# PRADUMAN-KR/Multimodal-Lip-Sync-Deepfake-Detection-System

Hardware: NVIDIA B200
Metric: windows_per_sec (higher is better)
Workload: dtype bf16

## Files before the change

### multimodal-lip-sync-deepfake-detection-system_b200/csrc/bf16_path.cu

```cuda
#include "forward_common.h"
#include "tok_front.cuh"
#include "tok_fused.cuh"
#include "token_kernels.cuh"
#include "umma_conv.cuh"
#include "stem_ring.cuh"

#include <cuda_fp16.h>

#include <algorithm>
#include <array>
#include <cstdio>
#include <cstdlib>
#include <cstring>
#include <functional>

using namespace lsd;
using namespace lsdfw;

#define LSD_ENV(name) ([]() -> const char* { static const char* const v_ = getenv(name); return v_; }())

namespace {

uint16_t f2bf(float f) {
  uint32_t u;
  memcpy(&u, &f, 4);
  if ((u & 0x7F800000u) == 0x7F800000u) return (uint16_t)(u >> 16);
  u += 0x7FFFu + ((u >> 16) & 1u);
  return (uint16_t)(u >> 16);
}

BGroup make_group(const ConvP& c, int sh, int sw, bool merge_kt = false) {
  BGroup g;
  g.Cin = c.Cin;
  for (int a = 0; a < c.kt; ++a)
    for (int b = 0; b < c.kh; ++b)
      for (int d = 0; d < c.kw; ++d) {
        BTap t;
        t.orig = (a * c.kh + b) * c.kw + d;
        t.dt = a - c.kt / 2;
        int hp = 0, wp = 0;
        const int oh = b - c.kh / 2, ow = d - c.kw / 2;
        if (sh == 2) { hp = oh & 1; t.dh = (oh - hp) / 2; } else t.dh = oh;
        if (sw == 2) { wp = ow & 1; t.dw = (ow - wp) / 2; } else t.dw = ow;
        const int set = hp * 2 + wp;
        BBand* band = nullptr;
        for (BBand& bb : g.bands)
          if (bb.set == set && (merge_kt || bb.taps[0].dt == t.dt) && (int)bb.taps.size() < UC_MAX_TAPS) band = &bb;
        if (!band) { g.bands.push_back(BBand{set, {}}); band = &g.bands.back(); }
        band->taps.push_back(t);
      }
  g.taps_total = c.kt * c.kh * c.kw;
  g.k16 = c.Cin / 16;
  return g;
}

BGroup make_group_toeplitz(const ConvP& c, int kpix, int dw_units) {
  BGroup g;
  g.Cin = c.Cin;
  g.toeplitz = 1;
  g.k16 = kpix * 4 / 16;
  for (int a = 0; a < c.kt; ++a)
    for (int b = 0; b < c.kh; ++b) {
      BTap t;
      t.orig = a * c.kh + b;
      t.dt = a - c.kt / 2;
      const int oh = b - c.kh / 2;
      const int hp = oh & 1;
      t.dh = (oh - hp) / 2;
      t.dw = dw_units;
      BBand* band = nullptr;
      for (BBand& bb : g.bands)
        if (bb.set == hp && bb.taps[0].dt == t.dt) band = &bb;
      if (!band) { g.bands.push_back(BBand{hp, {}}); band = &g.bands.back(); }
      band->taps.push_back(t);
    }
  g.taps_total = c.kt * c.kh;
  return g;
}

struct Packer {
  lsd_handle* h;
  const std::vector<float>& f32;
  std::vector<uint16_t> w;
  std::vector<float> bias;
  int ds_sh = 2, ds_sw = 2;
  void pack_group(BGroup& g, const ConvP& c, int ntile, int part = 0) {
    g.w_off = w.size();
    const int Cout = c.Cout;
    const float* W = &f32[c.w_off];
    const float* sc = c.has_scale ? &f32[c.scale_off] : nullptr;
    g.slice_stride = (size_t)(c.Cin / 16) * g.taps_total * ntile * 16;
    for (int sl = 0; sl < Cout / ntile; ++sl)
      for (int ch = 0; ch < c.Cin / 16; ++ch)
        for (const BBand& b : g.bands)
          for (const BTap& t : b.taps)
            for (int kc = 0; kc < 2; ++kc)
              for (int nn = 0; nn < ntile; ++nn)
                for (int e = 0; e < 8; ++e) {
                  const int ci = ch * 16 + kc * 8 + e, n = sl * ntile + nn;
                  const float v = W[((size_t)t.orig * c.Cin + ci) * Cout + n] * (sc ? sc[n] : 1.0f);
                  const uint16_t hi = f2bf(v);
                  if (part == 0) w.push_back(hi);
                  else { uint32_t u = (uint32_t)hi << 16; float hf; memcpy(&hf, &u, 4); w.push_back(f2bf(v - hf)); }
                }
  }
  void add_toeplitz(const std::string& name, const std::string& key, int kpix, int dw_units, bool dup_lo = false, bool halves = false) {
    const ConvP& c = h->convs.at(key);
    BLayer L;
    L.Cout = c.Cout;
    L.ntile = c.Cout;
    L.halves = halves;
    L.groups.push_back(make_group_toeplitz(c, kpix, dw_units));
    BGroup& g = L.groups[0];
    g.w_off = w.size();
    const float* W = &f32[c.w_off];
    const float* sc = c.has_scale ? &f32[c.scale_off] : nullptr;
    const int nsl = halves ? 2 : 1, ncol = c.Cout / nsl;
    g.slice_stride = (size_t)g.k16 * g.taps_total * ncol * 16;
    for (int sl = 0; sl < nsl; ++sl)
    for (int ch = 0; ch < g.k16; ++ch)
      for (const BBand& b : g.bands)
        for (const BTap& t : b.taps)
          for (int kc = 0; kc < 2; ++kc)
            for (int n = sl * ncol; n < (sl + 1) * ncol; ++n)
              for (int e = 0; e < 8; ++e) {
                const int k = ch * 16 + kc * 8 + e, j = k / 4, kw = j - 1;
                int ci = k % 4;
                const bool lo_part = dup_lo && ci == 2;
                if (dup_lo) ci = ci < 3 ? 0 : 99;
                float v = 0.f;
                if (ci < c.Cin && kw >= 0 && kw < c.kw) v = W[((size_t)(t.orig * c.kw + kw) * c.Cin + ci) * c.Cout + n] * (sc ? sc[n] : 1.0f);
                const uint16_t hi = f2bf(v);
                if (!lo_part) w.push_back(hi);
                else { uint32_t u = (uint32_t)hi << 16; float hf; memcpy(&hf, &u, 4); w.push_back(f2bf(v - hf)); }
              }
    L.bias_off = bias.size();
    for (int i = 0; i < c.Cout; ++i) bias.push_back(f32[c.shift_off + i]);
    while (w.size() % 64) w.push_back(0);
    h->blayers[name] = L;
  }
  void add(const std::string& name, const std::string& key, int sh, int sw, const std::string& ds_key = "", int ntile = 0, bool split = false,
           bool merge_kt = false, bool halves = false) {
    const ConvP& c = h->convs.at(key);
    BLayer L;
    L.Cout = c.Cout;
    L.ntile = ntile > 0 ? ntile : c.Cout;
    L.halves = halves;
    L.groups.push_back(make_group(c, sh, sw, merge_kt));
    pack_group(L.groups[0], c, halves ? L.ntile / 2 : L.ntile);
    if (split) {
      BGroup g1 = L.groups[0]; g1.src = 2;
      BGroup g2 = make_group(c, sh, sw, merge_kt);
      pack_group(g2, c, L.ntile, 1);
      L.groups.push_back(g1);
      L.groups.push_back(g2);
    }
    L.bias_off = bias.size();
    for (int i = 0; i < c.Cout; ++i) bias.push_back(f32[c.shift_off + i]);
    if (!ds_key.empty()) {
      const ConvP& d = h->convs.at(ds_key);
      const int sh_ds = ds_sh, sw_ds = ds_sw;
      BGroup gd = make_group(d, sh_ds, sw_ds);
      gd.src = 1;
      pack_group(gd, d, L.ntile);
      L.groups.push_back(gd);
      if (split) {
        BGroup g1 = gd; g1.src = 3;
        BGroup g2 = make_group(d, sh_ds, sw_ds); g2.src = 1;
        pack_group(g2, d, L.ntile, 1);
        L.groups.push_back(g1);
        L.groups.push_back(g2);
      }
      for (int i = 0; i < c.Cout; ++i) bias[L.bias_off + i] += f32[d.shift_off + i];
    }
    while (w.size() % 64) w.push_back(0);
    h->blayers[name] = L;
  }
  void add_fold(const std::string& name, const std::string& key, const std::string& ds_key, int ntile) {
    const ConvP& c = h->convs.at(key);
    if (c.kt != 3 || c.kh != 3 || c.kw != 3 || c.Cout % ntile) return;
    BLayer L;
    L.Cout = c.Cout;
    L.ntile = ntile;
    BGroup g;
    g.Cin = c.Cin;
    g.taps_total = 27;
    g.k16 = c.Cin / 16;
    for (int b = 0; b < 3; ++b)
      for (int d = 0; d < 3; ++d) {
        BBand band{b * 3 + d, {}};
        for (int a = 0; a < 3; ++a) band.taps.push_back(BTap{(a * 3 + b) * 3 + d, a - 1, b - 1, d - 1});
        g.bands.push_back(band);
      }
    pack_group(g, c, ntile);
    L.groups.push_back(g);
    L.bias_off = bias.size();
    for (int i = 0; i < c.Cout; ++i) bias.push_back(f32[c.shift_off + i]);
    if (!ds_key.empty()) {
      const ConvP& d = h->convs.at(ds_key);
      BGroup gd = make_group(d, 1, 1);
      gd.src = 1;
      pack_group(gd, d, ntile);
      L.groups.push_back(gd);
      for (int i = 0; i < c.Cout; ++i) bias[L.bias_off + i] += f32[d.shift_off + i];
    }
    while (w.size() % 64) w.push_back(0);
    h->blayers[name] = L;
  }
  void add_split(const std::string& name, const std::string& key, int ntile) {
    const ConvP& c = h->convs.at(key);
    BLayer L;
    L.Cout = c.Cout;
    L.ntile = ntile;
    BGroup g0 = make_group(c, 1, 1);
    pack_group(g0, c, ntile, 0);
    BGroup g1 = g0; g1.src = 2;
    BGroup g2 = make_group(c, 1, 1);
    pack_group(g2, c, ntile, 1);
    L.groups = {g0, g1, g2};
    L.bias_off = bias.size();
    for (int i = 0; i < c.Cout; ++i) bias.push_back(f32[c.shift_off + i]);
    while (w.size() % 64) w.push_back(0);
    h->blayers[name] = L;
  }
};

struct PBuf {
  size_t off = 0;
  int C = 0, sets = 1;
  UcGeom g;
  int64_t plane_stride = 0, set_stride = 0, origin = 0;
  size_t bytes() const { return (size_t)sets * set_stride * 2; }
};

constexpr int TILE_MAX = 1024;

PBuf make_pbuf(int C, int sets, UcGeom g) {
  PBuf b;
  b.C = C; b.sets = sets; b.g = g;
  const int64_t gf = ((int64_t)g.SL + 3 * g.RW + 16 + 7) / 8 * 8;
  const int64_t gb = gf + TILE_MAX;
  const int64_t plane_pos = (gf + g.P_total + gb + 7) / 8 * 8;
  b.origin = gf * 8;
  b.plane_stride = plane_pos * 8;
  b.set_stride = b.plane_stride * (C / 8);
  return b;
}

bool fold_route(int H, int W) {
  static const bool off = LSD_ENV("LSD_FOLD") && atoi(LSD_ENV("LSD_FOLD")) == 0;
  return !off && H * W <= 36;
}

struct BPlan {
  Shapes s;
  bool fold3 = false, fold4 = false;
  Plan f32;
  std::map<std::string, PBuf> pb;
  size_t planar_begin = 0, planar_end = 0;
  UcGeom gt, g33, gta;
  void addp(const char* name, int C, int sets, UcGeom g) {
    PBuf b = make_pbuf(C, sets, g);
    f32.cursor = (f32.cursor + 255) & ~size_t(255);
    b.off = f32.cursor;
    f32.cursor += b.bytes();
    pb[name] = b;
  }
};

void build_plan(const Shapes& s, BPlan& P, bool video = true) {
  P.s = s;
  Plan& p = P.f32;
  const int64_t B = s.B, T = s.T, TA = s.A4;
  if (video) p.add("vid", B * T * s.H * s.W * 3);
  p.add("aud", B * s.F * s.Ta);
  if (video) p.add("v_feat", B * T * 256);
  p.add("a_feat", B * TA * 256);
  if (video) {
  p.add("v_emb", B * T * 256);
  p.add("a_emb", B * TA * 256);
  p.add("a_int", B * T * 256);
  p.add("proj_v", B * T * 768);
  p.add("proj_a", B * T * 768);
  p.add("vcomb", B * T * 1024);
  }
  p.add("acomb", B * T * 1024);
  p.add("a_fint", B * T * 256);
  p.add("gate_in", B * T * 512);
  if (video) p.add("gate_h", B * T * 256);
  p.add("fused", B * T * 256);
  p.add("tok", B * (T + 1) * 256);
  if (video) {
  p.add("tok_qkv", B * (T + 1) * 768);
  p.add("comb", B * 448);
  }
  P.planar_begin = (p.cursor + 255) & ~size_t(255);
  const int Bn = s.B, Tn = s.T;
  const UcGeom g1 = make_geom(Bn, Tn, s.H1, s.W1), g2 = make_geom(Bn, Tn, s.H2, s.W2), g3 = make_geom(Bn, Tn, s.H3, s.W3),
               g4 = make_geom(Bn, Tn, s.H4, s.W4), gd = make_geom(Bn, s.Td, s.H4, s.W4), gh = make_geom(Bn, Tn, s.Hg, s.Wg);
  const UcGeom gs = make_geom_ex(Bn, Tn, s.Hs, s.Ws, 1, 2, 0, 0, 2);
  if (video) {
  P.addp("xs", 8, 2, gs);
  P.addp("xl", 8, 2, gs);
  P.addp("s_out", 64, 1, gs);
  P.addp("x1", 64, 1, g1);
  P.addp("l1a", 64, 1, g1);
  P.addp("y1", 64, 4, g2);
  P.addp("l2a", 128, 1, g2);
  P.fold3 = fold_route(s.H3, s.W3);
  P.fold4 = fold_route(s.H4, s.W4);
  const UcGeom gr = make_geom_ex(Bn, Tn, 1, 1, 1, 0, 0, 0, 0);
  if (P.fold3) P.addp("y2", 128, s.H2 * s.W2, gr); else P.addp("y2", 128, 4, g3);
  if (P.fold3) P.addp("l3a", 256, s.H3 * s.W3, gr); else P.addp("l3a", 256, 1, g3);
  if (P.fold4) P.addp("y3", 256, s.H3 * s.W3, gr); else P.addp("y3", 256, 4, g4);
  if (P.fold4) P.addp("l4a", 256, s.H4 * s.W4, gr); else P.addp("l4a", 256, 1, g4);
  P.addp("y4", 256, 1, g4);
  P.addp("art_a", 128, 1, g4);
  P.addp("art_b", 64, 1, g4);
  P.addp("delta", 256, 1, gd);
  P.addp("artd_a", 128, 1, gd);
  P.addp("artd_b", 64, 1, gd);
  P.addp("hf_f", 32, 4, gh);
  P.addp("hf_b", 64, 1, gh);
  }
  const UcGeom as = make_geom_ex(Bn, 1, s.Fs, s.As, 0, 2, 0, 0, 4);
  auto g2d = [&](int H, int W) { return make_geom_ex(Bn, 1, H, W, 0, 1, 0, 1, 0); };
  P.addp("xa", 8, 2, as);
  for (const char* sfx : {"", "_lo"}) {
    auto nm = [&](const char* n) { return std::string(n) + sfx; };
    P.addp(nm("sa_out").c_str(), 64, 1, as);
    P.addp(nm("a1").c_str(), 64, 1, g2d(s.F1, s.A1));
    P.addp(nm("a1a").c_str(), 64, 1, g2d(s.F1, s.A1));
    P.addp(nm("ya1").c_str(), 64, 4, g2d(s.F2, s.A2));
    P.addp(nm("a2a").c_str(), 128, 1, g2d(s.F2, s.A2));
    P.addp(nm("ya2").c_str(), 128, 4, g2d(s.F3, s.A3));
    P.addp(nm("a3a").c_str(), 256, 1, g2d(s.F3, s.A3));
    P.addp(nm("ya3").c_str(), 256, 4, g2d(s.F4, s.A4));
    P.addp(nm("a4a").c_str(), 256, 1, g2d(s.F4, s.A4));
    P.addp(nm("ya4").c_str(), 256, 1, g2d(s.F4, s.A4));
  }
  P.gt = make_geom_ex(Bn, 1, 1, Tn, 0, 0, 0, 3, 0);
  P.g33 = make_geom_rows(Bn * (Tn + 1));
  P.gta = make_geom_rows(Bn * (int)TA);
  for (const char* sfx : {"", "_lo"}) {
    auto nm = [&](const char* n) { return std::string(n) + sfx; };
    P.addp(nm("afeat_p").c_str(), 256, 1, P.gta);
    if (!video) { P.addp(nm("afint_p").c_str(), 256, 1, P.gt); continue; }
    for (const char* n : {"vfeat_p", "vemb_p", "aint_p", "afint_p", "att1_p", "att2_p", "blend_p", "fused_p"}) P.addp(nm(n).c_str(), 256, 1, P.gt);
    P.addp(nm("gatein_p").c_str(), 512, 1, P.gt);
    P.addp(nm("mscat_p").c_str(), 768, 1, P.gt);
    P.addp(nm("tokln_p").c_str(), 256, 1, P.g33);
    P.addp(nm("tokatt_p").c_str(), 256, 1, P.g33);
    P.addp(nm("tokff_p").c_str(), 1024, 1, P.g33);
  }
  P.planar_end = p.cursor;
}

struct BCtx {
  lsd_handle* h;
  char* ws;
  const BPlan* P;
  cudaStream_t st;
  int max_ctas = 0;
  __nv_bfloat16* base(const PBuf& b) const { return reinterpret_cast<__nv_bfloat16*>(ws + b.off); }
  __nv_bfloat16* org(const PBuf& b) const { return base(b) + b.origin; }
  float* f(const char* name) const { return reinterpret_cast<float*>(ws + P->f32.find(name)); }
  const float* W(const char* key) const { return h->warena + h->vecs.at(key); }
};

struct UArgs {
  const PBuf* in = nullptr;
  const PBuf* in_ds = nullptr;
  const PBuf* in_lo = nullptr;
  const PBuf* in_ds_lo = nullptr;
  const PBuf* res_lo = nullptr;
  const PBuf* yp_lo = nullptr;
  UcGeom og;
  int act = ACT_NONE;
  const PBuf* yp = nullptr;
  int y_plane_off = 0;
  int y_mode = -1;
  const PBuf* res = nullptr;
  float* y32 = nullptr;
  int y32_ld = 0, y32_outer_stride = -1, y32_row_off = 0;
  const float* res32 = nullptr;
  int res32_ld = 0;
};

int stage_program(const BCtx& c, const std::string& name, UmmaConvP& p, const std::function<void(std::vector<UcStageDesc>&)>& build,
                  std::initializer_list<uint64_t> salt = {}) {
  uint64_t hkey = 1469598103934665603ull;
  for (uint64_t v : salt) { hkey ^= v; hkey *= 1099511628211ull; hkey ^= hkey >> 29; }
  static_assert(sizeof(UmmaConvP) % 8 == 0, "UmmaConvP is hashed in 8-byte words");
  const uint64_t* pw = reinterpret_cast<const uint64_t*>(&p);
  for (size_t i = 0; i < sizeof(p) / 8; ++i) { hkey ^= pw[i]; hkey *= 1099511628211ull; hkey ^= hkey >> 29; }
  auto it = c.h->prog_cache.find(hkey);
  if (it == c.h->prog_cache.end()) {
    std::vector<UcStageDesc> host;
    build(host);
    const size_t bytes = host.size() * sizeof(UcStageDesc);
    if (!c.h->prog_arena) {
      c.h->prog_cap = 64u << 20;
      if (cudaMalloc(&c.h->prog_arena, c.h->prog_cap) != cudaSuccess) return lsd_fail(c.h, LSD_ERR_CUDA, "stage-program arena allocation failed");
      c.h->prog_cursor = 0;
    }
    if (c.h->prog_cursor + bytes > c.h->prog_cap) {
      cudaDeviceSynchronize();
      c.h->prog_cache.clear();
      c.h->prog_cursor = 0;
      ++c.h->generation;
    }
    char* dst = c.h->prog_arena + c.h->prog_cursor;
    cudaError_t e = cudaMemcpy(dst, host.data(), bytes, cudaMemcpyHostToDevice);
    if (e != cudaSuccess) return lsd_fail(c.h, LSD_ERR_CUDA, "%s: stage program upload: %s", name.c_str(), cudaGetErrorString(e));
    c.h->prog_cursor += (bytes + 255) & ~size_t(255);
    it = c.h->prog_cache.emplace(hkey, dst).first;
  }
  p.prog = reinterpret_cast<const UcStageDesc*>(it->second);
  return 0;
}

int run_umma(const BCtx& c, const std::string& name, const UArgs& a) {
  const BLayer& L = c.h->blayers.at(name);
  const UcGeom& og = a.og;
  if (og.P_total >= ((int64_t)1 << 31) - 1024) return lsd_fail(c.h, LSD_ERR_SHAPE, "%s: more than 2^31 padded positions in one launch (reduce the batch)", name.c_str());
  UmmaConvP p;
  memset(&p, 0, sizeof(p));
  p.w = reinterpret_cast<const __nv_bfloat16*>(c.h->barena);
  p.bias = c.h->bbias + L.bias_off;
  p.Cout = L.ntile;
  const int slices = L.Cout / L.ntile;
  p.act = a.act;
  p.g = og;
  p.cta2 = L.halves ? 1 : 0;
  if (a.yp) {
    p.y_mode = a.y_mode >= 0 ? a.y_mode : (a.yp->sets == 4 ? UC_Y_PARITY : UC_Y_PLAIN);
    p.y = c.org(*a.yp) + (int64_t)a.y_plane_off * a.yp->plane_stride;
    p.y_plane_stride = a.yp->plane_stride; p.y_set_stride = a.yp->set_stride;
    p.g2 = a.yp->g;
    p.ymap_W = og.W;
    if (a.yp_lo) p.ylo = c.org(*a.yp_lo) + (int64_t)a.y_plane_off * a.yp_lo->plane_stride;
  }
  if (a.y32) {
    p.y32 = a.y32; p.y32_ld = a.y32_ld;
    p.y32_outer_stride = a.y32_outer_stride >= 0 ? a.y32_outer_stride : og.W;
    p.y32_row_off = a.y32_row_off;
  }
  if (a.res) { p.res = c.org(*a.res); p.res_plane_stride = a.res->plane_stride; }
  if (a.res_lo) p.res_lo = c.org(*a.res_lo);
  if (a.res32) { p.res32 = a.res32; p.res32_ld = a.res32_ld; }
  const int mt_cap = L.ntile <= 32 ? 8 : 4;
  const int mt2 = std::max(1, std::min(mt_cap, 256 / L.ntile));
  p.MT = std::max(1, std::min(mt_cap, 512 / L.ntile));
  const int cta_budget = (c.max_ctas > 0 && c.max_ctas < c.h->num_sms) ? c.max_ctas : c.h->num_sms;
  while (p.MT > 1 && ((og.P_total + p.MT * 128 - 1) / (p.MT * 128)) * slices < cta_budget) p.MT /= 2;
  p.nbuf = (p.MT <= mt2 && 2 * p.MT * L.ntile <= 512) ? 2 : 1;
  if (const char* e = LSD_ENV("LSD_UMMA_NBUF")) {
    const int v = atoi(e);
    if (v == 1) p.nbuf = 1;
    if (v == 2 && 2 * L.ntile <= 512) { p.nbuf = 2; p.MT = std::min(p.MT, mt2); }
  }
  p.issuers = std::min(p.MT, 4);
  if (const char* e = LSD_ENV("LSD_UMMA_ISSUERS")) { const int v = atoi(e); if (v >= 1 && v <= 4 && v <= p.MT && p.MT % v == 0 && p.MT / v <= 4) p.issuers = v; }
  uint32_t cols = 32;
  while ((int)cols < p.nbuf * p.MT * L.ntile) cols *= 2;
  p.tmem_cols = cols;
  const int S = p.MT * 128;
  int nb = 0, max_a = 0, max_taps = 0, min_k16 = 1 << 30;
  bool any_toeplitz = false;
  p.ngroups = (int)L.groups.size();
  for (int gi = 0; gi < p.ngroups; ++gi) {
    const BGroup& G = L.groups[gi];
    const PBuf* srcp = G.src == 0 ? a.in : (G.src == 1 ? a.in_ds : (G.src == 2 ? a.in_lo : a.in_ds_lo));
    if (!srcp) return lsd_fail(c.h, LSD_ERR_ARG, "%s: missing input for group %d", name.c_str(), gi);
    const PBuf& src = *srcp;
    UcGroup& ug = p.groups[gi];
    ug.band_begin = nb;
    ug.k16 = G.k16;
    ug.taps_total = G.taps_total;
    ug.w_off = (int64_t)G.w_off;
    ug.slice_stride = (int64_t)G.slice_stride;
    int tap_begin = 0;
    int wkb = 40;
    if (const char* e = LSD_ENV("LSD_UMMA_WKB")) wkb = std::max(8, atoi(e));
    const int tmax = std::max(1, std::min(UC_MAX_TAPS, (wkb * 1024) / (L.ntile * 32)));
    for (const BBand& b : G.bands) {
      const int nt = (int)b.taps.size();
      const int pieces = (nt + tmax - 1) / tmax, per = (nt + pieces - 1) / pieces;
      for (int t0 = 0; t0 < nt; t0 += per) {
        const int t1 = std::min(nt, t0 + per);
        if (nb >= UC_MAX_BANDS) return lsd_fail(c.h, LSD_ERR_UNSUPPORTED, "%s: too many bands", name.c_str());
        UcBand& ub = p.bands[nb++];
        ub.base = c.org(src) + (int64_t)b.set * src.set_stride;
        ub.plane_stride = src.plane_stride;
        ub.toeplitz = G.toeplitz;
        ub.chunk_stride = G.toeplitz ? 16 : 2 * src.plane_stride;
        int mn = INT32_MAX, mx = INT32_MIN;
        for (int j = t0; j < t1; ++j) {
          const BTap& t = b.taps[j];
          const int sft = t.dt * og.SL + t.dh * og.RW + t.dw;
          mn = std::min(mn, sft); mx = std::max(mx, sft);
        }
        ub.start = mn;
        ub.len_extra = mx - mn;
        ub.ntaps = t1 - t0;
        ub.tap_begin = tap_begin;
        for (int j = t0; j < t1; ++j) ub.rel[j - t0] = b.taps[j].dt * og.SL + b.taps[j].dh * og.RW + b.taps[j].dw - mn;
        tap_begin += ub.ntaps;
        max_a = std::max(max_a, G.toeplitz ? (S + ub.len_extra + 1 + 2 * (G.k16 - 1)) * 16 : 2 * (S + ub.len_extra) * 16);
        max_taps = std::max(max_taps, ub.ntaps);
        min_k16 = std::min(min_k16, G.k16);
        any_toeplitz = any_toeplitz || G.toeplitz;
        if (-(int64_t)ub.start * 8 > src.origin || (int64_t)mx * 8 > src.origin)
          return lsd_fail(c.h, LSD_ERR_UNSUPPORTED, "%s: guard zone too small", name.c_str());
      }
    }
    ug.band_end = nb;
  }
  p.nbands = nb;
  const int w_chunk = max_taps * (L.halves ? L.ntile / 2 : L.ntile) * 32;
  if (any_toeplitz) p.kpack = min_k16;
  else {
    bool single_band = true;
    for (int gi = 0; gi < p.ngroups; ++gi) single_band = single_band && (p.groups[gi].band_end - p.groups[gi].band_begin) == 1;
    int stage_kb = single_band ? 64 : 24;
    if (const char* e = LSD_ENV("LSD_UMMA_STAGE_KB")) stage_kb = std::max(8, atoi(e));
    p.kpack = std::max(1, std::min(std::min(8, min_k16), (stage_kb * 1024) / (max_a + w_chunk)));
  }
  p.a_stage_bytes = ((uint32_t)(any_toeplitz ? max_a : max_a * p.kpack) + 127u) & ~127u;
  p.w_stage_bytes = (uint32_t)(w_chunk * p.kpack);
  const uint32_t stage = p.a_stage_bytes + p.w_stage_bytes;
  p.nst_tile = 0;
  for (int gi = 0; gi < p.ngroups; ++gi)
    p.nst_tile += ((p.groups[gi].k16 + p.kpack - 1) / p.kpack) * (p.groups[gi].band_end - p.groups[gi].band_begin);
  const uint32_t prog_bytes = (uint32_t)p.nst_tile * (uint32_t)umma_conv_stage_desc_bytes();
  uint32_t budget = 211u * 1024u;
  const uint32_t extra_bytes = (uint32_t)umma_conv_extra_smem_bytes(p);
  budget -= extra_bytes;
  if (prog_bytes + 2 * stage > budget) return lsd_fail(c.h, LSD_ERR_UNSUPPORTED, "%s: stage program of %u bytes does not fit", name.c_str(), prog_bytes);
  int stages = (int)((budget - prog_bytes) / stage);
  stages = std::max(2, std::min(stages, 8));
  if ((size_t)stages * stage + prog_bytes + extra_bytes + 1024 > 223u * 1024u) return lsd_fail(c.h, LSD_ERR_UNSUPPORTED, "%s: stage of %u bytes does not fit", name.c_str(), stage);
  p.stages = stages;
  double kflop = 0;
  for (const BGroup& G : L.groups) kflop += (double)G.taps_total * G.Cin;
  if (L.groups[0].toeplitz) { const ConvP& cp = c.h->convs.at(name); kflop = (double)cp.kt * cp.kh * cp.kw * cp.Cin; }
  if (const char* e = getenv("LSD_UMMA_SKIP")) p.skip = atoi(e);
  if (const char* why = umma_conv_config_error(p)) return lsd_fail(c.h, LSD_ERR_UNSUPPORTED, "%s: %s", name.c_str(), why);
  if (int rc = stage_program(c, name, p, [&](std::vector<UcStageDesc>& v) { v.resize((size_t)p.nst_tile); umma_conv_build_program(p, v.data()); }))
    return rc;
  if (const char* e = getenv("LSD_UMMA_TRACE")) {
    static long long* dbuf = nullptr;
    if (!dbuf) cudaMalloc(&dbuf, 512);
    cudaMemsetAsync(dbuf, 0, 512, c.st);
    p.dbg = dbuf;
    launch_umma_conv(p, slices, c.st, c.h->num_sms, c.max_ctas);
    long long hv[64];
    cudaMemcpyAsync(hv, dbuf, 512, cudaMemcpyDeviceToHost, c.st);
    cudaStreamSynchronize(c.st);
    if (atoi(e) > 0)
      fprintf(stderr, "[umma] %-34s MT=%d N=%d slices=%d stages=%d kpack=%d tiles=%lld | prologue %lld, first-data %lld, mma-issued %lld, acc-done %lld, epi-done %lld, total %lld cycles\n",
              name.c_str(), p.MT, p.Cout, slices, p.stages, p.kpack, hv[7], hv[1] - hv[0], hv[2] - hv[0], hv[3] - hv[0], hv[4] - hv[0], hv[5] - hv[0], hv[6] - hv[0]);
    if (atoi(e) > 1) {
      fprintf(stderr, "        full-wait done at:");
      for (int i = 0; i < 24 && hv[8 + i]; ++i) fprintf(stderr, " %lld", hv[8 + i] - hv[0]);
      fprintf(stderr, "\n        producer issue at:");
      for (int i = 0; i < 24 && hv[32 + i]; ++i) fprintf(stderr, " %lld", hv[32 + i] - hv[0]);
      fprintf(stderr, "\n        copies issued at: ");
      for (int i = 0; i < 8 && hv[56 + i]; ++i) fprintf(stderr, " %lld", hv[56 + i] - hv[0]);
      fprintf(stderr, "\n");
    }
    return 0;
  }
  c.h->prof.begin(c.st, 2.0 * (double)og.N * og.T * og.H * og.W * L.Cout * kflop, name.rfind("visual_encoder.", 0) == 0 ? 2 : 3);
  launch_umma_conv(p, slices, c.st, c.h->num_sms, c.max_ctas);
  c.h->prof.end(c.st);
  return 0;
}

int ring_table(const BCtx& c, const UcGeom& g, const lsd_handle::RingTab** out) {
  lsd_handle* h = c.h;
  const int T = g.T, CH = (g.SL + 127) / 128;
  const int64_t G = (int64_t)g.N * CH * T;
  const int budget = (c.max_ctas > 0 && c.max_ctas < h->num_sms) ? c.max_ctas : h->num_sms;
  uint64_t key = 1469598103934665603ull;
  for (uint64_t v : {(uint64_t)g.N, (uint64_t)T, (uint64_t)g.SL, (uint64_t)g.TS, (uint64_t)g.ot, (uint64_t)budget}) { key ^= v; key *= 1099511628211ull; key ^= key >> 29; }
  auto it = h->ring_tabs.find(key);
  if (it == h->ring_tabs.end()) {
    int grid = budget;
    int64_t Lr = (G + 2 * (int64_t)grid - 1) / (2 * (int64_t)grid);
    if (Lr < 8) { Lr = 8; grid = (int)((G + 2 * Lr - 1) / (2 * Lr)); }
    if (grid < 1) grid = 1;
    std::vector<std::vector<SrStep>> lists((size_t)2 * grid);
    size_t nsteps = 0;
    auto add_range = [&](int sg, int64_t col, int ta, int tb) {
      const int n = (int)(col / CH), sp = (int)(col % CH);
      const int t_first = std::max(ta - 1, 0);
      for (int t_in = t_first; t_in <= tb; ++t_in) {
        SrStep st;
        st.in_pos = (int32_t)(((int64_t)n * g.TS + t_in + g.ot) * g.SL + (int64_t)sp * 128);
        const int t_out = t_in - 1;
        st.flags = SR_ACTIVE | (t_in == t_first ? SR_FIRST : 0u) | ((t_out >= ta && t_out < tb) ? SR_STORE : 0u) |
                   ((uint32_t)std::min(128, g.SL - sp * 128) << 8);
        lists[sg].push_back(st);
      }
    };
    for (int sg = 0; sg < 2 * grid; ++sg) {
      int64_t g0 = (int64_t)sg * Lr;
      const int64_t g1 = std::min(G, g0 + Lr);
      while (g0 < g1) {
        const int64_t col = g0 / T;
        const int ta = (int)(g0 % T), tb = (int)std::min<int64_t>(T, ta + (g1 - g0));
        add_range(sg, col, ta, tb);
        g0 += tb - ta;
      }
    }
    for (int sg = 0; sg < 2 * grid; ++sg) nsteps = std::max(nsteps, lists[sg].size());
    std::vector<SrStep> flat((size_t)2 * grid * nsteps);
    memset(flat.data(), 0, flat.size() * sizeof(SrStep));
    for (int sg = 0; sg < 2 * grid; ++sg) std::copy(lists[sg].begin(), lists[sg].end(), flat.begin() + (size_t)sg * nsteps);
    lsd_handle::RingTab tab;
    tab.nsteps = (int)nsteps; tab.grid = grid;
    if (cudaMalloc(&tab.dev, std::max<size_t>(flat.size(), 1) * sizeof(SrStep)) != cudaSuccess ||
        cudaMemcpy(tab.dev, flat.data(), flat.size() * sizeof(SrStep), cudaMemcpyHostToDevice) != cudaSuccess)
      return lsd_fail(h, LSD_ERR_CUDA, "stem: step table upload failed");
    it = h->ring_tabs.emplace(key, tab).first;
  }
  *out = &it->second;
  return 0;
}

int run_stem_ring(const BCtx& c, const PBuf& xs, const PBuf& so) {
  lsd_handle* h = c.h;
  const UcGeom& g = xs.g;
  if (g.P_total >= ((int64_t)1 << 31) - 4096) return lsd_fail(h, LSD_ERR_SHAPE, "stem: more than 2^31 padded positions in one launch (reduce the batch)");
  const BLayer& L = h->blayers.at("visual_encoder.stem");
  StemRingP p;
  memset(&p, 0, sizeof(p));
  p.xs[0] = c.org(xs);
  p.xs[1] = c.org(xs) + xs.set_stride;
  p.w = reinterpret_cast<const __nv_bfloat16*>(h->barena) + h->stem_ring_w_off;
  p.bias = h->bbias + L.bias_off;
  p.y = c.org(so);
  p.y_plane_stride = so.plane_stride;
  p.g = g;
  p.ntap[0] = 3; p.ntap[1] = 4;
  for (int t = 0; t < 4; ++t) { p.rel[0][t] = t * g.RW; p.rel[1][t] = t * g.RW; }
  p.start[0] = -g.RW; p.start[1] = -2 * g.RW;
  p.units[0] = 128 + 2 * g.RW + 3; p.units[1] = 128 + 3 * g.RW + 3;
  if ((int64_t)(2 * g.RW + 3) * 8 > xs.origin) return lsd_fail(h, LSD_ERR_UNSUPPORTED, "stem: guard zone too small");
  const lsd_handle::RingTab* tab = nullptr;
  if (int trc = ring_table(c, g, &tab)) return trc;
  p.steps = reinterpret_cast<const SrStep*>(tab->dev);
  p.nsteps = tab->nsteps;
  p.nst = 6;
  if (const char* e = getenv("LSD_SR_SKIP")) p.skip = atoi(e);
  while (p.nst > 3 && stem_ring_smem_bytes(p) > 223u * 1024u) --p.nst;
  if (stem_ring_smem_bytes(p) > 223u * 1024u) return lsd_fail(h, LSD_ERR_UNSUPPORTED, "stem: batch too large for the ring kernel (LSD_STEM_RING=0)");
  const ConvP& cp = h->convs.at("visual_encoder.stem");
  h->prof.begin(c.st, 2.0 * (double)g.N * g.T * g.H * g.W * 64.0 * (double)cp.kt * cp.kh * cp.kw * cp.Cin, 2);
  if (getenv("LSD_SR_TRACE")) {
    static long long* dbuf = nullptr;
    constexpr int kDbg = 256 + 4 * 160;
    if (!dbuf) cudaMalloc(&dbuf, kDbg * sizeof(long long));
    cudaMemsetAsync(dbuf, 0, kDbg * sizeof(long long), c.st);
    p.dbg = dbuf;
    launch_stem_ring(p, tab->grid, c.st);
    long long hv[kDbg];
    cudaMemcpyAsync(hv, dbuf, sizeof(hv), cudaMemcpyDeviceToHost, c.st);
    cudaStreamSynchronize(c.st);
    {
      long long g0 = INT64_MAX, g1 = 0, cmin = INT64_MAX, cmax = 0, csum = 0, smax = 0;
      const int nc = std::min(tab->grid, 160);
      for (int i = 0; i < nc; ++i) g0 = std::min(g0, hv[256 + 4 * i]);
      for (int i = 0; i < nc; ++i) {
        const long long* d = hv + 256 + 4 * i;
        g1 = std::max(g1, d[1]); smax = std::max(smax, d[0] - g0);
        const long long cy = d[3] - d[2];
        cmin = std::min(cmin, cy); cmax = std::max(cmax, cy); csum += cy;
      }
      fprintf(stderr, "[sr] %d CTAs x %d steps: kernel span %.1f us (globaltimer), latest CTA start +%.1f us, CTA cycles min %lld avg %lld max %lld\n", nc,
              p.nsteps, (g1 - g0) / 1e3, smax / 1e3, cmin, csum / nc, cmax);
    }
    const long long t0 = hv[0];
    for (int k = 0; k < 32; ++k)
      fprintf(stderr, "[sr] step %2d | prod free %7lld issued %7lld | mma landed %7lld blockfree %7lld issued %7lld | epi complete %7lld back %7lld\n", k + 16,
              hv[(0 * 32 + k) * 2] - t0, hv[(0 * 32 + k) * 2 + 1] - t0, hv[(1 * 32 + k) * 2] - t0, hv[(1 * 32 + k) * 2 + 1] - t0,
              hv[(2 * 32 + k) * 2] - t0, hv[(3 * 32 + k) * 2] - t0, hv[(3 * 32 + k) * 2 + 1] - t0);
    h->prof.end(c.st);
    return 0;
  }
  launch_stem_ring(p, tab->grid, c.st);
  h->prof.end(c.st);
  return 0;
}

#define RUN(name, ...)                            \
  do {                                            \
    UArgs a_;                                     \
    __VA_ARGS__;                                  \
    if ((rc = run_umma(b, name, a_))) return rc;  \
  } while (0)

#define RUNC(ctx, name, ...)                        \
  do {                                              \
    UArgs a_;                                       \
    __VA_ARGS__;                                    \
    if ((rc = run_umma(ctx, name, a_))) return rc;  \
  } while (0)

#define RUNS(name, ...)                            \
  do {                                             \
    UArgs a_;                                      \
    __VA_ARGS__;                                   \
    if ((rc = run_umma(bs, name, a_))) return rc;  \
  } while (0)

PlanarOut pout(const BCtx& c, const PBuf& p, const PBuf* lo = nullptr, int plane_off = 0) {
  PlanarOut o;
  o.y = c.org(p) + (int64_t)plane_off * p.plane_stride;
  o.ylo = lo ? c.org(*lo) + (int64_t)plane_off * lo->plane_stride : nullptr;
  o.plane_stride = p.plane_stride;
  if (p.g.ow > 0 && p.g.HP == 1) { o.grp = p.g.W; o.grp_stride = p.g.RW; o.off = p.g.ow; }
  else { o.grp = 0; o.grp_stride = 0; o.off = 0; }
  return o;
}

int res_stage_umma(const BCtx& b, const std::string& p, const PBuf& x, const PBuf& mid, const PBuf& y, bool has_ds, int y_mode,
                   const PBuf* x_lo = nullptr, const PBuf* mid_lo = nullptr, const PBuf* y_lo = nullptr) {
  int rc = 0;
  RUN(p + ".conv1", a_.in = &x; a_.in_lo = x_lo; a_.og = mid.g; a_.act = ACT_RELU; a_.yp = &mid; a_.yp_lo = mid_lo);
  if (has_ds) RUN(p + ".conv2", a_.in = &mid; a_.in_lo = mid_lo; a_.in_ds = &x; a_.in_ds_lo = x_lo; a_.og = mid.g; a_.act = ACT_RELU;
                  a_.yp = &y; a_.yp_lo = y_lo; a_.y_mode = y_mode);
  else RUN(p + ".conv2", a_.in = &mid; a_.in_lo = mid_lo; a_.og = mid.g; a_.act = ACT_RELU; a_.yp = &y; a_.yp_lo = y_lo; a_.y_mode = y_mode;
           a_.res = &x; a_.res_lo = x_lo);
  return 0;
}

int run_umma_fold(const BCtx& c, const std::string& name, const PBuf& x, int Hi, int Wi, int stride, const PBuf* x_ds, int Hd, int Wd,
                  int Ho, int Wo, const PBuf& yp, int y_mode) {
  const auto itL = c.h->blayers.find(name + "#fold");
  if (itL == c.h->blayers.end()) return lsd_fail(c.h, LSD_ERR_UNSUPPORTED, "%s: no weights packed for the folded route (LSD_FOLD=0)", name.c_str());
  const BLayer& L = itL->second;
  const UcGeom& og = x.g;
  if (og.P_total >= ((int64_t)1 << 31) - 1024) return lsd_fail(c.h, LSD_ERR_SHAPE, "%s: more than 2^31 rows in one launch (reduce the batch)", name.c_str());
  if ((L.groups.size() == 2) != (x_ds != nullptr) || x.sets != Hi * Wi || (x_ds && x_ds->sets != Hd * Wd))
    return lsd_fail(c.h, LSD_ERR_ARG, "%s: folded inputs do not match the layer", name.c_str());
  UmmaConvP p;
  memset(&p, 0, sizeof(p));
  p.w = reinterpret_cast<const __nv_bfloat16*>(c.h->barena);
  p.bias = c.h->bbias + L.bias_off;
  p.Cout = L.ntile;
  p.act = ACT_RELU;
  p.g = og;
  p.fold = 1;
  p.y_mode = y_mode;
  p.y = c.org(yp);
  p.y_plane_stride = yp.plane_stride; p.y_set_stride = yp.set_stride;
  p.g2 = yp.g;
  p.ymap_W = Wo;
  int mt = 2;
  if (const char* e = LSD_ENV("LSD_FOLD_MT")) mt = std::max(1, std::min(4, atoi(e)));
  p.MT = (int)std::max<int64_t>(1, std::min<int64_t>(mt, (og.P_total + 127) / 128));
  p.nbuf = 1;
  p.issuers = std::min(p.MT, 4);
  uint32_t cols = 32;
  while ((int)cols < p.MT * L.ntile) cols *= 2;
  p.tmem_cols = cols;
  const int S = p.MT * 128;
  const PBuf* srcs[2] = {&x, x_ds};
  p.ngroups = (int)L.groups.size();
  p.nbands = p.ngroups;
  int max_a = 0, max_w = 0, min_k16 = 1 << 30;
  for (int gi = 0; gi < p.ngroups; ++gi) {
    const BGroup& G = L.groups[gi];
    UcGroup& ug = p.groups[gi];
    ug.band_begin = gi; ug.band_end = gi + 1;
    ug.k16 = G.k16; ug.taps_total = G.taps_total;
    ug.w_off = (int64_t)G.w_off; ug.slice_stride = (int64_t)G.slice_stride;
    UcBand& ub = p.bands[gi];
    const PBuf& src = *srcs[gi];
    ub.base = c.org(src);
    ub.plane_stride = src.plane_stride;
    ub.chunk_stride = 2 * src.plane_stride;
    ub.ntaps = gi == 0 ? 3 : 1;
    ub.start = gi == 0 ? -1 : 0;
    ub.len_extra = gi == 0 ? 2 : 0;
    for (int j = 0; j < ub.ntaps; ++j) ub.rel[j] = j;
    if ((int64_t)8 > src.origin) return lsd_fail(c.h, LSD_ERR_UNSUPPORTED, "%s: guard zone too small", name.c_str());
    max_a = std::max(max_a, 2 * (S + ub.len_extra) * 16);
    max_w = std::max(max_w, ub.ntaps * L.ntile * 32);
    min_k16 = std::min(min_k16, G.k16);
  }
  p.kpack = std::max(1, std::min(std::min(8, min_k16), (48 * 1024) / (max_a + max_w)));
  p.a_stage_bytes = ((uint32_t)(max_a * p.kpack) + 127u) & ~127u;
  p.w_stage_bytes = (uint32_t)(max_w * p.kpack);
  const int cslices = L.Cout / L.ntile;
  std::vector<std::array<int, 3>> pos;
  auto inb = [&](int o, int k, int n) { const int i = stride * o + k - 1; return i >= 0 && i < n; };
  for (int ho = 0; ho < Ho; ++ho)
    for (int wo = 0; wo < Wo; ++wo) {
      int nq = 0;
      for (int kh = 0; kh < 3; ++kh)
        for (int kw = 0; kw < 3; ++kw) nq += inb(ho, kh, Hi) && inb(wo, kw, Wi);
      pos.push_back({-nq, ho, wo});
    }
  std::stable_sort(pos.begin(), pos.end(), [](const std::array<int, 3>& a, const std::array<int, 3>& b) { return a[0] < b[0]; });
  const int nslices = (int)pos.size() * cslices;
  if (nslices > UC_MAX_FSLICES || Ho > 255 || Wo > 255) return lsd_fail(c.h, LSD_ERR_UNSUPPORTED, "%s: map too large for the folded route", name.c_str());
  auto chunks = [&](int k16) { return (k16 + p.kpack - 1) / p.kpack; };
  int off = 0;
  for (int i = 0; i < nslices; ++i) {
    const auto& q = pos[(size_t)(i / cslices)];
    const int nst = -q[0] * chunks(p.groups[0].k16) + (x_ds ? chunks(p.groups[1].k16) : 0);
    p.fslice[i] = UcFoldSlice{(uint16_t)off, (uint16_t)nst, (uint8_t)q[1], (uint8_t)q[2], (uint8_t)(i % cslices), 0};
    p.nst_tile = std::max(p.nst_tile, nst);
    off += nst;
  }
  if (off > 65535) return lsd_fail(c.h, LSD_ERR_UNSUPPORTED, "%s: folded stage programs too long", name.c_str());
  const uint32_t stage = p.a_stage_bytes + p.w_stage_bytes;
  const uint32_t prog_bytes = (uint32_t)p.nst_tile * (uint32_t)umma_conv_stage_desc_bytes();
  const uint32_t budget = 211u * 1024u - (uint32_t)umma_conv_extra_smem_bytes(p);
  if (prog_bytes + 2 * stage > budget) return lsd_fail(c.h, LSD_ERR_UNSUPPORTED, "%s: stage program of %u bytes does not fit", name.c_str(), prog_bytes);
  p.stages = std::max(2, std::min((int)((budget - prog_bytes) / stage), 8));
  if (const char* e = getenv("LSD_UMMA_SKIP")) p.skip = atoi(e);
  if (const char* why = umma_conv_config_error(p)) return lsd_fail(c.h, LSD_ERR_UNSUPPORTED, "%s: %s", name.c_str(), why);
  auto build = [&](std::vector<UcStageDesc>& v) {
    for (int i = 0; i < nslices; ++i) {
      const UcFoldSlice& f = p.fslice[i];
      for (int kh = 0; kh < 3; ++kh)
        for (int kw = 0; kw < 3; ++kw) {
          if (!inb(f.h, kh, Hi) || !inb(f.w, kw, Wi)) continue;
          UcBand bq = p.bands[0];
          bq.base = c.org(x) + (int64_t)((stride * f.h + kh - 1) * Wi + stride * f.w + kw - 1) * x.set_stride;
          bq.tap_begin = (kh * 3 + kw) * 3;
          for (int c0 = 0; c0 < p.groups[0].k16; c0 += p.kpack) v.push_back(umma_conv_stage(p, p.groups[0], bq, 0, c0, f.col));
        }
      if (x_ds) {
        UcBand bd = p.bands[1];
        bd.base = c.org(*x_ds) + (int64_t)(2 * f.h * Wd + 2 * f.w) * x_ds->set_stride;
        for (int c0 = 0; c0 < p.groups[1].k16; c0 += p.kpack) v.push_back(umma_conv_stage(p, p.groups[1], bd, 1, c0, f.col));
      }
    }
  };
  if (int rc = stage_program(c, name + "#fold", p, build, {(uint64_t)Hi, (uint64_t)Wi, (uint64_t)stride, (uint64_t)Hd, (uint64_t)Wd,
                                                          (uint64_t)x.set_stride, (uint64_t)(x_ds ? x_ds->set_stride : 0)})) return rc;
  double kflop = 0;
  for (const BGroup& G : L.groups) kflop += (double)G.taps_total * G.Cin;
  c.h->prof.begin(c.st, 2.0 * (double)og.N * og.T * Ho * Wo * L.Cout * kflop, 2);
  launch_umma_conv(p, nslices, c.st, c.h->num_sms, c.max_ctas);
  c.h->prof.end(c.st);
  return 0;
}

int res_stage_fold(const BCtx& b, const std::string& p, const PBuf& x, int Hi, int Wi, const PBuf& mid, int Ho, int Wo, const PBuf& y, int y_mode) {
  int rc = 0;
  if ((rc = run_umma_fold(b, p + ".conv1", x, Hi, Wi, 2, nullptr, 0, 0, Ho, Wo, mid, UC_Y_FOLD))) return rc;
  return run_umma_fold(b, p + ".conv2", mid, Ho, Wo, 1, &x, Hi, Wi, Ho, Wo, y, y_mode);
}

}

static int pack_tok_fused(lsd_handle* h, const std::vector<float>& f32) {
  std::vector<TfBlock> blocks;
  tf_layer_blocks(blocks);
  std::vector<uint32_t> stage_bytes;
  for (const TfBlock& b : blocks)
    for (int k0 = 0; k0 < b.k16; k0 += b.kps) stage_bytes.push_back((uint32_t)b.kps * (uint32_t)b.N * 32u);
  std::vector<__half> w;
  std::vector<float> vec((size_t)TF_LAYERS * TF_VEC_LAYER + (size_t)(2 * TF_LAYERS + 1) * TF_D, 0.f);
  std::vector<float> cum(TF_D, 0.f);
  float* cum_out = vec.data() + (size_t)TF_LAYERS * TF_VEC_LAYER;
  for (int l = 0; l < TF_LAYERS; ++l) {
    const std::string k = "t" + std::to_string(l);
    const ConvP &cin = h->convs.at(k + ".in"), &cout = h->convs.at(k + ".out"), &cf1 = h->convs.at(k + ".ff1"), &cf2 = h->convs.at(k + ".ff2");
    const size_t w0 = w.size();
    for (const TfBlock& b : blocks) {
      const ConvP& c = b.kind == 0 ? cin : (b.kind == 1 ? cout : (b.kind == 2 ? cf1 : cf2));
      for (int k16 = 0; k16 < b.k16; ++k16)
        for (int pl = 0; pl < 2; ++pl)
          for (int n = 0; n < b.N; ++n)
            for (int e = 0; e < 8; ++e) {
              const int kk = k16 * 16 + pl * 8 + e;
              int co, ci;
              if (b.kind == 0) { co = ((n % 96) / 32) * 256 + (2 * b.idx + n / 96) * 32 + (n % 32); ci = kk; }
              else if (b.kind == 1) { co = n; ci = 64 * b.idx + kk; }
              else if (b.kind == 2) { co = 128 * b.idx + n; ci = kk; }
              else { co = n; ci = 128 * b.idx + kk; }
              w.push_back(__float2half_rn(f32[c.w_off + (size_t)ci * c.Cout + co]));
            }
    }
    if (l == 0) h->tokf_layer_bytes = (uint32_t)((w.size() - w0) * sizeof(__half));
    float* lv = vec.data() + (size_t)l * TF_VEC_LAYER;
    const char* names[4] = {".ln1.w", ".ln1.b", ".ln2.w", ".ln2.b"};
    for (int i = 0; i < 4; ++i) memcpy(lv + 256 * i, &f32[h->vecs.at(k + names[i])], 256 * sizeof(float));
    for (int n = 0; n < 768; ++n) {
      const int hp = n / 192, r = n % 192;
      lv[1024 + n] = f32[cin.shift_off + ((r % 96) / 32) * 256 + (2 * hp + r / 96) * 32 + (r % 32)];
    }
    memcpy(lv + 1024 + 768, &f32[cf1.shift_off], 1024 * sizeof(float));
    memcpy(cum_out + (size_t)(2 * l) * TF_D, cum.data(), TF_D * sizeof(float));
    for (int i = 0; i < TF_D; ++i) cum[i] += f32[cout.shift_off + i];
    memcpy(cum_out + (size_t)(2 * l + 1) * TF_D, cum.data(), TF_D * sizeof(float));
    for (int i = 0; i < TF_D; ++i) cum[i] += f32[cf2.shift_off + i];
  }
  memcpy(cum_out + (size_t)(2 * TF_LAYERS) * TF_D, cum.data(), TF_D * sizeof(float));
  h->tokf_n_stage = (int)stage_bytes.size();
  for (void* q : {(void*)h->tokf_w, (void*)h->tokf_stage_bytes, (void*)h->tokf_vec}) if (q) cudaFree(q);
  h->tokf_w = nullptr; h->tokf_stage_bytes = nullptr; h->tokf_vec = nullptr;
  cudaError_t e = cudaMalloc(&h->tokf_w, w.size() * sizeof(__half));
  if (e == cudaSuccess) e = cudaMemcpy(h->tokf_w, w.data(), w.size() * sizeof(__half), cudaMemcpyHostToDevice);
  if (e == cudaSuccess) e = cudaMalloc(&h->tokf_stage_bytes, stage_bytes.size() * sizeof(uint32_t));
  if (e == cudaSuccess) e = cudaMemcpy(h->tokf_stage_bytes, stage_bytes.data(), stage_bytes.size() * sizeof(uint32_t), cudaMemcpyHostToDevice);
  if (e == cudaSuccess) e = cudaMalloc(&h->tokf_vec, vec.size() * sizeof(float));
  if (e == cudaSuccess) e = cudaMemcpy(h->tokf_vec, vec.data(), vec.size() * sizeof(float), cudaMemcpyHostToDevice);
  if (e != cudaSuccess) return lsd_fail(h, LSD_ERR_CUDA, "pack_tok_fused: %s", cudaGetErrorString(e));
  return 0;
}

static int pack_tok_front(lsd_handle* h, const std::vector<float>& f32) {
  std::vector<__half> w;
  w.reserve((size_t)TFR_K16_TOTAL * 16 * 256);
  auto emit = [&](int k16, auto&& get) {
    for (int k = 0; k < k16; ++k)
      for (int pl = 0; pl < 2; ++pl)
        for (int n = 0; n < 256; ++n)
          for (int e = 0; e < 8; ++e) w.push_back(__float2half_rn(get(k * 16 + pl * 8 + e, n)));
  };
  const ConvP &o0 = h->convs.at("cross.v2a.out"), &o1 = h->convs.at("cross.a2v.out"), &g0 = h->convs.at("cross.gate0"),
              &fu = h->convs.at("cross.fuse"), &pp = h->convs.at("temporal.pre_scale_proj");
  for (const ConvP* o : {&o0, &o1})
    for (int hp = 0; hp < 4; ++hp) emit(4, [&](int ci, int co) { return f32[o->w_off + (size_t)(64 * hp + ci) * 256 + co]; });
  emit(32, [&](int ci, int co) { return f32[g0.w_off + (size_t)ci * 256 + co]; });
  emit(16, [&](int ci, int co) { return f32[fu.w_off + (size_t)ci * 256 + co]; });
  const int ks[3] = {3, 5, 7};
  for (int b = 0; b < 3; ++b) {
    const ConvP& c = h->convs.at("temporal.branch_k" + std::to_string(ks[b]));
    for (int j = 0; j < ks[b]; ++j)
      emit(16, [&](int ci, int co) { return f32[c.w_off + ((size_t)j * 256 + ci) * 256 + co] * (c.has_scale ? f32[c.scale_off + co] : 1.0f); });
    emit(16, [&](int ci, int co) { return f32[pp.w_off + (size_t)(256 * b + ci) * 256 + co]; });
  }
  if (w.size() != (size_t)TFR_N_STAGES * TFR_STAGE_BYTES / sizeof(__half)) return lsd_fail(h, LSD_ERR_WEIGHTS, "pack_tok_front: stream size mismatch");
  std::vector<float> vec(TFR_V_TOTAL, 0.f);
  auto cp = [&](int dst, size_t src, int n) { memcpy(vec.data() + dst, &f32[src], (size_t)n * sizeof(float)); };
  cp(TFR_V_BO0, o0.shift_off, 256); cp(TFR_V_BO1, o1.shift_off, 256); cp(TFR_V_BG0, g0.shift_off, 256);
  cp(TFR_V_WG2, h->vecs.at("cross.gate2.w"), 256); cp(TFR_V_BG2, h->vecs.at("cross.gate2.b"), 1);
  cp(TFR_V_BF, fu.shift_off, 256);
  cp(TFR_V_SH3, h->convs.at("temporal.branch_k3").shift_off, 256); cp(TFR_V_SH5, h->convs.at("temporal.branch_k5").shift_off, 256);
  cp(TFR_V_SH7, h->convs.at("temporal.branch_k7").shift_off, 256);
  cp(TFR_V_BP, pp.shift_off, 256); cp(TFR_V_CLS, h->vecs.at("temporal.cls"), 256);
  for (void* q : {(void*)h->tokfr_w, (void*)h->tokfr_vec}) if (q) cudaFree(q);
  h->tokfr_w = nullptr; h->tokfr_vec = nullptr;
  cudaError_t e = cudaMalloc(&h->tokfr_w, w.size() * sizeof(__half));
  if (e == cudaSuccess) e = cudaMemcpy(h->tokfr_w, w.data(), w.size() * sizeof(__half), cudaMemcpyHostToDevice);
  if (e == cudaSuccess) e = cudaMalloc(&h->tokfr_vec, vec.size() * sizeof(float));
  if (e == cudaSuccess) e = cudaMemcpy(h->tokfr_vec, vec.data(), vec.size() * sizeof(float), cudaMemcpyHostToDevice);
  if (e != cudaSuccess) return lsd_fail(h, LSD_ERR_CUDA, "pack_tok_front: %s", cudaGetErrorString(e));
  return 0;
}

int pack_bf16_weights(lsd_handle* h, const std::vector<float>& f32_arena) {
  Packer P{h, f32_arena, {}, {}};
  memcpy(h->lapw_host, &f32_arena[h->convs.at("art.lap").w_off], sizeof(h->lapw_host));
  h->blayers.clear();
  const int vstr[4] = {1, 2, 2, 2};
  for (int l = 1; l <= 4; ++l) {
    const std::string p = "visual_encoder.layer" + std::to_string(l);
    const int s = vstr[l - 1];
    int nt = l >= 3 ? 128 : 0;
    if (const char* e = getenv(l == 3 ? "LSD_UMMA_NT3" : (l == 4 ? "LSD_UMMA_NT4" : "LSD_UMMA_NTX"))) nt = atoi(e);
    const bool pairs = l == 1;
    P.add(p + ".conv1", p + ".conv1", s, s, "", nt, false, l >= 2, pairs);
    P.ds_sh = 2; P.ds_sw = 2;
    P.add(p + ".conv2", p + ".conv2", 1, 1, l == 1 ? "" : p + ".downsample", nt, false, false, pairs);
    if (l >= 3) {
      int fnt = 128;
      if (const char* e = LSD_ENV("LSD_FOLD_NT")) fnt = atoi(e) == 256 ? 256 : 128;
      P.add_fold(p + ".conv1#fold", p + ".conv1", "", fnt);
      P.add_fold(p + ".conv2#fold", p + ".conv2", p + ".downsample", fnt);
    }
  }
  P.add_toeplitz("visual_encoder.stem", "visual_encoder.stem", 8, 0, false, true);
  {
    const ConvP& c = h->convs.at("visual_encoder.stem");
    h->stem_ring_w_off = 0;
    if (c.kt == 3 && c.kh == 7 && c.kw == 7 && c.Cin == 3 && c.Cout == 64) {
      h->stem_ring_w_off = P.w.size();
      const float* W = &f32_arena[c.w_off];
      const float* sc = c.has_scale ? &f32_arena[c.scale_off] : nullptr;
      for (int set = 0; set < 2; ++set)
        for (int b = 0; b < 7; ++b) {
          if (((b - 3) & 1) != set) continue;
          for (int ch = 0; ch < 2; ++ch)
            for (int kc = 0; kc < 2; ++kc)
              for (int n = 0; n < 192; ++n)
                for (int e = 0; e < 8; ++e) {
                  const int k = ch * 16 + kc * 8 + e, j = k / 4, kw = j - 1, ci = k % 4, a = n / 64, co = n % 64;
                  float v = 0.f;
                  if (ci < 3 && kw >= 0 && kw < 7) v = W[((size_t)((a * 7 + b) * 7 + kw) * 3 + ci) * 64 + co] * (sc ? sc[co] : 1.0f);
                  P.w.push_back(f2bf(v));
                }
        }
      while (P.w.size() % 64) P.w.push_back(0);
    }
  }
  P.add_toeplitz("art.hf0", "art.hf0", 4, 1);
  P.add("art.td0", "art.td0", 1, 1);
  P.add("art.td3", "art.td3", 1, 1);
  P.add("art.hf3", "art.hf3", 2, 2);
  P.add_toeplitz("audio_encoder.stem", "audio_encoder.stem", 8, 0, true);
  const int ash[4] = {1, 2, 2, 2}, asw[4] = {1, 2, 1, 1};
  for (int l = 1; l <= 4; ++l) {
    const std::string p = "audio_encoder.layer" + std::to_string(l);
    P.add(p + ".conv1", p + ".conv1", ash[l - 1], asw[l - 1], "", 0, true);
    P.ds_sh = ash[l - 1]; P.ds_sw = asw[l - 1];
    P.add(p + ".conv2", p + ".conv2", 1, 1, l == 1 ? "" : p + ".downsample", 0, true);
  }
  int wide = 128;
  if (const char* e = LSD_ENV("LSD_UMMA_NTW")) wide = atoi(e);
  int narrow = 64;
  if (const char* e = LSD_ENV("LSD_UMMA_NTN")) narrow = atoi(e);
  for (const char* k : {"projection.visual_proj", "projection.audio_proj", "cross.v2a.out", "cross.a2v.out",
                        "cross.gate0", "cross.fuse", "temporal.branch_k3", "temporal.branch_k5", "temporal.branch_k7",
                        "temporal.pre_scale_proj"})
    P.add_split(k, k, narrow);
  for (const char* k : {"cross.in_v", "cross.in_a", "cross.vcomb", "cross.acomb"}) P.add_split(k, k, wide);
  for (int l = 0; l < 4; ++l)
    for (const char* k : {".in", ".out", ".ff1", ".ff2"})
      P.add_split("t" + std::to_string(l) + k, "t" + std::to_string(l) + k, (k[1] == 'i' || (k[1] == 'f' && k[3] == '1')) ? wide : narrow);
  if (h->barena) { cudaFree(h->barena); h->barena = nullptr; }
  if (h->bbias) { cudaFree(h->bbias); h->bbias = nullptr; }
  cudaError_t e = cudaMalloc(&h->barena, P.w.size() * 2);
  if (e == cudaSuccess) e = cudaMemcpy(h->barena, P.w.data(), P.w.size() * 2, cudaMemcpyHostToDevice);
  if (e == cudaSuccess) e = cudaMalloc(&h->bbias, P.bias.size() * 4);
  if (e == cudaSuccess) e = cudaMemcpy(h->bbias, P.bias.data(), P.bias.size() * 4, cudaMemcpyHostToDevice);
  if (e != cudaSuccess) return lsd_fail(h, LSD_ERR_CUDA, "pack_bf16_weights: %s", cudaGetErrorString(e));
  if (int rc = pack_tok_fused(h, f32_arena)) return rc;
  return pack_tok_front(h, f32_arena);
}

void make_plan_bf16(lsd_handle* h, int B, int T, int H, int W, int F, int Ta, std::vector<Stage>& stages, size_t& bytes) {
  Shapes s;
  if (make_shapes(h, B, T, H, W, F, Ta, s) != 0) { bytes = 0; return; }
  BPlan P;
  build_plan(s, P);
  stages = P.f32.stages;
  bytes = P.f32.cursor;
}

struct Timeline {
  bool on = false;
  std::vector<std::pair<std::string, cudaEvent_t>> marks;
  void mark(cudaStream_t st, const char* name) {
    if (!on) return;
    cudaEvent_t e; cudaEventCreate(&e); cudaEventRecord(e, st);
    marks.emplace_back(name, e);
  }
  void dump() {
    if (!on || marks.empty()) return;
    cudaDeviceSynchronize();
    fprintf(stderr, "[timeline]");
    for (auto& m : marks) { float ms = 0; cudaEventElapsedTime(&ms, marks[0].second, m.second); fprintf(stderr, " %s=%.0f", m.first.c_str(), ms * 1000.0f); }
    fprintf(stderr, " (us)\n");
    for (auto& m : marks) cudaEventDestroy(m.second);
    marks.clear();
  }
};
static Timeline g_tl;

static int audio_encoder_bf16(const BCtx& b, const Shapes& s, bool inputs_ready, const void* audio, int adt) {
  const BPlan& P = *b.P;
  auto pbf = [&](const char* n) -> const PBuf& { return P.pb.at(n); };
  cudaStream_t st = b.st;
  int rc = 0;
  const PBuf &xa = pbf("xa"), &sao = pbf("sa_out"), &a1 = pbf("a1");
  if (inputs_ready) launch_audio_rows(b.f("aud"), LSD_F32, b.org(xa), xa.set_stride, xa.g, s.F, s.Ta, st);
  else launch_audio_rows(audio, adt, b.org(xa), xa.set_stride, xa.g, s.F, s.Ta, st);
  RUN("audio_encoder.stem", a_.in = &xa; a_.og = xa.g; a_.act = ACT_RELU; a_.yp = &sao; a_.yp_lo = &pbf("sa_out_lo"));
  launch_planar_maxpool(b.org(sao), sao.plane_stride, sao.g, b.org(a1), a1.plane_stride, a1.g, 64, st, b.org(pbf("sa_out_lo")), b.org(pbf("a1_lo")));
  if ((rc = res_stage_umma(b, "audio_encoder.layer1", a1, pbf("a1a"), pbf("ya1"), false, UC_Y_PARITY, &pbf("a1_lo"), &pbf("a1a_lo"), &pbf("ya1_lo")))) return rc;
  if ((rc = res_stage_umma(b, "audio_encoder.layer2", pbf("ya1"), pbf("a2a"), pbf("ya2"), true, UC_Y_PARITY_H, &pbf("ya1_lo"), &pbf("a2a_lo"), &pbf("ya2_lo")))) return rc;
  if ((rc = res_stage_umma(b, "audio_encoder.layer3", pbf("ya2"), pbf("a3a"), pbf("ya3"), true, UC_Y_PARITY_H, &pbf("ya2_lo"), &pbf("a3a_lo"), &pbf("ya3_lo")))) return rc;
  if ((rc = res_stage_umma(b, "audio_encoder.layer4", pbf("ya3"), pbf("a4a"), pbf("ya4"), true, UC_Y_PLAIN, &pbf("ya3_lo"), &pbf("a4a_lo"), &pbf("ya4_lo")))) return rc;
  const PBuf& ya4 = pbf("ya4");
  launch_planar_mean2(b.org(ya4), ya4.plane_stride, ya4.g, 256, b.f("a_feat"), 256, 2, pout(b, pbf("afeat_p"), &pbf("afeat_p_lo")), st,
                      b.org(pbf("ya4_lo")));
  return 0;
}

static bool token_front_enabled(int T) {
  const char* e = getenv("LSD_TOK_FRONT");
  return !(e && atoi(e) == 0) && tok_front_supported(T);
}
static int token_path_bf16(const BCtx& b, const Shapes& s, bool combined = false, const float* vcomb = nullptr, int K = 1) {
  const BPlan& P = *b.P;
  auto pbf = [&](const char* n) -> const PBuf& { return P.pb.at(n); };
  cudaStream_t st = b.st;
  const int B = s.B, T = s.T, TA = s.A4, NT = T + 1;
  const UcGeom gt = P.gt;
  int rc = 0;
  lsd_handle* h = b.h;
  if (!h->tok_stream[0]) {
    for (int i = 0; i < 2; ++i)
      if (cudaStreamCreateWithFlags(&h->tok_stream[i], cudaStreamNonBlocking) != cudaSuccess ||
          cudaEventCreateWithFlags(&h->ev_tok_join[i], cudaEventDisableTiming) != cudaSuccess)
        return lsd_fail(h, LSD_ERR_CUDA, "token helper stream creation failed");
    if (cudaEventCreateWithFlags(&h->ev_tok_fork, cudaEventDisableTiming) != cudaSuccess) return lsd_fail(h, LSD_ERR_CUDA, "token helper event creation failed");
  }
  BCtx b1 = b, b2 = b;
  b1.st = h->tok_stream[0]; b2.st = h->tok_stream[1];
  auto fork = [&](int n) { cudaEventRecord(h->ev_tok_fork, st); for (int i = 0; i < n; ++i) cudaStreamWaitEvent(h->tok_stream[i], h->ev_tok_fork, 0); };
  auto join = [&](int n) { for (int i = 0; i < n; ++i) { cudaEventRecord(h->ev_tok_join[i], h->tok_stream[i]); cudaStreamWaitEvent(st, h->ev_tok_join[i], 0); } };
  float *pv = combined ? nullptr : b.f("proj_v"), *pa = combined ? nullptr : b.f("proj_a"), *gi = b.f("gate_in");
  if (!combined) {
    fork(1);
    launch_lerp_tokens_p(b.f("a_emb"), b.f("a_int"), B, TA, T, 256, pout(b, pbf("aint_p"), &pbf("aint_p_lo")), b1.st);
    RUNC(b1, "cross.in_a", a_.in = &pbf("aint_p"); a_.in_lo = &pbf("aint_p_lo"); a_.og = gt; a_.y32 = pa; a_.y32_ld = 768);
    RUN("cross.in_v", a_.in = &pbf("vemb_p"); a_.in_lo = &pbf("vemb_p_lo"); a_.og = gt; a_.y32 = pv; a_.y32_ld = 768);
    join(1);
  }
  g_tl.mark(st, "T:inproj");
  float* tok = b.f("tok");
  if (token_front_enabled(T)) {
    TokFrontP fp;
    memset(&fp, 0, sizeof(fp));
    if (combined) {
      fp.v_emb = vcomb ? vcomb : b.f("vcomb"); fp.pv = fp.v_emb + 256; fp.a_int = b.f("acomb"); fp.pa = fp.a_int + 256;
      fp.ld_e = 1024; fp.ld_p = 1024;
    } else {
      fp.pv = pv; fp.pa = pa; fp.v_emb = b.f("v_emb"); fp.a_int = b.f("a_int");
      fp.ld_e = 256; fp.ld_p = 768;
    }
    fp.gi = gi; fp.fused = b.f("fused"); fp.tok = tok;
    fp.w = reinterpret_cast<const __half*>(h->tokfr_w);
    fp.vec = h->tokfr_vec;
    fp.B = B; fp.T = T; fp.K = K;
    tok_front_geometry(T, fp.SL, fp.G, fp.KW);
    if (getenv("LSD_TOKF_TRACE")) {
      static long long* dbuf = nullptr;
      if (!dbuf) cudaMalloc(&dbuf, 256 * sizeof(long long));
      cudaMemsetAsync(dbuf, 0, 256 * sizeof(long long), st);
      fp.dbg = dbuf;
      launch_tok_front(fp, st);
      std::vector<long long> hv(256);
      cudaMemcpyAsync(hv.data(), dbuf, 256 * sizeof(long long), cudaMemcpyDeviceToHost, st);
      cudaStreamSynchronize(st);
      const long long t0 = hv[128];
      fprintf(stderr, "[tokfront] compute (start=0) then (hand-over, next arrival):");
      for (int i = 0; i < 63 && hv[128 + 2 * i + 1]; ++i) fprintf(stderr, " (%lld,%lld)", hv[128 + 2 * i + 1] - t0, hv[128 + 2 * i + 2] ? hv[128 + 2 * i + 2] - t0 : 0);
      fprintf(stderr, "\n[tokfront] mma phases (start, issue-end):");
      for (int i = 0; i < 64 && hv[2 * i + 1]; ++i) fprintf(stderr, " (%lld,%lld)", hv[2 * i] - t0, hv[2 * i + 1] - t0);
      fprintf(stderr, "\n");
      fp.dbg = nullptr;
    } else
    launch_tok_front(fp, st);
    g_tl.mark(st, "T:cross");
  } else {
  fork(1);
  launch_mha_core_p(pv, 768, pa + 256, 768, pa + 512, 768, B, T, T, 8, pout(b, pbf("att1_p"), &pbf("att1_p_lo")), st);
  RUN("cross.v2a.out", a_.in = &pbf("att1_p"); a_.in_lo = &pbf("att1_p_lo"); a_.og = gt; a_.res32 = b.f("v_emb"); a_.res32_ld = 256; a_.y32 = gi; a_.y32_ld = 512;
      a_.yp = &pbf("gatein_p"); a_.yp_lo = &pbf("gatein_p_lo"));
  launch_mha_core_p(pa, 768, pv + 256, 768, pv + 512, 768, B, T, T, 8, pout(b, pbf("att2_p"), &pbf("att2_p_lo")), b1.st);
  RUNC(b1, "cross.a2v.out", a_.in = &pbf("att2_p"); a_.in_lo = &pbf("att2_p_lo"); a_.og = gt; a_.res32 = b.f("a_int"); a_.res32_ld = 256; a_.y32 = gi + 256; a_.y32_ld = 512;
      a_.yp = &pbf("gatein_p"); a_.yp_lo = &pbf("gatein_p_lo"); a_.y_plane_off = 32);
  join(1);
  RUN("cross.gate0", a_.in = &pbf("gatein_p"); a_.in_lo = &pbf("gatein_p_lo"); a_.og = gt; a_.act = ACT_GELU; a_.y32 = b.f("gate_h"); a_.y32_ld = 256);
  launch_gate_blend_p(b.f("gate_h"), b.W("cross.gate2.w"), b.W("cross.gate2.b"), gi, 512, gi + 256, 512, B * T, 256, pout(b, pbf("blend_p"), &pbf("blend_p_lo")), st);
  RUN("cross.fuse", a_.in = &pbf("blend_p"); a_.in_lo = &pbf("blend_p_lo"); a_.og = gt; a_.act = ACT_RELU; a_.y32 = b.f("fused"); a_.y32_ld = 256; a_.yp = &pbf("fused_p"); a_.yp_lo = &pbf("fused_p_lo"));
  g_tl.mark(st, "T:cross");
  fork(2);
  RUNC(b1, "temporal.branch_k5", a_.in = &pbf("fused_p"); a_.in_lo = &pbf("fused_p_lo"); a_.og = gt; a_.act = ACT_GELU; a_.yp = &pbf("mscat_p"); a_.yp_lo = &pbf("mscat_p_lo"); a_.y_plane_off = 32);
  RUNC(b2, "temporal.branch_k3", a_.in = &pbf("fused_p"); a_.in_lo = &pbf("fused_p_lo"); a_.og = gt; a_.act = ACT_GELU; a_.yp = &pbf("mscat_p"); a_.yp_lo = &pbf("mscat_p_lo"); a_.y_plane_off = 0);
  launch_set_cls(b.W("temporal.cls"), tok, B, NT, 256, b2.st);
  RUN("temporal.branch_k7", a_.in = &pbf("fused_p"); a_.in_lo = &pbf("fused_p_lo"); a_.og = gt; a_.act = ACT_GELU; a_.yp = &pbf("mscat_p"); a_.yp_lo = &pbf("mscat_p_lo"); a_.y_plane_off = 64);
  join(2);
  RUN("temporal.pre_scale_proj", a_.in = &pbf("mscat_p"); a_.in_lo = &pbf("mscat_p_lo"); a_.og = gt; a_.res32 = b.f("fused"); a_.res32_ld = 256; a_.y32 = tok; a_.y32_ld = 256;
      a_.y32_outer_stride = NT; a_.y32_row_off = 1);
  }
  const char* fused_env = getenv("LSD_TOK_FUSED");
  const bool fused_off = fused_env && atoi(fused_env) == 0;
  if (!fused_off && tok_fused_supported(NT)) {
    TokFusedP fp;
    memset(&fp, 0, sizeof(fp));
    fp.tok = tok;
    fp.w = reinterpret_cast<const __half*>(h->tokf_w);
    fp.stage_bytes = h->tokf_stage_bytes;
    fp.n_stage_layer = h->tokf_n_stage;
    fp.layer_bytes = h->tokf_layer_bytes;
    fp.vec = h->tokf_vec;
    fp.B = B; fp.NT = NT;
    tok_fused_geometry(NT, fp.SL, fp.G, fp.KW);
    if (getenv("LSD_TOKF_TRACE")) {
      static long long* dbuf = nullptr;
      if (!dbuf) cudaMalloc(&dbuf, 384 * sizeof(long long));
      cudaMemsetAsync(dbuf, 0, 384 * sizeof(long long), st);
      fp.dbg = dbuf;
      launch_tok_fused(fp, st);
      std::vector<long long> hv(384);
      cudaMemcpyAsync(hv.data(), dbuf, 384 * sizeof(long long), cudaMemcpyDeviceToHost, st);
      cudaStreamSynchronize(st);
      const long long t0 = hv[192];
      fprintf(stderr, "[tokf] compute phases (wait-return, hand-over) cycles from start:");
      for (int i = 0; i < 96 && hv[192 + 2 * i + 1]; ++i) fprintf(stderr, " (%lld,%lld)", hv[192 + 2 * i] - t0, hv[192 + 2 * i + 1] - t0);
      fprintf(stderr, "\n[tokf] mma phases (start, issue-end):");
      for (int i = 0; i < 96 && hv[2 * i + 1]; ++i) fprintf(stderr, " (%lld,%lld)", hv[2 * i] - t0, hv[2 * i + 1] - t0);
      fprintf(stderr, "\n");
      return 0;
    }
    launch_tok_fused(fp, st);
    return 0;
  }
  const UcGeom g33 = P.g33;
  for (int l = 0; l < 4; ++l) {
    const std::string k = "t" + std::to_string(l);
    launch_layernorm_p(tok, 256, b.W((k + ".ln1.w").c_str()), b.W((k + ".ln1.b").c_str()), B * NT, 256, pout(b, pbf("tokln_p"), &pbf("tokln_p_lo")), st);
    RUN(k + ".in", a_.in = &pbf("tokln_p"); a_.in_lo = &pbf("tokln_p_lo"); a_.og = g33; a_.y32 = b.f("tok_qkv"); a_.y32_ld = 768);
    const float* qkv = b.f("tok_qkv");
    launch_mha_core_p(qkv, 768, qkv + 256, 768, qkv + 512, 768, B, NT, NT, 8, pout(b, pbf("tokatt_p"), &pbf("tokatt_p_lo")), st);
    RUN(k + ".out", a_.in = &pbf("tokatt_p"); a_.in_lo = &pbf("tokatt_p_lo"); a_.og = g33; a_.res32 = tok; a_.res32_ld = 256; a_.y32 = tok; a_.y32_ld = 256);
    launch_layernorm_p(tok, 256, b.W((k + ".ln2.w").c_str()), b.W((k + ".ln2.b").c_str()), B * NT, 256, pout(b, pbf("tokln_p"), &pbf("tokln_p_lo")), st);
    RUN(k + ".ff1", a_.in = &pbf("tokln_p"); a_.in_lo = &pbf("tokln_p_lo"); a_.og = g33; a_.act = ACT_GELU; a_.yp = &pbf("tokff_p"); a_.yp_lo = &pbf("tokff_p_lo"));
    RUN(k + ".ff2", a_.in = &pbf("tokff_p"); a_.in_lo = &pbf("tokff_p_lo"); a_.og = g33; a_.res32 = tok; a_.res32_ld = 256; a_.y32 = tok; a_.y32_ld = 256);
  }
  return 0;
}


static int ws_prepare(lsd_handle* h, const Shapes& s, const BPlan& P, char* ws, size_t ws_bytes, cudaStream_t st, int slot) {
  const int sig[6] = {s.B, s.T, s.H, s.W, s.F, s.Ta};
  WsSig& mine = h->ws_sig[slot];
  for (WsSig& other : h->ws_sig) {
    if (&other == &mine || !other.ptr) continue;
    const char* o0 = reinterpret_cast<const char*>(other.ptr);
    if (o0 < ws + ws_bytes && ws < o0 + other.bytes) other.ptr = nullptr;
  }
  if (mine.ptr == ws && mine.bytes == ws_bytes && memcmp(mine.shape, sig, sizeof(sig)) == 0) return 0;
  cudaError_t e = cudaMemsetAsync(ws + P.planar_begin, 0, P.planar_end - P.planar_begin, st);
  if (e != cudaSuccess) return lsd_fail(h, LSD_ERR_CUDA, "workspace init: %s", cudaGetErrorString(e));
  mine.ptr = ws; mine.bytes = ws_bytes; memcpy(mine.shape, sig, sizeof(sig));
  return 0;
}

struct VarTail {
  int K = 1, gB = 1;
  char* ws = nullptr;
  size_t ws_bytes = 0;
  char* ws_last = nullptr;
  size_t ws_last_bytes = 0;
  const void* audio = nullptr;
  int adt = LSD_F32;
  const float* mel_full = nullptr;
  int Ta_full = 0;
  const int32_t* d_astarts = nullptr;
};

static size_t dtype_bytes(int dt) { return dt == LSD_F32 ? 4 : (dt == LSD_U8 ? 1 : 2); }

static int forward_bf16_impl(lsd_handle* h, const Shapes& s, float* logits, const lsd_aux* aux, char* ws, size_t ws_bytes,
                             cudaStream_t st, bool inputs_ready, const void* video, int vdt, int vlayout, const void* audio, int adt,
                             const int32_t* vstarts = nullptr, int n_frames = 0, int pipe_parity = -1, const VarTail* vt = nullptr) {
  BPlan P;
  build_plan(s, P);
  if (P.f32.cursor > ws_bytes) return lsd_fail(h, LSD_ERR_WORKSPACE, "workspace too small: need %zu bytes, got %zu", P.f32.cursor, ws_bytes);
  h->stages = P.f32.stages;
  h->planar_stages.clear();
  for (const auto& kv : P.pb) {
    const PBuf& b = kv.second;
    PlanarStage ps;
    ps.off = b.off; ps.C = b.C; ps.sets = b.sets; ps.plane_stride = b.plane_stride; ps.set_stride = b.set_stride; ps.origin = b.origin;
    ps.N = b.g.N; ps.T = b.g.T; ps.H = b.g.H; ps.W = b.g.W; ps.ot = b.g.ot; ps.oh = b.g.oh; ps.hp_extra = b.g.HP - b.g.H - b.g.oh;
    ps.ow = b.g.ow; ps.wp_extra = b.g.RW - b.g.W - b.g.ow;
    h->planar_stages[kv.first] = ps;
  }
  int rc0 = 0;
  if ((rc0 = ws_prepare(h, s, P, ws, ws_bytes, st, pipe_parity == 1 ? 1 : 0))) return rc0;
  BCtx b{h, ws, &P, st};
  const int B = s.B, T = s.T, TA = s.A4, NT = T + 1;
  auto& pb = P.pb;
  int rc = 0;
  if (!h->side_stream) {
    if (cudaStreamCreateWithFlags(&h->side_stream, cudaStreamNonBlocking) != cudaSuccess || cudaEventCreateWithFlags(&h->ev_fork, cudaEventDisableTiming) != cudaSuccess ||
        cudaEventCreateWithFlags(&h->ev_join, cudaEventDisableTiming) != cudaSuccess || cudaEventCreateWithFlags(&h->ev_start, cudaEventDisableTiming) != cudaSuccess ||
        cudaEventCreateWithFlags(&h->ev_audio, cudaEventDisableTiming) != cudaSuccess)
      return lsd_fail(h, LSD_ERR_CUDA, "side stream creation failed");
  }
  cudaStream_t sst = h->side_stream;
  BCtx bs{h, ws, &P, sst};
  bs.max_ctas = h->num_sms / 2;
  if (const char* e = LSD_ENV("LSD_SIDE_CTAS")) bs.max_ctas = atoi(e);
  int art_ctas = bs.max_ctas;
  if (const char* e = LSD_ENV("LSD_ART_CTAS")) art_ctas = atoi(e);
  if (const char* e = LSD_ENV("LSD_MAIN_CTAS")) { b.max_ctas = atoi(e); bs.max_ctas = h->num_sms - b.max_ctas; }
  const bool audio_early = LSD_ENV("LSD_AUDIO_LATE") == nullptr;
  const bool tcomb = token_front_enabled(T);
  auto audio_tokens = [&](const BCtx& c, const Shapes& sc) -> int {
    int rc = 0;
    const auto& q = c.P->pb;
    launch_lerp_tokens_p(c.f("a_feat"), c.f("a_fint"), sc.B, sc.A4, sc.T, 256, pout(c, q.at("afint_p"), &q.at("afint_p_lo")), c.st);
    RUNC(c, "cross.acomb", a_.in = &q.at("afint_p"); a_.in_lo = &q.at("afint_p_lo"); a_.og = c.P->gt; a_.y32 = c.f("acomb"); a_.y32_ld = 1024);
    if (aux && aux->audio_tokens) RUNC(c, "projection.audio_proj", a_.in = &q.at("afeat_p"); a_.in_lo = &q.at("afeat_p_lo"); a_.og = c.P->gta; a_.y32 = c.f("a_emb"); a_.y32_ld = 256);
    return 0;
  };
  const int n_groups = vt ? (B + vt->gB - 1) / vt->gB : 0;
  const bool short_last = vt && B - (n_groups - 1) * vt->gB < vt->gB;
  auto plan_of = [&](int g) { return short_last && g == n_groups - 1 ? 1 : 0; };
  Shapes sA[2];
  BPlan PA[2];
  char* aws[2] = {nullptr, nullptr};
  if (vt) {
    aws[0] = vt->ws; aws[1] = vt->ws_last;
    for (int i = 0; i < 2; ++i) {
      if (i != plan_of(0) && i != plan_of(n_groups - 1)) continue;
      const int nb = i == 0 ? vt->gB : B - (n_groups - 1) * vt->gB;
      const size_t cap = i == 0 ? vt->ws_bytes : vt->ws_last_bytes;
      if ((rc = make_shapes(h, nb * vt->K, T, 16, 16, s.F, s.Ta, sA[i]))) return rc;
      build_plan(sA[i], PA[i], false);
      if (!aws[i] || PA[i].f32.cursor > cap) return lsd_fail(h, LSD_ERR_WORKSPACE, "audio-variant workspace too small: need %zu bytes, got %zu", PA[i].f32.cursor, cap);
    }
  }
  auto var_audio = [&](int g, cudaStream_t stream, int max_ctas) -> int {
    const int pi = plan_of(g);
    int rc = ws_prepare(h, sA[pi], PA[pi], aws[pi], pi ? vt->ws_last_bytes : vt->ws_bytes, stream, 1 + pi);
    if (rc) return rc;
    BCtx c{h, aws[pi], &PA[pi], stream};
    c.max_ctas = max_ctas;
    const size_t r0 = (size_t)g * vt->gB * vt->K;
    if (vt->d_astarts) launch_gather_audio(vt->mel_full, s.F, vt->Ta_full, vt->d_astarts + r0, c.f("aud"), sA[pi].B, s.Ta, stream);
    const void* au = vt->audio ? reinterpret_cast<const char*>(vt->audio) + r0 * s.F * s.Ta * dtype_bytes(vt->adt) : nullptr;
    if ((rc = audio_encoder_bf16(c, sA[pi], vt->d_astarts != nullptr, au, vt->adt))) return rc;
    return audio_tokens(c, sA[pi]);
  };
  g_tl.on = LSD_ENV("LSD_TIMELINE") != nullptr;
  g_tl.mark(st, "start");
  if (vt) {
    cudaEventRecord(h->ev_start, st);
    cudaStreamWaitEvent(sst, h->ev_start, 0);
    if ((rc = var_audio(0, sst, bs.max_ctas))) return rc;
    cudaEventRecord(h->ev_audio, sst);
  } else if (audio_early) {
    cudaEventRecord(h->ev_start, st);
    cudaStreamWaitEvent(sst, h->ev_start, 0);
    if ((rc = audio_encoder_bf16(bs, s, inputs_ready, audio, adt))) return rc;
    if (tcomb && (rc = audio_tokens(bs, s))) return rc;
    g_tl.mark(sst, "S:audio_enc");
    cudaEventRecord(h->ev_audio, sst);
  }
  const PBuf &xs = pb["xs"], &xl = pb["xl"], &so = pb["s_out"], &x1 = pb["x1"];
  const float* lapw = h->warena + h->convs.at("art.lap").w_off;
  if (vstarts) launch_video_rows(video, vdt, vlayout, lapw, h->lapw_host, b.org(xs), b.org(xl), xs.set_stride, xs.g, s.H, s.W, st, h->num_sms, vstarts, n_frames);
  else if (inputs_ready) launch_video_rows(b.f("vid"), LSD_F32, LSD_NDHWC, lapw, h->lapw_host, b.org(xs), b.org(xl), xs.set_stride, xs.g, s.H, s.W, st, h->num_sms);
  else launch_video_rows(video, vdt, vlayout, lapw, h->lapw_host, b.org(xs), b.org(xl), xs.set_stride, xs.g, s.H, s.W, st, h->num_sms);
  g_tl.mark(st, "M:video_rows");
  float* comb = b.f("comb");
  PlanarOut none{nullptr, nullptr, 0, 0, 0, 0};
  const PBuf& hf = pb["hf_f"];
  static const bool ring_env = !(LSD_ENV("LSD_STEM_RING") && atoi(LSD_ENV("LSD_STEM_RING")) == 0);
  if (ring_env && h->stem_ring_w_off != 0 && 128 + 3 * xs.g.RW + 3 <= 640) {
    if ((rc = run_stem_ring(b, xs, so))) return rc;
  } else {
    RUN("visual_encoder.stem", a_.in = &xs; a_.og = xs.g; a_.act = ACT_RELU; a_.yp = &so);
  }
  g_tl.mark(st, "M:stem");
  launch_planar_maxpool(b.org(so), so.plane_stride, so.g, b.org(x1), x1.plane_stride, x1.g, 64, st);
  g_tl.mark(st, "M:maxpool");
  if ((rc = res_stage_umma(b, "visual_encoder.layer1", x1, pb["l1a"], pb["y1"], false, UC_Y_PARITY))) return rc;
  g_tl.mark(st, "M:layer1");
  if ((rc = res_stage_umma(b, "visual_encoder.layer2", pb["y1"], pb["l2a"], pb["y2"], true, P.fold3 ? UC_Y_FOLD : UC_Y_PARITY))) return rc;
  g_tl.mark(st, "M:layer2");
  if (P.fold3) rc = res_stage_fold(b, "visual_encoder.layer3", pb["y2"], s.H2, s.W2, pb["l3a"], s.H3, s.W3, pb["y3"], UC_Y_FOLD);
  else rc = res_stage_umma(b, "visual_encoder.layer3", pb["y2"], pb["l3a"], pb["y3"], true, P.fold4 ? UC_Y_FOLD : UC_Y_PARITY);
  if (rc) return rc;
  g_tl.mark(st, "M:layer3");
  if (P.fold4) rc = res_stage_fold(b, "visual_encoder.layer4", pb["y3"], s.H3, s.W3, pb["l4a"], s.H4, s.W4, pb["y4"], UC_Y_MAP);
  else rc = res_stage_umma(b, "visual_encoder.layer4", pb["y3"], pb["l4a"], pb["y4"], true, UC_Y_PLAIN);
  if (rc) return rc;
  g_tl.mark(st, "M:layer4");
  b.max_ctas = 0;
  const PBuf& y4 = pb["y4"];
  launch_planar_mean2(b.org(y4), y4.plane_stride, y4.g, 256, b.f("v_feat"), 256, 0, pout(b, pb["vfeat_p"], &pb["vfeat_p_lo"]), st);
  cudaEventRecord(h->ev_fork, st);
  cudaStreamWaitEvent(sst, h->ev_fork, 0);
  const bool skip_art = LSD_ENV("LSD_SKIP_ART") != nullptr;
  bs.max_ctas = art_ctas;
  if (!skip_art) {
  RUNS("art.td0", a_.in = &y4; a_.og = y4.g; a_.act = ACT_RELU; a_.yp = &pb["art_a"]);
  RUNS("art.td3", a_.in = &pb["art_a"]; a_.og = y4.g; a_.act = ACT_RELU; a_.yp = &pb["art_b"]);
  launch_planar_mean2(bs.org(pb["art_b"]), pb["art_b"].plane_stride, y4.g, 64, comb + 256, 448, 1, none, sst);
  g_tl.mark(sst, "S:td_feat");
  const PBuf& dl = pb["delta"];
  if (T > 1) launch_planar_delta(bs.org(y4), y4.plane_stride, y4.g, bs.org(dl), dl.plane_stride, dl.g, 256, sst);
  RUNS("art.td0", a_.in = &dl; a_.og = dl.g; a_.act = ACT_RELU; a_.yp = &pb["artd_a"]);
  RUNS("art.td3", a_.in = &pb["artd_a"]; a_.og = dl.g; a_.act = ACT_RELU; a_.yp = &pb["artd_b"]);
  launch_planar_mean2(bs.org(pb["artd_b"]), pb["artd_b"].plane_stride, dl.g, 64, comb + 320, 448, 1, none, sst);
  g_tl.mark(sst, "S:td_delta");
  if (!h->side2_stream) {
    if (cudaStreamCreateWithFlags(&h->side2_stream, cudaStreamNonBlocking) != cudaSuccess || cudaEventCreateWithFlags(&h->ev_join2, cudaEventDisableTiming) != cudaSuccess)
      return lsd_fail(h, LSD_ERR_CUDA, "second side stream creation failed");
  }
  const cudaStream_t hst = h->side2_stream;
  cudaStreamWaitEvent(hst, h->ev_fork, 0);
  BCtx bh = bs;
  bh.st = hst;
  if (const char* e = LSD_ENV("LSD_HF_CTAS")) bh.max_ctas = atoi(e);
  RUNC(bh, "art.hf0", a_.in = &xl; a_.og = xl.g; a_.act = ACT_RELU; a_.yp = &hf);
  g_tl.mark(hst, "S:hf0");
  RUNC(bh, "art.hf3", a_.in = &hf; a_.og = hf.g; a_.act = ACT_RELU; a_.yp = &pb["hf_b"]);
  launch_planar_mean2(bh.org(pb["hf_b"]), pb["hf_b"].plane_stride, hf.g, 64, comb + 384, 448, 1, none, hst);
  g_tl.mark(hst, "S:hf3");
  cudaEventRecord(h->ev_join2, hst);
  cudaStreamWaitEvent(sst, h->ev_join2, 0);
  }
  cudaEventRecord(h->ev_join, sst);
  cudaStream_t tst = st;
  if (pipe_parity >= 0) {
    cudaEventRecord(h->ev_front[pipe_parity], st);
    cudaStreamWaitEvent(h->tail_stream, h->ev_front[pipe_parity], 0);
    tst = h->tail_stream;
  }
  {
  BCtx b{h, ws, &P, tst};
  cudaStream_t st = tst;
  HeadW hw;
  auto cw = [&](const char* key) { return h->warena + h->convs.at(key).w_off; };
  auto cb = [&](const char* key) { return h->warena + h->convs.at(key).shift_off; };
  hw.w0 = cw("art.fuse0"); hw.b0 = cb("art.fuse0"); hw.w2 = cw("art.fuse2"); hw.b2 = cb("art.fuse2");
  hw.wc = cw("head.fc0"); hw.bc = cb("head.fc0");
  hw.lng = b.W("head.ln.w"); hw.lnb = b.W("head.ln.b"); hw.wo = b.W("head.out.w"); hw.bo = b.W("head.out.b");
  if (vt) {
    RUN("cross.vcomb", a_.in = &pb["vfeat_p"]; a_.in_lo = &pb["vfeat_p_lo"]; a_.og = P.gt; a_.y32 = b.f("vcomb"); a_.y32_ld = 1024);
    for (int g = 0; g < n_groups; ++g) {
      if (g == 0) cudaStreamWaitEvent(st, h->ev_audio, 0);
      else if ((rc = var_audio(g, st, 0))) return rc;
      const int pi = plan_of(g), b0 = g * vt->gB;
      BCtx c{h, aws[pi], &PA[pi], st};
      if ((rc = token_path_bf16(c, sA[pi], true, b.f("vcomb") + (size_t)b0 * T * 1024, vt->K))) return rc;
      if (g == 0) cudaStreamWaitEvent(st, h->ev_join, 0);
      launch_head(c.f("tok"), (int64_t)NT * 256, comb + (size_t)b0 * 448, hw, logits + (size_t)b0 * vt->K, sA[pi].B, st, vt->K);
    }
    if (pipe_parity >= 0) cudaEventRecord(h->ev_tail_done[pipe_parity], st);
    return 0;
  }
  if (!audio_early) { if ((rc = audio_encoder_bf16(b, s, inputs_ready, audio, adt))) return rc; }
  const UcGeom gt = P.gt;
  if (tcomb) {
    if (!audio_early) { if ((rc = audio_tokens(b, s))) return rc; }
    RUN("cross.vcomb", a_.in = &pb["vfeat_p"]; a_.in_lo = &pb["vfeat_p_lo"]; a_.og = gt; a_.y32 = b.f("vcomb"); a_.y32_ld = 1024);
    if (audio_early) cudaStreamWaitEvent(st, h->ev_audio, 0);
  } else {
    RUN("projection.visual_proj", a_.in = &pb["vfeat_p"]; a_.in_lo = &pb["vfeat_p_lo"]; a_.og = gt; a_.yp = &pb["vemb_p"]; a_.yp_lo = &pb["vemb_p_lo"]; a_.y32 = b.f("v_emb"); a_.y32_ld = 256);
    if (audio_early) cudaStreamWaitEvent(st, h->ev_audio, 0);
    RUN("projection.audio_proj", a_.in = &pb["afeat_p"]; a_.in_lo = &pb["afeat_p_lo"]; a_.og = P.gta; a_.y32 = b.f("a_emb"); a_.y32_ld = 256);
  }
  g_tl.mark(st, "T:proj");
  if ((rc = token_path_bf16(b, s, tcomb))) return rc;
  float* tok = b.f("tok");
  g_tl.mark(st, "T:tokens");
  cudaStreamWaitEvent(st, h->ev_join, 0);
  launch_head(tok, (int64_t)NT * 256, comb, hw, logits, B, st);
  g_tl.mark(st, "T:head");
  g_tl.dump();
  if (aux) {
    const size_t tb = (size_t)B * T * 256 * sizeof(float);
    if (aux->visual_tokens) {
      if (tcomb) launch_copy_rows(b.f("vcomb"), 1024, aux->visual_tokens, 256, B * T, 256, st);
      else cudaMemcpyAsync(aux->visual_tokens, b.f("v_emb"), tb, cudaMemcpyDeviceToDevice, st);
    }
    if (aux->audio_tokens) cudaMemcpyAsync(aux->audio_tokens, b.f("a_emb"), (size_t)B * TA * 256 * sizeof(float), cudaMemcpyDeviceToDevice, st);
    if (aux->fused_tokens) cudaMemcpyAsync(aux->fused_tokens, b.f("fused"), tb, cudaMemcpyDeviceToDevice, st);
    if (aux->cls_output) launch_copy_rows(tok, (int64_t)NT * 256, aux->cls_output, 256, B, 256, st);
  }
  if (pipe_parity >= 0) cudaEventRecord(h->ev_tail_done[pipe_parity], st);
  }
  return 0;
}

int planar_stage_read(lsd_handle* h, const char* name, const char* name_lo, const char* ws, float* out, int64_t out_elems, int Hf, int Wf,
                      cudaStream_t st) {
  auto it = h->planar_stages.find(name);
  if (it == h->planar_stages.end()) return lsd_fail(h, LSD_ERR_ARG, "unknown planar stage %s", name);
  const PlanarStage& ps = it->second;
  const PlanarStage* pl = nullptr;
  if (name_lo && *name_lo) {
    auto il = h->planar_stages.find(name_lo);
    if (il == h->planar_stages.end()) return lsd_fail(h, LSD_ERR_ARG, "unknown planar stage %s", name_lo);
    pl = &il->second;
  }
  const UcGeom g = make_geom_ex(ps.N, ps.T, ps.H, ps.W, ps.ot, ps.oh, ps.hp_extra, ps.ow, ps.wp_extra);
  if (ps.sets == 1) { Hf = ps.H; Wf = ps.W; }
  if ((int64_t)ps.N * ps.T * Hf * Wf * ps.C != out_elems) return lsd_fail(h, LSD_ERR_SHAPE, "stage %s holds %lld elements", name, (long long)ps.N * ps.T * Hf * Wf * ps.C);
  const __nv_bfloat16* x = reinterpret_cast<const __nv_bfloat16*>(ws + ps.off) + ps.origin;
  const __nv_bfloat16* xlo = pl ? reinterpret_cast<const __nv_bfloat16*>(ws + pl->off) + pl->origin : nullptr;
  launch_unpack_planar_any(x, xlo, ps.plane_stride, ps.set_stride, g, ps.C, ps.sets, Hf, Wf, out, st);
  return 0;
}

int ensure_pipeline(lsd_handle* h) {
  if (h->tail_stream) return 0;
  if (cudaStreamCreateWithFlags(&h->tail_stream, cudaStreamNonBlocking) != cudaSuccess) return lsd_fail(h, LSD_ERR_CUDA, "tail stream creation failed");
  for (int i = 0; i < 2; ++i)
    if (cudaEventCreateWithFlags(&h->ev_front[i], cudaEventDisableTiming) != cudaSuccess ||
        cudaEventCreateWithFlags(&h->ev_tail_done[i], cudaEventDisableTiming) != cudaSuccess)
      return lsd_fail(h, LSD_ERR_CUDA, "pipeline event creation failed");
  return 0;
}

static int subpath_begin(lsd_handle* h, const Shapes& s, BPlan& P, char* ws, size_t ws_bytes, cudaStream_t st) {
  build_plan(s, P);
  if (P.f32.cursor > ws_bytes) return lsd_fail(h, LSD_ERR_WORKSPACE, "workspace too small: need %zu bytes, got %zu", P.f32.cursor, ws_bytes);
  h->stages = P.f32.stages;
  if (int rc = ws_prepare(h, s, P, ws, ws_bytes, st, 0)) return rc;
  return 0;
}

size_t audio_encoder_bf16_bytes(lsd_handle* h, int B, int F, int Ta) {
  Shapes s;
  if (make_shapes(h, B, 1, 16, 16, F, Ta, s) != 0) return 0;
  BPlan P;
  build_plan(s, P);
  return P.f32.cursor + 256;
}

int audio_encoder_bf16_run(lsd_handle* h, int B, int F, int Ta, const void* audio, int adt, float* feats_out, char* ws, size_t ws_bytes,
                           cudaStream_t st) {
  Shapes s;
  int rc = make_shapes(h, B, 1, 16, 16, F, Ta, s);
  if (rc) return rc;
  BPlan P;
  if ((rc = subpath_begin(h, s, P, ws, ws_bytes, st))) return rc;
  BCtx b{h, ws, &P, st};
  if ((rc = audio_encoder_bf16(b, s, false, audio, adt))) return rc;
  cudaMemcpyAsync(feats_out, b.f("a_feat"), (size_t)B * s.A4 * 256 * sizeof(float), cudaMemcpyDeviceToDevice, st);
  return 0;
}

size_t token_path_bf16_bytes(lsd_handle* h, int B, int T, int TA) {
  Shapes s;
  if (make_shapes(h, B, T, 16, 16, 16, 8 * TA, s) != 0) return 0;
  BPlan P;
  build_plan(s, P);
  return P.f32.cursor + 256;
}

int token_path_bf16_run(lsd_handle* h, int B, int T, int TA, const float* v_emb, const float* a_emb, float* fused_out, float* cls_out,
                        char* ws, size_t ws_bytes, cudaStream_t st) {
  Shapes s;
  int rc = make_shapes(h, B, T, 16, 16, 16, 8 * TA, s);
  if (rc) return rc;
  if (s.A4 != TA) return lsd_fail(h, LSD_ERR_SHAPE, "lsd_token_path: unsupported audio token count %d", TA);
  BPlan P;
  if ((rc = subpath_begin(h, s, P, ws, ws_bytes, st))) return rc;
  BCtx b{h, ws, &P, st};
  cudaMemcpyAsync(b.f("a_emb"), a_emb, (size_t)B * TA * 256 * sizeof(float), cudaMemcpyDeviceToDevice, st);
  launch_lerp_tokens_p(v_emb, b.f("v_emb"), B, T, T, 256, pout(b, P.pb.at("vemb_p"), &P.pb.at("vemb_p_lo")), st);
  if ((rc = token_path_bf16(b, s))) return rc;
  if (fused_out) cudaMemcpyAsync(fused_out, b.f("fused"), (size_t)B * T * 256 * sizeof(float), cudaMemcpyDeviceToDevice, st);
  if (cls_out) launch_copy_rows(b.f("tok"), (int64_t)(T + 1) * 256, cls_out, 256, B, 256, st);
  return 0;
}

int forward_bf16(lsd_handle* h, int B, int T, int H, int W, int F, int Ta, const void* video, int vdt, int vlayout,
                 const void* audio, int adt, float* logits, const lsd_aux* aux, char* ws, size_t ws_bytes, cudaStream_t st,
                 bool inputs_ready) {
  Shapes s;
  int rc = make_shapes(h, B, T, H, W, F, Ta, s);
  if (rc) return rc;
  return forward_bf16_impl(h, s, logits, aux, ws, ws_bytes, st, inputs_ready, video, vdt, vlayout, audio, adt);
}

int score_batch_bf16(lsd_handle* h, const uint8_t* track, int n_frames, const int32_t* d_vstarts, const int32_t* d_astarts,
                     const float* mel_full, int Ta_full, int nb, int T, int H, int W, int F, int Ta, float* logits, char* ws,
                     size_t ws_bytes, cudaStream_t st, int pipe_parity) {
  Shapes s;
  int rc = make_shapes(h, nb, T, H, W, F, Ta, s);
  if (rc) return rc;
  BPlan P;
  build_plan(s, P);
  if (P.f32.cursor > ws_bytes) return lsd_fail(h, LSD_ERR_WORKSPACE, "workspace too small: need %zu bytes, got %zu", P.f32.cursor, ws_bytes);
  BCtx b{h, ws, &P, st};
  launch_gather_audio(mel_full, F, Ta_full, d_astarts, b.f("aud"), nb, Ta, st);
  if (video_rows_bulk_ok(track, LSD_U8, LSD_NDHWC, W))
    return forward_bf16_impl(h, s, logits, nullptr, ws, ws_bytes, st, true, track, LSD_U8, LSD_NDHWC, nullptr, 0, d_vstarts, n_frames, pipe_parity);
  launch_gather_windows_u8(track, n_frames, d_vstarts, b.f("vid"), nb, T, H * W * 3, st);
  return forward_bf16_impl(h, s, logits, nullptr, ws, ws_bytes, st, true, nullptr, 0, 0, nullptr, 0, nullptr, 0, pipe_parity);
}

bool variants_shared_route(int T) {
  const char* fe = getenv("LSD_TOK_FUSED");
  return token_front_enabled(T) && !(fe && atoi(fe) == 0) && tok_fused_supported(T + 1);
}

static int variants_group(int B, int K) {
  int cap = 512;
  if (const char* e = getenv("LSD_VARIANT_ROWS")) cap = std::max(1, atoi(e));
  const int per = std::max(1, cap / K);
  const int n_groups = (B + per - 1) / per;
  return std::max(1, (B + n_groups - 1) / n_groups);
}

static size_t variants_visual_bytes(const Shapes& s) {
  BPlan P;
  build_plan(s, P);
  return (P.f32.cursor + 255) & ~size_t(255);
}

static size_t variants_audio_bytes(int rows, int T, int F, int Ta) {
  Shapes sa;
  if (rows < 1 || make_shapes(nullptr, rows, T, 16, 16, F, Ta, sa) != 0) return 0;
  BPlan PA;
  build_plan(sa, PA, false);
  return (PA.f32.cursor + 255) & ~size_t(255);
}

size_t variants_bf16_bytes(lsd_handle* h, int B, int K, int T, int H, int W, int F, int Ta) {
  Shapes s;
  if (B < 1 || K < 1 || make_shapes(h, B, T, H, W, F, Ta, s) != 0) return 0;
  const int gB = variants_group(B, K);
  const size_t a0 = variants_audio_bytes(gB * K, T, F, Ta);
  if (a0 == 0) return 0;
  return variants_visual_bytes(s) + a0 + variants_audio_bytes((gB - 1) * K, T, F, Ta) + 256;
}

static int variants_run(lsd_handle* h, const Shapes& s, int plan_B, VarTail& vt, float* logits, char* ws, size_t ws_bytes, cudaStream_t st,
                        bool inputs_ready, const void* video, int vdt, int vlayout, const int32_t* vstarts, int n_frames) {
  const size_t vb = variants_visual_bytes(s);
  vt.gB = variants_group(plan_B, vt.K);
  const size_t a0 = variants_audio_bytes(vt.gB * vt.K, s.T, s.F, s.Ta);
  if (vb + a0 > ws_bytes) return lsd_fail(h, LSD_ERR_WORKSPACE, "workspace too small: need more than %zu bytes, got %zu", vb + a0, ws_bytes);
  vt.ws = ws + vb;
  vt.ws_bytes = a0;
  vt.ws_last = ws + vb + a0;
  vt.ws_last_bytes = ws_bytes - vb - a0;
  return forward_bf16_impl(h, s, logits, nullptr, ws, vb, st, inputs_ready, video, vdt, vlayout, nullptr, 0, vstarts, n_frames, -1, &vt);
}

int forward_variants_bf16(lsd_handle* h, int B, int K, int T, int H, int W, int F, int Ta, const void* video, int vdt, int vlayout,
                          const void* audio, int adt, float* logits, char* ws, size_t ws_bytes, cudaStream_t st) {
  Shapes s;
  int rc = make_shapes(h, B, T, H, W, F, Ta, s);
  if (rc) return rc;
  VarTail vt;
  vt.K = K; vt.audio = audio; vt.adt = adt;
  return variants_run(h, s, B, vt, logits, ws, ws_bytes, st, false, video, vdt, vlayout, nullptr, 0);
}

int score_offsets_batch_bf16(lsd_handle* h, const uint8_t* track, int n_frames, const int32_t* d_vstarts, const int32_t* d_astarts,
                             const float* mel_full, int Ta_full, int nb, int batch, int K, int T, int H, int W, int F, int Ta, float* logits,
                             char* ws, size_t ws_bytes, cudaStream_t st) {
  Shapes s;
  int rc = make_shapes(h, nb, T, H, W, F, Ta, s);
  if (rc) return rc;
  VarTail vt;
  vt.K = K; vt.mel_full = mel_full; vt.Ta_full = Ta_full; vt.d_astarts = d_astarts;
  if (video_rows_bulk_ok(track, LSD_U8, LSD_NDHWC, W))
    return variants_run(h, s, batch, vt, logits, ws, ws_bytes, st, true, track, LSD_U8, LSD_NDHWC, d_vstarts, n_frames);
  BPlan P;
  build_plan(s, P);
  BCtx b{h, ws, &P, st};
  launch_gather_windows_u8(track, n_frames, d_vstarts, b.f("vid"), nb, T, H * W * 3, st);
  return variants_run(h, s, batch, vt, logits, ws, ws_bytes, st, true, nullptr, 0, 0, nullptr, 0);
}
```

### multimodal-lip-sync-deepfake-detection-system_b200/csrc/umma_conv.cu

```cuda
#include "umma_conv.cuh"
#include "token_kernels.cuh"

#include <algorithm>
#include <cstdio>
#include <cstdlib>
#include <cstring>

#include "lsd_kernels.h"
#include "umma.cuh"

namespace lsd {

using namespace umma;

struct F8 { float v[8]; };
__device__ __noinline__ F8 gelu8(F8 x) {
#pragma unroll
  for (int e = 0; e < 8; ++e) x.v[e] = 0.5f * x.v[e] * (1.0f + erff(x.v[e] * 0.70710678118654752f));
  return x;
}

__device__ __forceinline__ float uc_act(float v, int act) {
  if (act == ACT_RELU) return fmaxf(v, 0.0f);
  if (act == ACT_GELU) return 0.5f * v * (1.0f + erff(v * 0.70710678118654752f));
  return v;
}

__device__ __forceinline__ uint32_t uc_div(uint32_t n, uint32_t m, int s) { return (uint32_t)(((uint64_t)n * m) >> (31 + s)); }
__device__ __forceinline__ bool uc_decode(const UcGeom& g, int64_t P, int& n, int& t, int& h, int& w) {
  if (P < 0 || P >= g.P_total) return false;
  const uint32_t Pu = (uint32_t)P;
  const uint32_t S = uc_div(Pu, g.mSL, g.sSL);
  const int r = (int)(Pu - S * (uint32_t)g.SL);
  const int row = (int)uc_div((uint32_t)r, g.mRW, g.sRW), col = r - row * g.RW;
  n = (int)uc_div(S, g.mTS, g.sTS);
  t = (int)(S - (uint32_t)n * (uint32_t)g.TS) - g.ot;
  h = row - g.oh; w = col - g.ow;
  return (unsigned)t < (unsigned)g.T && (unsigned)h < (unsigned)g.H && (unsigned)w < (unsigned)g.W && n < g.N;
}

__device__ __forceinline__ int64_t uc_flat(const UcGeom& g, int n, int t, int h, int w) {
  return (((int64_t)n * g.TS + t + g.ot) * g.HP + h + g.oh) * g.RW + w + g.ow;
}

__device__ __forceinline__ uint4 pack8(const float* v) {
  uint4 o;
  __nv_bfloat162* ob = reinterpret_cast<__nv_bfloat162*>(&o);
#pragma unroll
  for (int e = 0; e < 4; ++e) ob[e] = __floats2bfloat162_rn(v[2 * e], v[2 * e + 1]);
  return o;
}
__device__ __forceinline__ uint4 pack8_relu(const float* v) {
  uint4 o;
  uint32_t* ow = reinterpret_cast<uint32_t*>(&o);
#pragma unroll
  for (int e = 0; e < 4; ++e) asm("cvt.rn.relu.bf16x2.f32 %0, %1, %2;" : "=r"(ow[e]) : "f"(v[2 * e + 1]), "f"(v[2 * e]));
  return o;
}
__device__ __forceinline__ void unpack8(const uint4& r, float* v) {
  const __nv_bfloat162* rb = reinterpret_cast<const __nv_bfloat162*>(&r);
#pragma unroll
  for (int e = 0; e < 4; ++e) { const float2 f = __bfloat1622float2(rb[e]); v[2 * e] = f.x; v[2 * e + 1] = f.y; }
}

constexpr int UC_THREADS = 512;
constexpr int UC_PROD_WARPS = 4, UC_MMA_WARP0 = 4, UC_MMA_WARPS = 4, UC_EPI_WARP0 = 8, UC_EPI_WARPS = 8;

#define UC_MMA(...) do { if constexpr (CTA2) mma2_bf16_ss_pred(__VA_ARGS__); else mma_bf16_ss_pred(__VA_ARGS__); } while (0)
#define UC_COMMIT(...) do { if constexpr (CTA2) mma2_commit_pred(__VA_ARGS__); else mma_commit_pred(__VA_ARGS__); } while (0)
template <int MODE>
__global__ void __launch_bounds__(UC_THREADS, 1) umma_conv_kernel(const __grid_constant__ UmmaConvP p) {
  constexpr bool GENERIC = MODE == 1, CTA2 = MODE == 3;
  extern __shared__ __align__(1024) uint8_t smem[];
  __shared__ uint64_t full_bar[8], empty_bar[8], tfull_bar[2], tempty_bar[2];
  __shared__ uint64_t full2_bar[8], tempty2_bar[2];
  __shared__ uint32_t tmem_base_s;
  __shared__ __align__(16) float bias_s[256];
  const int tid = threadIdx.x, warp = tid >> 5, lane = tid & 31;
  const bool dbg = p.dbg != nullptr && blockIdx.x == 0 && blockIdx.y == 0;
  if (dbg && tid == 0) p.dbg[0] = clock64();
  const int S = p.MT * 128;
  const uint32_t stage_bytes = p.a_stage_bytes + p.w_stage_bytes;
  const int num_tiles = (int)((p.g.P_total + S - 1) / S);
  const uint32_t cta_rank = CTA2 ? cluster_ctarank() : 0u;
  const int slice = blockIdx.y;
  const bool fold = p.fold != 0;
  const int nst = fold ? (int)p.fslice[slice].nst : p.nst_tile;
  const int ch0 = (fold ? (int)p.fslice[slice].col : slice) * p.Cout;
  const int bcols = CTA2 ? p.Cout >> 1 : p.Cout;
  const uint32_t buf_cols = (uint32_t)(p.MT * p.Cout);
  int tile_first = blockIdx.x, tile_step = gridDim.x, tile_end = num_tiles;
  if constexpr (CTA2) {
    tile_first = blockIdx.x >> 1; tile_step = gridDim.x >> 1; tile_end = (num_tiles + 1) >> 1;
  }
  auto tile_p0 = [&](int tile) -> int64_t {
    if constexpr (CTA2) return (int64_t)min(2 * tile + (int)cta_rank, num_tiles - 1) * S;
    return (int64_t)tile * S;
  };

  const int n_issuers = p.issuers;
  if (tid == 0) {
    for (int i = 0; i < p.stages; ++i) { mbar_init(&full_bar[i], 1); mbar_init(&empty_bar[i], n_issuers); }
    for (int i = 0; i < 2; ++i) { mbar_init(&tfull_bar[i], n_issuers); mbar_init(&tempty_bar[i], UC_EPI_WARPS); mbar_init(&tempty2_bar[i], UC_EPI_WARPS); }
    for (int i = 0; i < p.stages; ++i) mbar_init(&full2_bar[i], 1);
    fence_barrier_init();
  }
  if (warp == UC_EPI_WARP0) {
    if constexpr (CTA2) { tmem_alloc2(&tmem_base_s, p.tmem_cols); tmem_relinquish2(); }
    else { tmem_alloc(&tmem_base_s, p.tmem_cols); tmem_relinquish(); }
  }
  for (int i = tid; i < p.Cout; i += UC_THREADS) bias_s[i] = p.bias ? p.bias[ch0 + i] : 0.0f;
  uint8_t* const bias_a = smem + (size_t)p.stages * stage_bytes + (((size_t)p.nst_tile * sizeof(UcStageDesc) + 127) & ~(size_t)127);
  uint8_t* const bias_b = bias_a + 2048;
  if constexpr (!GENERIC) {
    for (int i = tid; i < 128; i += UC_THREADS) reinterpret_cast<uint4*>(bias_a)[i] = make_uint4(0x3F803F80u, 0x00003F80u, 0u, 0u);
    for (int i = tid; i < 2 * bcols; i += UC_THREADS) {
      uint4 o = make_uint4(0u, 0u, 0u, 0u);
      if (i < bcols && p.bias) {
        const float b = p.bias[ch0 + (int)cta_rank * bcols + i];
        const __nv_bfloat16 hi = __float2bfloat16_rn(b);
        const float r1 = b - __bfloat162float(hi);
        const __nv_bfloat16 mid = __float2bfloat16_rn(r1);
        const __nv_bfloat16 lo = __float2bfloat16_rn(r1 - __bfloat162float(mid));
        o.x = (uint32_t)__bfloat16_as_ushort(hi) | ((uint32_t)__bfloat16_as_ushort(mid) << 16);
        o.y = (uint32_t)__bfloat16_as_ushort(lo);
      }
      reinterpret_cast<uint4*>(bias_b)[i] = o;
    }
    fence_proxy_async_smem();
  }
  UcStageDesc* prog = reinterpret_cast<UcStageDesc*>(smem + (size_t)p.stages * stage_bytes);
  {
    const uint4* psrc = reinterpret_cast<const uint4*>(p.prog + (fold ? (int)p.fslice[slice].prog_off : 0));
    uint4* pdst = reinterpret_cast<uint4*>(prog);
    for (int i = tid; i < nst * 4; i += UC_THREADS) pdst[i] = psrc[i];
  }
  tc_fence_before();
  if constexpr (CTA2) cluster_sync_all();
  else __syncthreads();
  tc_fence_after();
  const uint32_t tmem_base = tmem_base_s;
  if (dbg && tid == 0) p.dbg[1] = clock64();

  if (warp < UC_PROD_WARPS) {
    const int npw = min(UC_PROD_WARPS, p.stages);
    if (warp >= npw) goto done;
    const uint32_t smem_base = smem_u32(smem);
    const uint64_t slice64 = CTA2 ? (uint64_t)cta_rank : (uint64_t)slice;
    int k = 0;
    for (int tile = tile_first; tile < tile_end; tile += tile_step, k += nst) {
      const uint64_t p0_bytes = (uint64_t)tile_p0(tile) * 16u;
      for (int si = ((warp - k) % npw + npw) % npw; si < nst; si += npw) {
        const int kk = k + si;
        const int stage = kk % p.stages;
        const uint32_t ph = (uint32_t)(kk / p.stages) & 1u;
        const UcStageDesc& d = prog[si];
        const uint32_t counts = d.counts;
        const uint32_t n_a = counts & 0xffu, n_all = n_a + ((counts >> 8) & 0xffu);
        const bool is_a = (uint32_t)lane < n_a;
        const bool mine = (uint32_t)lane < n_all;
        const uint32_t j = is_a ? ((uint32_t)lane >> 1) : ((uint32_t)lane - n_a);
        const uint32_t sa = smem_base + (uint32_t)stage * stage_bytes;
        const uint64_t gsrc = is_a ? d.a_src + p0_bytes + (uint64_t)j * d.chunk_stride_b + (uint64_t)(lane & 1) * d.plane_stride_b
                                   : d.w_src + slice64 * d.w_slice_stride_b + (uint64_t)j * (uint64_t)d.w_src_step;
        const uint32_t dst = is_a ? sa + (uint32_t)lane * d.bytesA : sa + p.a_stage_bytes + j * d.w_dst_step;
        const uint32_t nbytes = is_a ? d.bytesA : d.w_copy_bytes;
        const uint32_t tx_bytes = d.tx_bytes;
        mbar_wait(&empty_bar[stage], ph ^ 1u);
        if (dbg && lane == 0 && tile == (int)blockIdx.x && si < 24) p.dbg[32 + si] = clock64();
        if (lane == 0) mbar_arrive_expect_tx(&full_bar[stage], tx_bytes);
        __syncwarp();
        if (mine) bulk_s2(dst, reinterpret_cast<const void*>(gsrc), nbytes, &full_bar[stage]);
        __syncwarp();
        if (dbg && lane == 0 && tile == (int)blockIdx.x && si < 8) p.dbg[56 + si] = clock64();
      }
    }
  } else if (warp < UC_MMA_WARP0 + UC_MMA_WARPS) {
    if (warp - UC_MMA_WARP0 >= n_issuers) goto done;
    if constexpr (CTA2) {
      if (cta_rank != 0) {
        if (warp != UC_MMA_WARP0) goto done;
        int stage = 0;
        uint32_t ph = 0;
        for (int tile = tile_first; tile < tile_end; tile += tile_step)
          for (int si = 0; si < nst; ++si) {
            mbar_wait(&full_bar[stage], ph);
            if (lane == 0) mbar_arrive_cluster(mapa_shared(smem_u32(&full2_bar[stage]), 0u));
            __syncwarp();
            if (++stage == p.stages) { stage = 0; ph ^= 1u; }
          }
        goto done;
      }
    }
    const int warp_u = __shfl_sync(0xffffffffu, warp, 0);
    const int mt_n = p.MT / n_issuers;
    const int mt_lo = (warp_u - UC_MMA_WARP0) * mt_n;
    const uint32_t idesc = idesc_bf16(CTA2 ? 256 : 128, p.Cout);
    const uint32_t smem_base = smem_u32(smem);
    const uint64_t desc_hi64 = ((uint64_t)8 << 32) | ((uint64_t)1 << 46);
    const uint32_t b_lbo = (uint32_t)bcols << 16;
    const uint32_t tap_w = (uint32_t)bcols * 2u;
    const uint32_t leader = elect_one() ? 1u : 0u;
    int stage = 0, lt = 0, dbg_it = 0;
    uint32_t ph = 0;
    for (int tile = tile_first; tile < tile_end; ++lt, tile += tile_step) {
      const int buf = p.nbuf == 2 ? (lt & 1) : 0;
      const uint32_t use = p.nbuf == 2 ? ((uint32_t)lt >> 1) : (uint32_t)lt;
      const uint32_t tb = tmem_base + (uint32_t)buf * buf_cols + (uint32_t)(mt_lo * p.Cout);
      mbar_wait(&tempty_bar[buf], (use & 1u) ^ 1u);
      if constexpr (CTA2) mbar_wait_cluster(&tempty2_bar[buf], (use & 1u) ^ 1u);
      tc_fence_after();
      uint32_t acc = 0;
      if constexpr (!GENERIC) {
        const uint64_t da = desc_hi64 | (uint64_t)(smem_u32(bias_a) >> 4);
        const uint64_t db = desc_hi64 | (uint64_t)((smem_u32(bias_b) >> 4) | b_lbo);
        UC_MMA(tb, da, db, idesc, 0u, leader);
        if (mt_n > 1) UC_MMA(tb + (uint32_t)p.Cout, da, db, idesc, 0u, leader);
        if (mt_n > 2) {
          UC_MMA(tb + 2u * (uint32_t)p.Cout, da, db, idesc, 0u, leader);
          UC_MMA(tb + 3u * (uint32_t)p.Cout, da, db, idesc, 0u, leader);
        }
        acc = 1u;
      }
      for (int si = 0; si < nst; ++si) {
        const uint32_t counts = __shfl_sync(0xffffffffu, prog[si].counts, 0);
        const int b = (int)((counts >> 16) & 0xffu), nc = (int)(counts >> 24);
        const UcBand& bd = p.bands[b];
        const int ntaps = bd.ntaps;
        const uint32_t unitsA = (uint32_t)(S + bd.len_extra);
        const uint32_t a_lbo = (bd.toeplitz ? 1u : unitsA) << 16;
        const uint32_t a_chunk = bd.toeplitz ? 2u : 2u * unitsA;
        const uint32_t w_chunk = (uint32_t)ntaps * tap_w;
        mbar_wait(&full_bar[stage], ph);
        if constexpr (CTA2) mbar_wait_cluster(&full2_bar[stage], ph);
        tc_fence_after();
        if (dbg && warp == UC_MMA_WARP0 && lane == 0 && acc == 0 && lt == 0) p.dbg[2] = clock64();
        if (dbg && warp == UC_MMA_WARP0 && lane == 0 && lt == 0 && dbg_it < 24) p.dbg[8 + dbg_it++] = clock64();
        const uint32_t sa = ((smem_base + (uint32_t)stage * stage_bytes) >> 4) + (uint32_t)mt_lo * 128u;
        const uint32_t sw = ((smem_base + (uint32_t)stage * stage_bytes + p.a_stage_bytes) >> 4) | b_lbo;
        if (ntaps == 1) {
          uint32_t at = (sa | a_lbo) + (uint32_t)bd.rel[0], wj = sw;
#pragma unroll 1
          for (int j = 0; j < nc; ++j, at += a_chunk, wj += w_chunk) {
            const uint64_t da = desc_hi64 | (uint64_t)at, db = desc_hi64 | (uint64_t)wj;
            UC_MMA(tb, da, db, idesc, acc, leader);
            if (mt_n > 1) UC_MMA(tb + (uint32_t)p.Cout, da + 128u, db, idesc, acc, leader);
            acc = 1u;
          }
        } else
        for (int j = 0; j < nc; ++j) {
          const uint32_t aj = (sa + (uint32_t)j * a_chunk) | a_lbo;
          uint32_t wj = sw + (uint32_t)j * w_chunk;
#pragma unroll 1
          for (int tp = 0; tp < ntaps; ++tp) {
            const uint32_t at = aj + (uint32_t)bd.rel[tp];
            const uint64_t da = desc_hi64 | (uint64_t)at, db = desc_hi64 | (uint64_t)wj;
            UC_MMA(tb, da, db, idesc, acc, leader);
            if (mt_n > 1) UC_MMA(tb + (uint32_t)p.Cout, da + 128u, db, idesc, acc, leader);
            if (mt_n > 2) {
              UC_MMA(tb + 2u * (uint32_t)p.Cout, da + 256u, db, idesc, acc, leader);
              UC_MMA(tb + 3u * (uint32_t)p.Cout, da + 384u, db, idesc, acc, leader);
            }
            acc = 1u;
            wj += tap_w;
          }
        }
        UC_COMMIT(&empty_bar[stage], leader);
        if (++stage == p.stages) { stage = 0; ph ^= 1u; }
      }
      UC_COMMIT(&tfull_bar[buf], leader);
      if (dbg && warp == UC_MMA_WARP0 && lane == 0 && lt == 0) p.dbg[3] = clock64();
    }
  } else {
    const int quarter = warp & 3;
    const int half = (warp - UC_EPI_WARP0) >> 2;
    const float act_lo = p.act == ACT_RELU ? 0.0f : -INFINITY;
    const int rowt = quarter * 32 + lane;
    int lt = 0;
    for (int tile = tile_first; tile < tile_end; ++lt, tile += tile_step) {
      const int buf = p.nbuf == 2 ? (lt & 1) : 0;
      const uint32_t use = p.nbuf == 2 ? ((uint32_t)lt >> 1) : (uint32_t)lt;
      const uint32_t tb = tmem_base + (uint32_t)buf * buf_cols + ((uint32_t)(quarter * 32) << 16);
      const int64_t P0 = tile_p0(tile);
      mbar_wait(&tfull_bar[buf], use & 1u);
      tc_fence_after();
      if (dbg && warp == UC_EPI_WARP0 && lane == 0 && lt == 0) p.dbg[4] = clock64();
      const bool split_m = !GENERIC && p.MT >= 2;
      const bool split_c = !split_m && (GENERIC || (p.Cout & 63) == 0);
      const int m_end = (!split_m && !split_c && half == 1) ? 0 : p.MT;
      for (int m = split_m ? half : 0; m < m_end; m += split_m ? 2 : 1) {
        const int64_t P = P0 + (int64_t)m * 128 + rowt;
        int n = 0, t = 0, h = 0, w = 0;
        const bool valid = (p.skip & 8) ? true : uc_decode(p.g, P, n, t, h, w);
        if (fold) { h = p.fslice[slice].h; w = p.fslice[slice].w; }
        const bool inrange = P < p.g.P_total;
        const int64_t outer = valid ? ((int64_t)n * p.g.T + t) * p.g.H + h : 0;
        int64_t dst = P * 8;
        if (valid && p.y_mode == UC_Y_PARITY)
          dst = (int64_t)((h & 1) * 2 + (w & 1)) * p.y_set_stride + uc_flat(p.g2, n, t, h >> 1, w >> 1) * 8;
        else if (valid && p.y_mode == UC_Y_PARITY_H)
          dst = (int64_t)((h & 1) * 2) * p.y_set_stride + uc_flat(p.g2, n, t, h >> 1, w) * 8;
        else if (valid && p.y_mode == UC_Y_FOLD)
          dst = (int64_t)(h * p.ymap_W + w) * p.y_set_stride + uc_flat(p.g2, n, t, 0, 0) * 8;
        else if (valid && p.y_mode == UC_Y_MAP)
          dst = uc_flat(p.g2, n, t, h, w) * 8;
        const bool store_planar = ((p.y_mode == UC_Y_PLAIN && inrange) || (p.y_mode >= UC_Y_PARITY && valid)) && !(p.skip & 4);
        const int cbeg = split_c ? half * (p.Cout >> 1) : 0, cend = split_c ? cbeg + (p.Cout >> 1) : p.Cout;
        if constexpr (!GENERIC) {
          char* yp = reinterpret_cast<char*>(p.y + (int64_t)((ch0 + cbeg) >> 3) * p.y_plane_stride + dst);
          const char* rp = reinterpret_cast<const char*>(p.res + (int64_t)((ch0 + cbeg) >> 3) * p.res_plane_stride + P * 8);
          const int64_t yps = p.y_plane_stride * 2, rps = p.res_plane_stride * 2;
          const bool has_res = p.res != nullptr;
          const bool relu = p.act == ACT_RELU;
          const uint32_t vmask = valid ? 0xffffffffu : 0u;
          uint32_t ta = tb + (uint32_t)(m * p.Cout + cbeg);
#pragma unroll 1
          for (int c = cbeg; c < cend; c += 32, yp += 4 * yps, rp += 4 * rps, ta += 32) {
            float v[32];
            uint4 rr[4];
            tmem_ld32(ta, v);
            if (has_res) {
#pragma unroll
              for (int q = 0; q < 4; ++q) rr[q] = valid ? *reinterpret_cast<const uint4*>(rp + q * rps) : make_uint4(0, 0, 0, 0);
            }
            tmem_ld_wait();
            if (has_res) {
#pragma unroll
              for (int q = 0; q < 4; ++q) {
                float f[8];
                unpack8(rr[q], f);
#pragma unroll
                for (int e = 0; e < 8; ++e) v[8 * q + e] += f[e];
              }
            }
            if (store_planar) {
#pragma unroll
              for (int q = 0; q < 4; ++q) {
                uint4 o = relu ? pack8_relu(v + 8 * q) : pack8(v + 8 * q);
                o.x &= vmask; o.y &= vmask; o.z &= vmask; o.w &= vmask;
                *reinterpret_cast<uint4*>(yp + q * yps) = o;
              }
            }
          }
        } else {
        const float* r32row = p.res32 ? p.res32 + (outer * p.g.W + w) * p.res32_ld + ch0 : nullptr;
        float* y32row = p.y32 ? p.y32 + (outer * p.y32_outer_stride + w + p.y32_row_off) * p.y32_ld + ch0 : nullptr;
        const bool use_res = valid && p.res != nullptr, use_lo = use_res && p.res_lo != nullptr, use_r32 = valid && p.res32 != nullptr;
#pragma unroll 1
        for (int c0 = cbeg; c0 < cend; c0 += 32) {
          float v[32];
          uint4 pre[8];
          tmem_ld32(tb + (uint32_t)(m * p.Cout + c0), v);
          if (use_res) {
            const int64_t roff = (int64_t)((ch0 + c0) >> 3) * p.res_plane_stride + P * 8;
#pragma unroll
            for (int q = 0; q < 4; ++q) pre[q] = *reinterpret_cast<const uint4*>(p.res + roff + (int64_t)q * p.res_plane_stride);
            if (use_lo) {
#pragma unroll
              for (int q = 0; q < 4; ++q) pre[4 + q] = *reinterpret_cast<const uint4*>(p.res_lo + roff + (int64_t)q * p.res_plane_stride);
            }
          } else if (use_r32) {
#pragma unroll
            for (int q = 0; q < 8; ++q) pre[q] = *reinterpret_cast<const uint4*>(r32row + c0 + 4 * q);
          }
          tmem_ld_wait();
#pragma unroll
          for (int q = 0; q < 4; ++q) {
            const int c = c0 + 8 * q;
            F8 x;
#pragma unroll
            for (int e = 0; e < 8; ++e) x.v[e] = v[8 * q + e];
            if (valid) {
              const float4 b0 = *reinterpret_cast<const float4*>(&bias_s[c]);
              const float4 b1 = *reinterpret_cast<const float4*>(&bias_s[c + 4]);
              x.v[0] += b0.x; x.v[1] += b0.y; x.v[2] += b0.z; x.v[3] += b0.w; x.v[4] += b1.x; x.v[5] += b1.y; x.v[6] += b1.z; x.v[7] += b1.w;
              if (use_res) {
                float f[8];
                unpack8(pre[q], f);
#pragma unroll
                for (int e = 0; e < 8; ++e) x.v[e] += f[e];
                if (use_lo) {
                  unpack8(pre[4 + q], f);
#pragma unroll
                  for (int e = 0; e < 8; ++e) x.v[e] += f[e];
                }
              } else if (use_r32) {
                const uint4 q0 = pre[2 * q], q1 = pre[2 * q + 1];
                x.v[0] += __uint_as_float(q0.x); x.v[1] += __uint_as_float(q0.y); x.v[2] += __uint_as_float(q0.z); x.v[3] += __uint_as_float(q0.w);
                x.v[4] += __uint_as_float(q1.x); x.v[5] += __uint_as_float(q1.y); x.v[6] += __uint_as_float(q1.z); x.v[7] += __uint_as_float(q1.w);
              }
              if (p.act == ACT_GELU) {
                x = gelu8(x);
              } else {
#pragma unroll
                for (int e = 0; e < 8; ++e) x.v[e] = fmaxf(x.v[e], act_lo);
              }
              if (y32row) {
                float4* o = reinterpret_cast<float4*>(y32row + c);
                o[0] = make_float4(x.v[0], x.v[1], x.v[2], x.v[3]);
                o[1] = make_float4(x.v[4], x.v[5], x.v[6], x.v[7]);
              }
            } else {
#pragma unroll
              for (int e = 0; e < 8; ++e) x.v[e] = 0.0f;
            }
            if (store_planar) {
              const uint4 hi4 = pack8(x.v);
              const int64_t off = (int64_t)((ch0 + c) >> 3) * p.y_plane_stride + dst;
              *reinterpret_cast<uint4*>(p.y + off) = hi4;
              if (p.ylo) {
                float hf[8];
                unpack8(hi4, hf);
#pragma unroll
                for (int e = 0; e < 8; ++e) hf[e] = x.v[e] - hf[e];
                *reinterpret_cast<uint4*>(p.ylo + off) = pack8(hf);
              }
            }
          }
        }
        }
      }
      tc_fence_before();
      __syncwarp();
      if (lane == 0) {
        if (CTA2 && cta_rank != 0) mbar_arrive_cluster(mapa_shared(smem_u32(&tempty2_bar[buf]), 0u));
        else mbar_arrive(&tempty_bar[buf]);
      }
      if (dbg && warp == UC_EPI_WARP0 && lane == 0 && lt == 0) p.dbg[5] = clock64();
    }
  }
done:
  tc_fence_before();
  if constexpr (CTA2) cluster_sync_all();
  else __syncthreads();
  if (warp == UC_EPI_WARP0) {
    if constexpr (CTA2) tmem_dealloc2(tmem_base, p.tmem_cols);
    else tmem_dealloc(tmem_base, p.tmem_cols);
  }
  if (dbg && tid == 0) { p.dbg[6] = clock64(); p.dbg[7] = num_tiles; }
}

UcStageDesc umma_conv_stage(const UmmaConvP& p, const UcGroup& g, const UcBand& bd, int band, int c0, int col) {
  const int S = p.MT * 128;
  const int bcols = p.cta2 ? p.Cout / 2 : p.Cout;
  const int nc = std::min(p.kpack, g.k16 - c0);
  UcStageDesc d;
  const uint32_t bytesW = (uint32_t)bd.ntaps * (uint32_t)bcols * 32u;
  d.bytesA = bd.toeplitz ? (uint32_t)(S + bd.len_extra + 1 + 2 * (nc - 1)) * 16u : (uint32_t)(S + bd.len_extra) * 16u;
  uint32_t n_a = bd.toeplitz ? 1u : 2u * (uint32_t)nc;
  const bool w_merged = bd.ntaps == g.taps_total;
  uint32_t n_w = w_merged ? 1u : (uint32_t)nc;
  d.w_copy_bytes = w_merged ? (uint32_t)nc * bytesW : bytesW;
  d.w_dst_step = bytesW;
  if (p.skip & 1) n_a = 0;
  if (p.skip & 2) n_w = 0;
  d.tx_bytes = n_a * d.bytesA + (n_w ? (uint32_t)nc * bytesW : 0u);
  d.a_src = reinterpret_cast<uint64_t>(bd.base + (int64_t)c0 * bd.chunk_stride + (int64_t)bd.start * 8);
  d.chunk_stride_b = (uint64_t)bd.chunk_stride * 2u;
  d.plane_stride_b = (uint64_t)bd.plane_stride * 2u;
  d.w_src = reinterpret_cast<uint64_t>(p.w + g.w_off + (col > 0 ? (int64_t)col * g.slice_stride : 0) +
                                       ((int64_t)c0 * g.taps_total + bd.tap_begin) * (int64_t)bcols * 16);
  d.w_slice_stride_b = col >= 0 ? 0u : (uint64_t)g.slice_stride * 2u;
  d.w_src_step = (uint32_t)g.taps_total * (uint32_t)bcols * 32u;
  d.counts = n_a | (n_w << 8) | ((uint32_t)band << 16) | ((uint32_t)nc << 24);
  return d;
}

void umma_conv_build_program(const UmmaConvP& p, UcStageDesc* out) {
  int s = 0;
  for (int gi = 0; gi < p.ngroups; ++gi) {
    const UcGroup& g = p.groups[gi];
    for (int c0 = 0; c0 < g.k16; c0 += p.kpack)
      for (int b = g.band_begin; b < g.band_end; ++b) out[s++] = umma_conv_stage(p, g, p.bands[b], b, c0);
  }
}

size_t umma_conv_smem_bytes(const UmmaConvP& p) {
  size_t b = (size_t)p.stages * (p.a_stage_bytes + p.w_stage_bytes) + (size_t)p.nst_tile * sizeof(UcStageDesc) + 1024;
  return b + umma_conv_extra_smem_bytes(p);
}
int umma_conv_stage_desc_bytes() { return (int)sizeof(UcStageDesc); }
static bool uc_is_generic(const UmmaConvP& p);
size_t umma_conv_extra_smem_bytes(const UmmaConvP& p) {
  if (uc_is_generic(p)) return 0;
  return 128 + 2048 + (size_t)(p.cta2 ? p.Cout / 2 : p.Cout) * 32u;
}

static bool uc_is_generic(const UmmaConvP& p) {
  return p.y32 || p.res32 || p.ylo || p.res_lo || p.act == ACT_GELU || p.y_mode == UC_Y_NONE || (p.Cout & 31);
}
const char* umma_conv_config_error(const UmmaConvP& p) {
  if (2 * p.kpack + p.kpack > 32) return "K chunks per stage exceed the producer lanes";
  if (p.res && p.res32) return "bf16 and fp32 residuals are mutually exclusive";
  if (uc_is_generic(p) && (p.Cout & 63)) return "the generic epilogue needs a column slice that is a multiple of 64";
  if (p.MT / p.issuers > 4 || p.MT % p.issuers) return "unsupported M-tiles per issuing warp";
  if (p.fold && (uc_is_generic(p) || p.cta2 || p.res || p.MT > 4))
    return "folded convolutions need the lean epilogue, no residual, single CTAs and at most 4 M-tiles";
  if (p.cta2 && (uc_is_generic(p) || (p.Cout & 31))) return "CTA pairs need the lean epilogue and a multiple of 32 columns";
  return nullptr;
}

cudaError_t umma_conv_device_init() {
  cudaError_t e = cudaFuncSetAttribute(umma_conv_kernel<0>, cudaFuncAttributeMaxDynamicSharedMemorySize, 223 * 1024);
  if (e == cudaSuccess) e = cudaFuncSetAttribute(umma_conv_kernel<1>, cudaFuncAttributeMaxDynamicSharedMemorySize, 223 * 1024);
  if (e == cudaSuccess) e = cudaFuncSetAttribute(umma_conv_kernel<3>, cudaFuncAttributeMaxDynamicSharedMemorySize, 223 * 1024);
  if (e == cudaSuccess) e = video_rows_device_init();
  return e;
}

void launch_umma_conv(const UmmaConvP& p, int n_slices, cudaStream_t s, int num_sms, int max_ctas) {
  if (const char* why = umma_conv_config_error(p)) { fprintf(stderr, "umma_conv: %s\n", why); abort(); }
  const int S = p.MT * 128;
  const int tiles = (int)((p.g.P_total + S - 1) / S);
  const int budget = (max_ctas > 0 && max_ctas < num_sms) ? max_ctas : num_sms;
  int gx = (budget + n_slices - 1) / n_slices;
  gx = gx < 1 ? 1 : (gx > tiles ? tiles : gx);
  const bool generic = uc_is_generic(p);
  if (p.cta2) {
    if (n_slices != 1) { fprintf(stderr, "umma_conv: CTA pairs take one column slice\n"); abort(); }
    const int pairs = (tiles + 1) / 2;
    int gp = budget / 2;
    gp = gp < 1 ? 1 : (gp > pairs ? pairs : gp);
    cudaLaunchConfig_t cfg = {};
    cfg.gridDim = dim3(2 * gp, 1, 1);
    cfg.blockDim = dim3(UC_THREADS, 1, 1);
    cfg.dynamicSmemBytes = umma_conv_smem_bytes(p);
    cfg.stream = s;
    cudaLaunchAttribute at[1];
    at[0].id = cudaLaunchAttributeClusterDimension;
    at[0].val.clusterDim.x = 2; at[0].val.clusterDim.y = 1; at[0].val.clusterDim.z = 1;
    cfg.attrs = at; cfg.numAttrs = 1;
    cudaLaunchKernelEx(&cfg, umma_conv_kernel<3>, p);
    count_launch();
    return;
  }
  if (p.fold) gx = tiles;
  if (generic) umma_conv_kernel<1><<<dim3(gx, n_slices), UC_THREADS, umma_conv_smem_bytes(p), s>>>(p);
  else umma_conv_kernel<0><<<dim3(gx, n_slices), UC_THREADS, umma_conv_smem_bytes(p), s>>>(p);
  count_launch();
}

__global__ void pack_planar_kernel(const float* __restrict__ x, __nv_bfloat16* __restrict__ y, int64_t plane_stride, int64_t set_stride,
                                   UcGeom g, UcGeom g2, int C, int parity, int64_t total) {
  const int64_t i = (int64_t)blockIdx.x * blockDim.x + threadIdx.x;
  if (i >= total) return;
  const int64_t npos = (int64_t)g.N * g.T * g.H * g.W;
  const int chunk = (int)(i / npos);
  int64_t r = i - (int64_t)chunk * npos;
  const int w = (int)(r % g.W); r /= g.W;
  const int h = (int)(r % g.H); r /= g.H;
  const int t = (int)(r % g.T);
  const int n = (int)(r / g.T);
  const float* src = x + ((((int64_t)n * g.T + t) * g.H + h) * g.W + w) * C + chunk * 8;
  float v[8];
#pragma unroll
  for (int e = 0; e < 8; ++e) v[e] = src[e];
  int64_t dst;
  if (parity) dst = (int64_t)((h & 1) * 2 + (w & 1)) * set_stride + uc_flat(g2, n, t, h >> 1, w >> 1) * 8;
  else dst = uc_flat(g, n, t, h, w) * 8;
  *reinterpret_cast<uint4*>(y + (int64_t)chunk * plane_stride + dst) = pack8(v);
}
void launch_pack_planar(const float* x, __nv_bfloat16* y, int64_t plane_stride, int64_t set_stride, UcGeom g, UcGeom g2, int C,
                        int parity, cudaStream_t s) {
  const int64_t total = (int64_t)g.N * g.T * g.H * g.W * (C / 8);
  if (total == 0) return;
  pack_planar_kernel<<<(unsigned)((total + 255) / 256), 256, 0, s>>>(x, y, plane_stride, set_stride, g, g2, C, parity, total);
  count_launch();
}

__global__ void unpack_planar_kernel(const __nv_bfloat16* __restrict__ x, int64_t plane_stride, UcGeom g, int C, float* __restrict__ y,
                                     int ld, int64_t total) {
  const int64_t i = (int64_t)blockIdx.x * blockDim.x + threadIdx.x;
  if (i >= total) return;
  const int nch = C / 8;
  const int chunk = (int)(i % nch);
  int64_t r = i / nch;
  const int64_t row = r;
  const int w = (int)(r % g.W); r /= g.W;
  const int h = (int)(r % g.H); r /= g.H;
  const int t = (int)(r % g.T);
  const int n = (int)(r / g.T);
  const uint4 v = *reinterpret_cast<const uint4*>(x + (int64_t)chunk * plane_stride + uc_flat(g, n, t, h, w) * 8);
  float f[8];
  unpack8(v, f);
  float4* o = reinterpret_cast<float4*>(y + row * ld + chunk * 8);
  o[0] = make_float4(f[0], f[1], f[2], f[3]);
  o[1] = make_float4(f[4], f[5], f[6], f[7]);
}
void launch_unpack_planar(const __nv_bfloat16* x, int64_t plane_stride, UcGeom g, int C, float* y, int ld, cudaStream_t s) {
  const int64_t total = (int64_t)g.N * g.T * g.H * g.W * (C / 8);
  if (total == 0) return;
  unpack_planar_kernel<<<(unsigned)((total + 255) / 256), 256, 0, s>>>(x, plane_stride, g, C, y, ld, total);
  count_launch();
}

__global__ void unpack_planar_any_kernel(const __nv_bfloat16* __restrict__ x, const __nv_bfloat16* __restrict__ xlo, int64_t plane_stride,
                                         int64_t set_stride, UcGeom g, int C, int sets, int Hf, int Wf, float* __restrict__ y, int64_t total) {
  const int64_t i = (int64_t)blockIdx.x * blockDim.x + threadIdx.x;
  if (i >= total) return;
  const int nch = C / 8;
  const int chunk = (int)(i % nch);
  int64_t r = i / nch;
  const int64_t row = r;
  const int w = (int)(r % Wf); r /= Wf;
  const int h = (int)(r % Hf); r /= Hf;
  const int t = (int)(r % g.T);
  const int n = (int)(r / g.T);
  int64_t src;
  if (sets == 1) src = uc_flat(g, n, t, h, w) * 8;
  else if (g.SL == 1 && sets == Hf * Wf) src = (int64_t)(h * Wf + w) * set_stride + uc_flat(g, n, t, 0, 0) * 8;
  else if (Wf == g.W) src = (int64_t)((h & 1) * 2) * set_stride + uc_flat(g, n, t, h >> 1, w) * 8;
  else src = (int64_t)((h & 1) * 2 + (w & 1)) * set_stride + uc_flat(g, n, t, h >> 1, w >> 1) * 8;
  src += (int64_t)chunk * plane_stride;
  float f[8];
  unpack8(*reinterpret_cast<const uint4*>(x + src), f);
  if (xlo) {
    float fl[8];
    unpack8(*reinterpret_cast<const uint4*>(xlo + src), fl);
#pragma unroll
    for (int e = 0; e < 8; ++e) f[e] += fl[e];
  }
  float4* o = reinterpret_cast<float4*>(y + row * C + chunk * 8);
  o[0] = make_float4(f[0], f[1], f[2], f[3]);
  o[1] = make_float4(f[4], f[5], f[6], f[7]);
}
void launch_unpack_planar_any(const __nv_bfloat16* x, const __nv_bfloat16* xlo, int64_t plane_stride, int64_t set_stride, UcGeom g, int C, int sets,
                              int Hf, int Wf, float* y, cudaStream_t s) {
  const int64_t total = (int64_t)g.N * g.T * Hf * Wf * (C / 8);
  if (total == 0) return;
  unpack_planar_any_kernel<<<(unsigned)((total + 255) / 256), 256, 0, s>>>(x, xlo, plane_stride, set_stride, g, C, sets, Hf, Wf, y, total);
  count_launch();
}

__global__ void planar_mean_kernel(const __nv_bfloat16* __restrict__ x, int64_t plane_stride, UcGeom g, float* __restrict__ y, int ld,
                                   int per_window) {
  __shared__ float part[256][9];
  const int row = blockIdx.x, chunk = blockIdx.y, tid = threadIdx.x;
  const int count = per_window ? g.T * g.H * g.W : g.H * g.W;
  const int n = per_window ? row : row / g.T;
  const int t0 = per_window ? 0 : row % g.T;
  float acc[8] = {0, 0, 0, 0, 0, 0, 0, 0};
  for (int i = tid; i < count; i += blockDim.x) {
    const int w = i % g.W;
    const int r = i / g.W;
    const int h = r % g.H;
    const int t = t0 + r / g.H;
    const uint4 v = *reinterpret_cast<const uint4*>(x + (int64_t)chunk * plane_stride + uc_flat(g, n, t, h, w) * 8);
    float f[8];
    unpack8(v, f);
#pragma unroll
    for (int e = 0; e < 8; ++e) acc[e] += f[e];
  }
#pragma unroll
  for (int e = 0; e < 8; ++e) part[tid][e] = acc[e];
  __syncthreads();
  for (int sft = blockDim.x >> 1; sft > 0; sft >>= 1) {
    if (tid < sft) {
#pragma unroll
      for (int e = 0; e < 8; ++e) part[tid][e] += part[tid + sft][e];
    }
    __syncthreads();
  }
  if (tid < 8) y[(int64_t)row * ld + chunk * 8 + tid] = part[0][tid] / (float)count;
}
void launch_planar_mean(const __nv_bfloat16* x, int64_t plane_stride, UcGeom g, int C, float* y, int ld, int per_window, cudaStream_t s) {
  const int rows = per_window ? g.N : g.N * g.T;
  if (rows == 0) return;
  const int count = per_window ? g.T * g.H * g.W : g.H * g.W;
  int threads = 32;
  while (threads < 256 && threads < count) threads <<= 1;
  planar_mean_kernel<<<dim3(rows, C / 8), threads, 0, s>>>(x, plane_stride, g, y, ld, per_window);
  count_launch();
}

__global__ void planar_delta_kernel(const __nv_bfloat16* __restrict__ x, int64_t xs, UcGeom g, __nv_bfloat16* __restrict__ d, int64_t ds,
                                    UcGeom gd, int64_t total) {
  const int64_t i = (int64_t)blockIdx.x * blockDim.x + threadIdx.x;
  if (i >= total) return;
  const int64_t npos = (int64_t)gd.N * gd.T * gd.H * gd.W;
  const int chunk = (int)(i / npos);
  int64_t r = i - (int64_t)chunk * npos;
  const int w = (int)(r % gd.W); r /= gd.W;
  const int h = (int)(r % gd.H); r /= gd.H;
  const int t = (int)(r % gd.T);
  const int n = (int)(r / gd.T);
  float a[8], b[8], o[8];
  unpack8(*reinterpret_cast<const uint4*>(x + (int64_t)chunk * xs + uc_flat(g, n, t + 1, h, w) * 8), a);
  unpack8(*reinterpret_cast<const uint4*>(x + (int64_t)chunk * xs + uc_flat(g, n, t, h, w) * 8), b);
#pragma unroll
  for (int e = 0; e < 8; ++e) o[e] = a[e] - b[e];
  *reinterpret_cast<uint4*>(d + (int64_t)chunk * ds + uc_flat(gd, n, t, h, w) * 8) = pack8(o);
}
void launch_planar_delta(const __nv_bfloat16* x, int64_t x_plane_stride, UcGeom g, __nv_bfloat16* d, int64_t d_plane_stride, UcGeom gd,
                         int C, cudaStream_t s) {
  const int64_t total = (int64_t)gd.N * gd.T * gd.H * gd.W * (C / 8);
  if (total == 0) return;
  planar_delta_kernel<<<(unsigned)((total + 255) / 256), 256, 0, s>>>(x, x_plane_stride, g, d, d_plane_stride, gd, total);
  count_launch();
}

__global__ void __launch_bounds__(256) planar_maxpool_kernel(const __nv_bfloat16* __restrict__ x, int64_t xs, UcGeom gi, __nv_bfloat16* __restrict__ y,
                                                             int64_t ys, UcGeom go, const __nv_bfloat16* __restrict__ xlo,
                                                             __nv_bfloat16* __restrict__ ylo) {
  const int frame = blockIdx.x, chunk = blockIdx.y;
  const int n = frame / go.T, t = frame - n * go.T;
  const int lane = threadIdx.x & 31, warp = threadIdx.x >> 5, nwarps = blockDim.x >> 5;
  const __nv_bfloat16* xc = x + (int64_t)chunk * xs + uc_flat(gi, n, t, 0, 0) * 8;
  const __nv_bfloat16* xlc = xlo ? xlo + (int64_t)chunk * xs + uc_flat(gi, n, t, 0, 0) * 8 : nullptr;
  __nv_bfloat16* yc = y + (int64_t)chunk * ys + uc_flat(go, n, t, 0, 0) * 8;
  __nv_bfloat16* ylc = ylo ? ylo + (int64_t)chunk * ys + uc_flat(go, n, t, 0, 0) * 8 : nullptr;
  auto ld = [&](int pos, float* f) {
    unpack8(*reinterpret_cast<const uint4*>(xc + pos * 8), f);
    if (xlc) {
      float fl[8];
      unpack8(*reinterpret_cast<const uint4*>(xlc + pos * 8), fl);
#pragma unroll
      for (int e = 0; e < 8; ++e) f[e] += fl[e];
    }
  };
  const int nseg = (gi.W + 31) >> 5;
  const int npairs = go.H * nseg;
  for (int pair = warp; pair < npairs; pair += nwarps) {
    const int h = pair / nseg, seg = pair - h * nseg;
    const int c = seg * 32 + lane;
    float mv[8], ml[8];
#pragma unroll
    for (int e = 0; e < 8; ++e) mv[e] = ml[e] = -INFINITY;
    const bool extra_left = lane == 0 && seg > 0;
#pragma unroll
    for (int dh = 0; dh < 3; ++dh) {
      const int hi = 2 * h - 1 + dh;
      if ((unsigned)hi >= (unsigned)gi.H) continue;
      float f[8];
      if (c < gi.W) {
        ld(hi * gi.RW + c, f);
#pragma unroll
        for (int e = 0; e < 8; ++e) mv[e] = fmaxf(mv[e], f[e]);
      }
      if (extra_left) {
        ld(hi * gi.RW + c - 1, f);
#pragma unroll
        for (int e = 0; e < 8; ++e) ml[e] = fmaxf(ml[e], f[e]);
      }
    }
    const int w = seg * 16 + lane;
    float m[8];
#pragma unroll
    for (int e = 0; e < 8; ++e) {
      const float a = __shfl_sync(0xffffffffu, mv[e], (2 * lane) & 31);
      const float b = __shfl_sync(0xffffffffu, mv[e], (2 * lane + 1) & 31);
      const float cl = __shfl_sync(0xffffffffu, mv[e], (2 * lane - 1) & 31);
      const float left = lane == 0 ? ml[e] : cl;
      m[e] = fmaxf(fmaxf(a, b), left);
    }
    if (lane < 16 && w < go.W) {
      const int dst = (h * go.RW + w) * 8;
      const uint4 hi4 = pack8(m);
      *reinterpret_cast<uint4*>(yc + dst) = hi4;
      if (ylc) {
        float hf[8], lo[8];
        unpack8(hi4, hf);
#pragma unroll
        for (int e = 0; e < 8; ++e) lo[e] = m[e] - hf[e];
        *reinterpret_cast<uint4*>(ylc + dst) = pack8(lo);
      }
    }
  }
}
__global__ void __launch_bounds__(192) planar_maxpool_direct_kernel(const __nv_bfloat16* __restrict__ x, int64_t xs, UcGeom gi,
                                                                    __nv_bfloat16* __restrict__ y, int64_t ys, UcGeom go) {
  const int frame = blockIdx.x, chunk = blockIdx.y;
  const int n = frame / go.T, t = frame - n * go.T;
  const uint4* xc = reinterpret_cast<const uint4*>(x + (int64_t)chunk * xs + uc_flat(gi, n, t, 0, 0) * 8);
  uint4* yc = reinterpret_cast<uint4*>(y + (int64_t)chunk * ys + uc_flat(go, n, t, 0, 0) * 8);
  const uint32_t NINF2 = 0xFF80FF80u;
  const int total = go.H * go.W;
  for (int o = threadIdx.x; o < total; o += blockDim.x) {
    const int h = o / go.W, w = o - h * go.W;
    uint4 v[9];
#pragma unroll
    for (int dh = 0; dh < 3; ++dh)
#pragma unroll
      for (int dw = 0; dw < 3; ++dw) {
        const int hi = 2 * h - 1 + dh, wi = 2 * w - 1 + dw;
        v[dh * 3 + dw] = ((unsigned)hi < (unsigned)gi.H && (unsigned)wi < (unsigned)gi.W) ? xc[hi * gi.RW + wi] : make_uint4(NINF2, NINF2, NINF2, NINF2);
      }
    uint32_t* m = reinterpret_cast<uint32_t*>(&v[0]);
#pragma unroll
    for (int k = 1; k < 9; ++k) {
      const uint32_t* r = reinterpret_cast<const uint32_t*>(&v[k]);
#pragma unroll
      for (int e = 0; e < 4; ++e) {
        const __nv_bfloat162 q = __hmax2(*reinterpret_cast<const __nv_bfloat162*>(&m[e]), *reinterpret_cast<const __nv_bfloat162*>(&r[e]));
        m[e] = *reinterpret_cast<const uint32_t*>(&q);
      }
    }
    yc[h * go.RW + w] = v[0];
  }
}

void launch_planar_maxpool(const __nv_bfloat16* x, int64_t x_plane_stride, UcGeom gi, __nv_bfloat16* y, int64_t y_plane_stride, UcGeom go,
                           int C, cudaStream_t s, const __nv_bfloat16* xlo, __nv_bfloat16* ylo) {
  const int frames = go.N * go.T;
  if (frames == 0 || go.H * go.W == 0) return;
  if (!xlo && !ylo) planar_maxpool_direct_kernel<<<dim3((unsigned)frames, (unsigned)(C / 8)), 192, 0, s>>>(x, x_plane_stride, gi, y, y_plane_stride, go);
  else planar_maxpool_kernel<<<dim3((unsigned)frames, (unsigned)(C / 8)), 256, 0, s>>>(x, x_plane_stride, gi, y, y_plane_stride, go, xlo, ylo);
  count_launch();
}

constexpr int VR_ROWS = 8;
template <typename T> __device__ __forceinline__ float vr_norm(float x) { return x; }
template <> __device__ __forceinline__ float vr_norm<uint8_t>(float x) { return x / 255.0f; }
template <typename T, int LAYOUT>
__global__ void __launch_bounds__(256) video_rows_kernel(const T* __restrict__ video, const float* __restrict__ lapw,
                                                         __nv_bfloat16* __restrict__ xs, __nv_bfloat16* __restrict__ xl, int64_t set_stride,
                                                         UcGeom g, int Tn, int H, int W, int bands, float inv_div) {
  extern __shared__ float tile[];
  const int tx = threadIdx.x, ty = threadIdx.y;
  const int WP2 = W + 2, per_c = (VR_ROWS + 2) * WP2;
  const int band = blockIdx.x % bands;
  const int nt = blockIdx.x / bands;
  const int t = nt % Tn, n = nt / Tn;
  const int h0 = band * VR_ROWS;
  __shared__ float lw[81];
  if (ty == 0 && tx < 27) { lw[tx] = lapw[tx]; lw[tx + 27] = lapw[tx + 27]; lw[tx + 54] = lapw[tx + 54]; }
  for (int r = ty; r < VR_ROWS + 2; r += 8) {
    const int hh = h0 + r - 1;
    const bool rin = (unsigned)hh < (unsigned)H;
    if (LAYOUT == 0) {
      const T* rp0 = video + ((((int64_t)n * 3) * Tn + t) * H + (rin ? hh : 0)) * W;
      const int64_t cstride = (int64_t)Tn * H * W;
      for (int col0 = 0; col0 < WP2; col0 += 128) {
        float vals[3][4];
#pragma unroll
        for (int c = 0; c < 3; ++c)
#pragma unroll
          for (int k = 0; k < 4; ++k) {
            const int ww = col0 + tx + 32 * k - 1;
            vals[c][k] = (rin && (unsigned)ww < (unsigned)W) ? vr_norm<T>((float)rp0[c * cstride + ww]) : 0.f;
          }
#pragma unroll
        for (int c = 0; c < 3; ++c)
#pragma unroll
          for (int k = 0; k < 4; ++k) {
            const int col = col0 + tx + 32 * k;
            if (col < WP2) tile[c * per_c + r * WP2 + col] = vals[c][k];
          }
      }
    } else {
      const T* rp = video + (((int64_t)nt * H + (rin ? hh : 0)) * W) * 3;
      for (int e0 = 0; e0 < 3 * WP2; e0 += 256) {
        float vals[8];
#pragma unroll
        for (int k = 0; k < 8; ++k) {
          const int e = e0 + tx + 32 * k, col = e / 3, c = e - col * 3, ww = col - 1;
          vals[k] = (rin && e < 3 * WP2 && (unsigned)ww < (unsigned)W) ? vr_norm<T>((float)rp[ww * 3 + c]) : 0.f;
        }
#pragma unroll
        for (int k = 0; k < 8; ++k) {
          const int e = e0 + tx + 32 * k, col = e / 3, c = e - col * 3;
          if (e < 3 * WP2) tile[c * per_c + r * WP2 + col] = vals[k];
        }
      }
    }
  }
  __syncthreads();
  const int h = h0 + ty;
  if (h >= H) return;
  const int64_t row_dst = (int64_t)(h & 1) * set_stride + uc_flat(g, n, t, h >> 1, 0) * 8 + 16;
  for (int p0 = 4 * tx; p0 < W; p0 += 128) {
    float acc[4][3];
#pragma unroll
    for (int q = 0; q < 4; ++q) acc[q][0] = acc[q][1] = acc[q][2] = 0.f;
    float ctr[4][3];
#pragma unroll
    for (int kh = 0; kh < 3; ++kh)
#pragma unroll
      for (int ci = 0; ci < 3; ++ci) {
        float x[6];
        const float* trow = &tile[ci * per_c + (ty + kh) * WP2 + p0];
#pragma unroll
        for (int j = 0; j < 6; ++j) x[j] = (p0 + j < WP2) ? trow[j] : 0.f;
        if (kh == 1) {
#pragma unroll
          for (int q = 0; q < 4; ++q) ctr[q][ci] = x[q + 1];
        }
#pragma unroll
        for (int kw = 0; kw < 3; ++kw) {
          const int wi = ((kh * 3 + kw) * 3 + ci) * 3;
          const float w0 = lw[wi], w1 = lw[wi + 1], w2 = lw[wi + 2];
#pragma unroll
          for (int q = 0; q < 4; ++q) {
            acc[q][0] = fmaf(w0, x[q + kw], acc[q][0]);
            acc[q][1] = fmaf(w1, x[q + kw], acc[q][1]);
            acc[q][2] = fmaf(w2, x[q + kw], acc[q][2]);
          }
        }
      }
#pragma unroll
    for (int u = 0; u < 2; ++u) {
      if (p0 + 2 * u >= W) break;
      float px[8], lp[8];
#pragma unroll
      for (int q = 0; q < 2; ++q) {
        const bool in = p0 + 2 * u + q < W;
#pragma unroll
        for (int c = 0; c < 3; ++c) {
          px[q * 4 + c] = in ? ctr[2 * u + q][c] : 0.f;
          lp[q * 4 + c] = in ? acc[2 * u + q][c] : 0.f;
        }
        px[q * 4 + 3] = 0.f;
        lp[q * 4 + 3] = 0.f;
      }
      *reinterpret_cast<uint4*>(xs + row_dst + (int64_t)(p0 + 2 * u) * 4) = pack8(px);
      *reinterpret_cast<uint4*>(xl + row_dst + (int64_t)(p0 + 2 * u) * 4) = pack8(lp);
    }
  }
}

constexpr int VR2_ROWS = 16, VR2_STAGES = 3, VR2_THREADS = 256;
template <typename T> __device__ __forceinline__ void vr_load4(const T* p, float* o);
template <> __device__ __forceinline__ void vr_load4<float>(const float* p, float* o) {
  const float4 v = *reinterpret_cast<const float4*>(p);
  o[0] = v.x; o[1] = v.y; o[2] = v.z; o[3] = v.w;
}
template <> __device__ __forceinline__ void vr_load4<__half>(const __half* p, float* o) {
  const uint2 v = *reinterpret_cast<const uint2*>(p);
  const float2 a = __half22float2(*reinterpret_cast<const __half2*>(&v.x)), b = __half22float2(*reinterpret_cast<const __half2*>(&v.y));
  o[0] = a.x; o[1] = a.y; o[2] = b.x; o[3] = b.y;
}
template <> __device__ __forceinline__ void vr_load4<__nv_bfloat16>(const __nv_bfloat16* p, float* o) {
  const uint2 v = *reinterpret_cast<const uint2*>(p);
  const float2 a = __bfloat1622float2(*reinterpret_cast<const __nv_bfloat162*>(&v.x)), b = __bfloat1622float2(*reinterpret_cast<const __nv_bfloat162*>(&v.y));
  o[0] = a.x; o[1] = a.y; o[2] = b.x; o[3] = b.y;
}
template <> __device__ __forceinline__ void vr_load4<uint8_t>(const uint8_t* p, float* o) {
  const uint32_t v = *reinterpret_cast<const uint32_t*>(p);
  o[0] = (float)(v & 0xffu) / 255.0f; o[1] = (float)((v >> 8) & 0xffu) / 255.0f;
  o[2] = (float)((v >> 16) & 0xffu) / 255.0f; o[3] = (float)(v >> 24) / 255.0f;
}
template <typename T> __device__ __forceinline__ void vr_load4_lut(const T* p, float* o, const float*) { vr_load4<T>(p, o); }
__device__ __forceinline__ float vr_u8_norm(float x) {
  const float c = 1.0f / 255.0f;
  const float q = x * c;
  return fmaf(fmaf(-255.0f, q, x), c, q);
}
template <> __device__ __forceinline__ void vr_load4_lut<uint8_t>(const uint8_t* p, float* o, const float* lut) {
  const uint32_t v = *reinterpret_cast<const uint32_t*>(p);
  if (lut) { o[0] = lut[v & 0xffu]; o[1] = lut[(v >> 8) & 0xffu]; o[2] = lut[(v >> 16) & 0xffu]; o[3] = lut[v >> 24]; return; }
  o[0] = vr_u8_norm((float)(v & 0xffu)); o[1] = vr_u8_norm((float)((v >> 8) & 0xffu));
  o[2] = vr_u8_norm((float)((v >> 16) & 0xffu)); o[3] = vr_u8_norm((float)(v >> 24));
}
template <typename T> __device__ __forceinline__ float vr_norm_lut(T x, const float*) { return vr_norm<T>((float)x); }
template <> __device__ __forceinline__ float vr_norm_lut<uint8_t>(uint8_t x, const float* lut) { return lut ? lut[x] : vr_u8_norm((float)x); }

struct VrLapW { float w[81]; };
template <typename T, int LAYOUT>
__global__ void __launch_bounds__(VR2_THREADS, 3) video_rows_tma_kernel(const T* __restrict__ video, const int32_t* __restrict__ starts, int n_frames,
                                                                    const __grid_constant__ VrLapW LW, __nv_bfloat16* __restrict__ xs,
                                                                    __nv_bfloat16* __restrict__ xl, int64_t set_stride, UcGeom g, int Tn, int H, int W,
                                                                    int bands, int num_tiles) {
  extern __shared__ __align__(128) uint8_t vr_smem[];
  __shared__ uint64_t full_bar[VR2_STAGES];
  const float* lut = nullptr;
  const int tid = threadIdx.x;
  const int row_elems = LAYOUT == 0 ? W : 3 * W;
  const int plane_elems = (VR2_ROWS + 2) * row_elems;
  const uint32_t stage_bytes = (uint32_t)((LAYOUT == 0 ? 3 : 1) * plane_elems * (int)sizeof(T));
  const uint32_t stage_pitch = (stage_bytes + 127u) & ~127u;
  if (tid == 0) {
    for (int i = 0; i < VR2_STAGES; ++i) mbar_init(&full_bar[i], 1);
    fence_barrier_init();
  }
  __syncthreads();

  auto issue = [&](int k) {
    const int tile = blockIdx.x + k * gridDim.x;
    if (tile >= num_tiles) return;
    const int band = tile % bands, nt = tile / bands;
    const int h0 = band * VR2_ROWS;
    const int r_lo = h0 == 0 ? 1 : 0;
    const int r_hi = min(VR2_ROWS + 2, H - h0 + 1);
    const uint32_t bytes = (uint32_t)((r_hi - r_lo) * row_elems * (int)sizeof(T));
    uint8_t* dst = vr_smem + (size_t)(k % VR2_STAGES) * stage_pitch + (size_t)r_lo * row_elems * sizeof(T);
    uint64_t* bar = &full_bar[k % VR2_STAGES];
    if (LAYOUT == 0) {
      const int n = nt / Tn, t = nt - n * Tn;
      mbar_arrive_expect_tx(bar, 3u * bytes);
#pragma unroll
      for (int c = 0; c < 3; ++c) {
        const T* src = video + ((((int64_t)n * 3 + c) * Tn + t) * H + (h0 - 1 + r_lo)) * W;
        bulk_g2s(dst + (size_t)c * plane_elems * sizeof(T), src, bytes, bar);
      }
    } else {
      int64_t frame = nt;
      if (starts) {
        const int n = nt / Tn, t = nt - n * Tn;
        int f = starts[n] + t;
        frame = f < 0 ? 0 : (f >= n_frames ? n_frames - 1 : f);
      }
      mbar_arrive_expect_tx(bar, bytes);
      bulk_g2s(dst, video + (frame * H + (h0 - 1 + r_lo)) * (int64_t)row_elems, bytes, bar);
    }
  };
  if (tid == 0)
    for (int k = 0; k < VR2_STAGES - 1; ++k) issue(k);

  const int nstrips = W >> 2;
  const int ntasks = VR2_ROWS * nstrips;
  for (int k = 0;; ++k) {
    const int tile = blockIdx.x + k * gridDim.x;
    if (tile >= num_tiles) break;
    if (tid == 0) issue(k + VR2_STAGES - 1);
    mbar_wait(&full_bar[k % VR2_STAGES], (uint32_t)(k / VR2_STAGES) & 1u);
    const T* st = reinterpret_cast<const T*>(vr_smem + (size_t)(k % VR2_STAGES) * stage_pitch);
    const int band = tile % bands, nt = tile / bands;
    const int n = nt / Tn, t = nt - n * Tn;
    const int h0 = band * VR2_ROWS;
    for (int task = tid; task < ntasks; task += VR2_THREADS) {
      const int ty = task / nstrips, p0 = (task - ty * nstrips) << 2;
      const int h = h0 + ty;
      if (h >= H) break;
      float acc[4][3], ctr[4][3];
#pragma unroll
      for (int q = 0; q < 4; ++q) acc[q][0] = acc[q][1] = acc[q][2] = 0.f;
#pragma unroll
      for (int kh = 0; kh < 3; ++kh) {
        const int hh = h - 1 + kh;
        float x[3][6];
        if ((unsigned)hh < (unsigned)H) {
          const T* trow = st + (size_t)(ty + kh) * row_elems;
          if (LAYOUT == 0) {
#pragma unroll
            for (int ci = 0; ci < 3; ++ci) {
              const T* pr = trow + (size_t)ci * plane_elems + p0;
              vr_load4_lut<T>(pr, &x[ci][1], lut);
              x[ci][0] = p0 > 0 ? vr_norm_lut<T>(pr[-1], lut) : 0.f;
              x[ci][5] = p0 + 4 < W ? vr_norm_lut<T>(pr[4], lut) : 0.f;
            }
          } else {
            const T* pr = trow + 3 * p0;
            float e[12];
            vr_load4_lut<T>(pr, e, lut); vr_load4_lut<T>(pr + 4, e + 4, lut); vr_load4_lut<T>(pr + 8, e + 8, lut);
#pragma unroll
            for (int q = 0; q < 4; ++q)
#pragma unroll
              for (int ci = 0; ci < 3; ++ci) x[ci][q + 1] = e[q * 3 + ci];
#pragma unroll
            for (int ci = 0; ci < 3; ++ci) {
              x[ci][0] = p0 > 0 ? vr_norm_lut<T>(pr[ci - 3], lut) : 0.f;
              x[ci][5] = p0 + 4 < W ? vr_norm_lut<T>(pr[12 + ci], lut) : 0.f;
            }
          }
        } else {
#pragma unroll
          for (int ci = 0; ci < 3; ++ci)
#pragma unroll
            for (int j = 0; j < 6; ++j) x[ci][j] = 0.f;
        }
        if (kh == 1) {
#pragma unroll
          for (int q = 0; q < 4; ++q)
#pragma unroll
            for (int ci = 0; ci < 3; ++ci) ctr[q][ci] = x[ci][q + 1];
        }
#pragma unroll
        for (int ci = 0; ci < 3; ++ci)
#pragma unroll
          for (int kw = 0; kw < 3; ++kw) {
            const int wi = ((kh * 3 + kw) * 3 + ci) * 3;
            const float w0 = LW.w[wi], w1 = LW.w[wi + 1], w2 = LW.w[wi + 2];
#pragma unroll
            for (int q = 0; q < 4; ++q) {
              acc[q][0] = fmaf(w0, x[ci][q + kw], acc[q][0]);
              acc[q][1] = fmaf(w1, x[ci][q + kw], acc[q][1]);
              acc[q][2] = fmaf(w2, x[ci][q + kw], acc[q][2]);
            }
          }
      }
      const int64_t dst = (int64_t)(h & 1) * set_stride + uc_flat(g, n, t, h >> 1, 0) * 8 + 16 + (int64_t)p0 * 4;
#pragma unroll
      for (int u = 0; u < 2; ++u) {
        float px[8], lp[8];
#pragma unroll
        for (int q = 0; q < 2; ++q) {
#pragma unroll
          for (int c = 0; c < 3; ++c) { px[q * 4 + c] = ctr[2 * u + q][c]; lp[q * 4 + c] = acc[2 * u + q][c]; }
          px[q * 4 + 3] = 0.f; lp[q * 4 + 3] = 0.f;
        }
        *reinterpret_cast<uint4*>(xs + dst + u * 8) = pack8(px);
        *reinterpret_cast<uint4*>(xl + dst + u * 8) = pack8(lp);
      }
    }
    __syncthreads();
  }
}

cudaError_t video_rows_device_init() {
  cudaError_t e = cudaSuccess;
#define VRA(TT, LL) if (e == cudaSuccess) e = cudaFuncSetAttribute(video_rows_tma_kernel<TT, LL>, cudaFuncAttributeMaxDynamicSharedMemorySize, 96 * 1024)
  VRA(float, 0); VRA(__half, 0); VRA(__nv_bfloat16, 0); VRA(uint8_t, 0);
  VRA(float, 1); VRA(__half, 1); VRA(__nv_bfloat16, 1); VRA(uint8_t, 1);
#undef VRA
  return e;
}

bool video_rows_bulk_ok(const void* video, int dtype, int layout, int W) {
  const size_t esz = dtype == 0 ? 4 : (dtype == 3 ? 1 : 2);
  const size_t row_bytes = (size_t)W * esz * (layout == 0 ? 1 : 3);
  const size_t stage = (((layout == 0 ? 3 : 1) * (size_t)(VR2_ROWS + 2) * row_bytes) + 127) & ~size_t(127);
  return (W % 4 == 0) && (row_bytes % 16 == 0) && (reinterpret_cast<uintptr_t>(video) % 16 == 0) && stage * VR2_STAGES <= 96 * 1024;
}

void launch_video_rows(const void* video, int dtype, int layout, const float* lapw, const float* lapw_host, __nv_bfloat16* xs, __nv_bfloat16* xl,
                       int64_t set_stride, UcGeom g, int H, int W, cudaStream_t s, int num_sms, const int32_t* starts, int n_frames) {
  const size_t esz = dtype == 0 ? 4 : (dtype == 3 ? 1 : 2);
  const size_t row_bytes = (size_t)W * esz * (layout == 0 ? 1 : 3);
  const size_t stage = (((layout == 0 ? 3 : 1) * (size_t)(VR2_ROWS + 2) * row_bytes) + 127) & ~size_t(127);
  if (video_rows_bulk_ok(video, dtype, layout, W)) {
    const int bands = (H + VR2_ROWS - 1) / VR2_ROWS;
    const int64_t tiles = (int64_t)g.N * g.T * bands;
    if (tiles == 0) return;
    const size_t smem = stage * VR2_STAGES;
    VrLapW lw;
    memcpy(lw.w, lapw_host, sizeof(lw.w));
    const int64_t per_sm = stage * VR2_STAGES * 3 <= 200 * 1024 ? 3 : 2;
    const unsigned grid = (unsigned)std::min<int64_t>(tiles, per_sm * num_sms);
#define VRT(TT, LL)                                                                                                             \
  do {                                                                                                                          \
    video_rows_tma_kernel<TT, LL><<<grid, VR2_THREADS, smem, s>>>(reinterpret_cast<const TT*>(video), starts, n_frames, lw, xs, xl,    \
                                                                  set_stride, g, g.T, H, W, bands, (int)tiles);               \
  } while (0)
    if (layout == 0) {
      if (dtype == 0) VRT(float, 0); else if (dtype == 1) VRT(__half, 0); else if (dtype == 2) VRT(__nv_bfloat16, 0); else VRT(uint8_t, 0);
    } else {
      if (dtype == 0) VRT(float, 1); else if (dtype == 1) VRT(__half, 1); else if (dtype == 2) VRT(__nv_bfloat16, 1); else VRT(uint8_t, 1);
    }
#undef VRT
    count_launch();
    return;
  }
  const int bands = (H + VR_ROWS - 1) / VR_ROWS;
  const int64_t blocks = (int64_t)g.N * g.T * bands;
  if (blocks == 0) return;
  const size_t smem = (size_t)3 * (VR_ROWS + 2) * (W + 2) * sizeof(float);
#define VR(TT, LL, DIV) video_rows_kernel<TT, LL><<<(unsigned)blocks, dim3(32, 8), smem, s>>>(reinterpret_cast<const TT*>(video), lapw, xs, xl, set_stride, g, g.T, H, W, bands, 1.0f / (DIV))
  if (layout == 0) {
    if (dtype == 0) VR(float, 0, 1.0f); else if (dtype == 1) VR(__half, 0, 1.0f); else if (dtype == 2) VR(__nv_bfloat16, 0, 1.0f); else VR(uint8_t, 0, 255.0f);
  } else {
    if (dtype == 0) VR(float, 1, 1.0f); else if (dtype == 1) VR(__half, 1, 1.0f); else if (dtype == 2) VR(__nv_bfloat16, 1, 1.0f); else VR(uint8_t, 1, 255.0f);
  }
#undef VR
  count_launch();
}

__global__ void planar_mean2_kernel(const __nv_bfloat16* __restrict__ x, int64_t plane_stride, UcGeom g, float* __restrict__ y32, int ld,
                                    int mode, PlanarOut po, const __nv_bfloat16* __restrict__ xlo) {
  __shared__ float part[256][9];
  const int row = blockIdx.x, chunk = blockIdx.y, tid = threadIdx.x;
  const int count = mode == 1 ? g.T * g.H * g.W : (mode == 0 ? g.H * g.W : g.H);
  float acc[8] = {0, 0, 0, 0, 0, 0, 0, 0};
  auto add = [&](int64_t pos) {
    float f[8];
    const int64_t src = (int64_t)chunk * plane_stride + pos * 8;
    unpack8(*reinterpret_cast<const uint4*>(x + src), f);
#pragma unroll
    for (int e = 0; e < 8; ++e) acc[e] += f[e];
    if (xlo) {
      unpack8(*reinterpret_cast<const uint4*>(xlo + src), f);
#pragma unroll
      for (int e = 0; e < 8; ++e) acc[e] += f[e];
    }
  };
  if (mode == 2) {
    const int n = row / g.W, w = row % g.W;
    for (int i = tid; i < count; i += blockDim.x) add(uc_flat(g, n, 0, i, w));
  } else {
    const int n = mode == 1 ? row : row / g.T, t0 = mode == 1 ? 0 : row % g.T;
    const int n_rows = (mode == 1 ? g.T : 1) * g.H;
    const int lane = tid & 31, warp = tid >> 5, nwarps = blockDim.x >> 5;
    if (g.W <= 32 && !xlo) {
      const bool act = lane < g.W;
      const __nv_bfloat16* xc = x + (int64_t)chunk * plane_stride;
      int rr = warp;
      for (; rr + 3 * nwarps < n_rows; rr += 4 * nwarps) {
        uint4 v[4];
#pragma unroll
        for (int u = 0; u < 4; ++u) {
          const int r = rr + u * nwarps, tt = r / g.H, h = r - tt * g.H;
          v[u] = act ? *reinterpret_cast<const uint4*>(xc + (uc_flat(g, n, t0 + tt, h, 0) + lane) * 8) : make_uint4(0, 0, 0, 0);
        }
#pragma unroll
        for (int u = 0; u < 4; ++u) {
          float f[8];
          unpack8(v[u], f);
#pragma unroll
          for (int e = 0; e < 8; ++e) acc[e] += f[e];
        }
      }
      for (; rr < n_rows; rr += nwarps) {
        const int tt = rr / g.H, h = rr - tt * g.H;
        if (act) add(uc_flat(g, n, t0 + tt, h, 0) + lane);
      }
    } else
    for (int rr = warp; rr < n_rows; rr += nwarps) {
      const int tt = rr / g.H, h = rr - tt * g.H;
      const int64_t base = uc_flat(g, n, t0 + tt, h, 0);
      for (int w = lane; w < g.W; w += 32) add(base + w);
    }
  }
#pragma unroll
  for (int e = 0; e < 8; ++e) part[tid][e] = acc[e];
  __syncthreads();
  for (int sft = blockDim.x >> 1; sft > 0; sft >>= 1) {
    if (tid < sft) {
#pragma unroll
      for (int e = 0; e < 8; ++e) part[tid][e] += part[tid + sft][e];
    }
    __syncthreads();
  }
  if (tid < 8) {
    const float m = part[0][tid] / (float)count;
    if (y32) y32[(int64_t)row * ld + chunk * 8 + tid] = m;
    if (po.y) {
      const int64_t pos = po.grp > 0 ? ((int64_t)row / po.grp) * po.grp_stride + (row % po.grp) + po.off : (int64_t)row + po.off;
      const __nv_bfloat16 hi = __float2bfloat16_rn(m);
      po.y[(int64_t)chunk * po.plane_stride + pos * 8 + tid] = hi;
      if (po.ylo) po.ylo[(int64_t)chunk * po.plane_stride + pos * 8 + tid] = __float2bfloat16_rn(m - __bfloat162float(hi));
    }
  }
}
__global__ void __launch_bounds__(256) planar_mean2_small_kernel(const __nv_bfloat16* __restrict__ x, int64_t plane_stride, UcGeom g,
                                                                 float* __restrict__ y32, int ld, int mode, PlanarOut po,
                                                                 const __nv_bfloat16* __restrict__ xlo, int rows, int nchunks) {
  const int i = blockIdx.x * blockDim.x + threadIdx.x;
  if (i >= rows * nchunks) return;
  const int chunk = i / rows, row = i - chunk * rows;
  const int count = mode == 0 ? g.H * g.W : g.H;
  float acc[8] = {0, 0, 0, 0, 0, 0, 0, 0};
  for (int k = 0; k < count; ++k) {
    int n, t, h, w;
    if (mode == 2) { n = row / g.W; w = row - n * g.W; t = 0; h = k; }
    else { n = row / g.T; t = row - n * g.T; h = k / g.W; w = k - h * g.W; }
    const int64_t off = (int64_t)chunk * plane_stride + uc_flat(g, n, t, h, w) * 8;
    float f[8];
    unpack8(*reinterpret_cast<const uint4*>(x + off), f);
    if (xlo) {
      float fl[8];
      unpack8(*reinterpret_cast<const uint4*>(xlo + off), fl);
#pragma unroll
      for (int e = 0; e < 8; ++e) f[e] += fl[e];
    }
#pragma unroll
    for (int e = 0; e < 8; ++e) acc[e] += f[e];
  }
  float m[8];
#pragma unroll
  for (int e = 0; e < 8; ++e) m[e] = acc[e] / (float)count;
  if (y32) {
    float4* o = reinterpret_cast<float4*>(y32 + (int64_t)row * ld + chunk * 8);
    o[0] = make_float4(m[0], m[1], m[2], m[3]);
    o[1] = make_float4(m[4], m[5], m[6], m[7]);
  }
  if (po.y) {
    const int64_t pos = po.grp > 0 ? ((int64_t)row / po.grp) * po.grp_stride + (row % po.grp) + po.off : (int64_t)row + po.off;
    const uint4 hi4 = pack8(m);
    *reinterpret_cast<uint4*>(po.y + (int64_t)chunk * po.plane_stride + pos * 8) = hi4;
    if (po.ylo) {
      float hf[8], lo[8];
      unpack8(hi4, hf);
#pragma unroll
      for (int e = 0; e < 8; ++e) lo[e] = m[e] - hf[e];
      *reinterpret_cast<uint4*>(po.ylo + (int64_t)chunk * po.plane_stride + pos * 8) = pack8(lo);
    }
  }
}

void launch_planar_mean2(const __nv_bfloat16* x, int64_t plane_stride, UcGeom g, int C, float* y32, int ld, int mode, PlanarOut po, cudaStream_t s,
                         const __nv_bfloat16* xlo) {
  const int rows = mode == 1 ? g.N : (mode == 0 ? g.N * g.T : g.N * g.W);
  if (rows == 0) return;
  const int count = mode == 1 ? g.T * g.H * g.W : (mode == 0 ? g.H * g.W : g.H);
  if (mode != 1 && count <= 32 && (ld % 4) == 0 && (!y32 || reinterpret_cast<uintptr_t>(y32) % 16 == 0)) {
    const int total = rows * (C / 8);
    planar_mean2_small_kernel<<<(total + 255) / 256, 256, 0, s>>>(x, plane_stride, g, y32, ld, mode, po, xlo, rows, C / 8);
    count_launch();
    return;
  }
  int threads = 32;
  while (threads < 256 && threads < count) threads <<= 1;
  planar_mean2_kernel<<<dim3(rows, C / 8), threads, 0, s>>>(x, plane_stride, g, y32, ld, mode, po, xlo);
  count_launch();
}

}
```

### multimodal-lip-sync-deepfake-detection-system_b200/csrc/umma_conv.cuh

```cuda
#pragma once
#include <cuda_bf16.h>
#include <cuda_runtime.h>
#include <stdint.h>

namespace lsd {

constexpr int UC_MAX_BANDS = 16;
constexpr int UC_MAX_TAPS = 12;
constexpr int UC_MAX_GROUPS = 6;

struct UcBand {
  const __nv_bfloat16* base;
  int64_t plane_stride;
  int64_t chunk_stride;
  int start;
  int len_extra;
  int ntaps;
  int tap_begin;
  int toeplitz;
  int rel[UC_MAX_TAPS];
};

struct UcGroup {
  int band_begin, band_end;
  int k16;
  int taps_total;
  int64_t w_off;
  int64_t slice_stride;
};

enum UcOut { UC_Y_NONE = 0, UC_Y_PLAIN = 1, UC_Y_PARITY = 2, UC_Y_PARITY_H = 3, UC_Y_FOLD = 5, UC_Y_MAP = 6 };

constexpr int UC_MAX_FSLICES = 96;
struct UcFoldSlice {
  uint16_t prog_off, nst;
  uint8_t h, w;
  uint8_t col, pad_;
};

struct UcGeom {
  int N, T, H, W;
  int TS, ot, HP, oh, RW, ow, SL;
  int64_t P_total;
  uint32_t mSL, mRW, mTS;
  int sSL, sRW, sTS;
};

inline void uc_magic(uint32_t d, uint32_t& m, int& s) {
  s = 0;
  while (((uint64_t)1 << s) < d) ++s;
  m = (uint32_t)((((uint64_t)1 << (31 + s)) / d) + 1);
}

struct alignas(16) UcStageDesc {
  uint64_t a_src;
  uint64_t w_src;
  uint64_t chunk_stride_b;
  uint64_t plane_stride_b;
  uint64_t w_slice_stride_b;
  uint32_t bytesA;
  uint32_t w_copy_bytes;
  uint32_t w_dst_step;
  uint32_t w_src_step;
  uint32_t tx_bytes;
  uint32_t counts;
};
static_assert(sizeof(UcStageDesc) == 64, "UcStageDesc must be 64 bytes");

struct UmmaConvP {
  const __nv_bfloat16* w;
  const float* bias;
  const __nv_bfloat16* res;
  const __nv_bfloat16* res_lo;
  int64_t res_plane_stride;
  const float* res32;
  int res32_ld;
  __nv_bfloat16* y;
  __nv_bfloat16* ylo;
  int64_t y_plane_stride, y_set_stride;
  int y_mode;
  float* y32;
  int y32_ld;
  int y32_outer_stride, y32_row_off;
  int act;
  int Cout;
  int MT, stages, ngroups, nbands;
  int issuers;
  int nbuf;
  long long* dbg;
  const UcStageDesc* prog;
  int nst_tile;
  int skip;
  int kpack;
  uint32_t a_stage_bytes, w_stage_bytes, tmem_cols;
  int cta2;
  UcGeom g;
  UcGeom g2;
  UcGroup groups[UC_MAX_GROUPS];
  UcBand bands[UC_MAX_BANDS];
  int ymap_W;
  int fold;
  UcFoldSlice fslice[UC_MAX_FSLICES];
};

size_t umma_conv_smem_bytes(const UmmaConvP& p);
int umma_conv_stage_desc_bytes();
size_t umma_conv_extra_smem_bytes(const UmmaConvP& p);
void umma_conv_build_program(const UmmaConvP& p, UcStageDesc* out);
UcStageDesc umma_conv_stage(const UmmaConvP& p, const UcGroup& g, const UcBand& bd, int band, int c0, int col = -1);
const char* umma_conv_config_error(const UmmaConvP& p);
void launch_umma_conv(const UmmaConvP& p, int n_slices, cudaStream_t s, int num_sms, int max_ctas = 0);
cudaError_t umma_conv_device_init();
cudaError_t video_rows_device_init();

void launch_pack_planar(const float* x, __nv_bfloat16* y, int64_t plane_stride, int64_t set_stride, UcGeom g, UcGeom g2, int C,
                        int parity, cudaStream_t s);
void launch_unpack_planar(const __nv_bfloat16* x, int64_t plane_stride, UcGeom g, int C, float* y, int ld, cudaStream_t s);
void launch_unpack_planar_any(const __nv_bfloat16* x, const __nv_bfloat16* xlo, int64_t plane_stride, int64_t set_stride, UcGeom g, int C, int sets,
                              int Hf, int Wf, float* y, cudaStream_t s);
void launch_planar_mean(const __nv_bfloat16* x, int64_t plane_stride, UcGeom g, int C, float* y, int ld, int per_window, cudaStream_t s);
void launch_planar_delta(const __nv_bfloat16* x, int64_t x_plane_stride, UcGeom g, __nv_bfloat16* d, int64_t d_plane_stride, UcGeom gd,
                         int C, cudaStream_t s);
void launch_planar_maxpool(const __nv_bfloat16* x, int64_t x_plane_stride, UcGeom gi, __nv_bfloat16* y, int64_t y_plane_stride, UcGeom go,
                           int C, cudaStream_t s, const __nv_bfloat16* xlo = nullptr, __nv_bfloat16* ylo = nullptr);

void launch_video_rows(const void* video, int dtype, int layout, const float* lapw, const float* lapw_host, __nv_bfloat16* xs, __nv_bfloat16* xl,
                       int64_t set_stride, UcGeom g, int H, int W, cudaStream_t s, int num_sms, const int32_t* starts = nullptr, int n_frames = 0);
bool video_rows_bulk_ok(const void* video, int dtype, int layout, int W);

inline UcGeom make_geom_ex(int N, int T, int H, int W, int tpad, int oh, int hp_extra, int ow, int wp_extra) {
  UcGeom g;
  g.N = N; g.T = T; g.H = H; g.W = W;
  g.TS = T + tpad; g.ot = tpad;
  g.HP = H + oh + hp_extra; g.oh = oh;
  g.RW = W + ow + wp_extra; g.ow = ow;
  g.SL = g.HP * g.RW;
  g.P_total = ((int64_t)N * g.TS + tpad) * g.SL;
  uc_magic((uint32_t)g.SL, g.mSL, g.sSL);
  uc_magic((uint32_t)g.RW, g.mRW, g.sRW);
  uc_magic((uint32_t)g.TS, g.mTS, g.sTS);
  return g;
}
inline UcGeom make_geom(int N, int T, int H, int W) { return make_geom_ex(N, T, H, W, 1, 1, 0, 1, 0); }
inline UcGeom make_geom_rows(int rows) { return make_geom_ex(1, 1, 1, rows, 0, 0, 0, 0, 0); }

}
```

Before: 25850.

## Schedule folded conv jobs via load-balanced per-CTA job lists and fold layer2

Folded convolutions now run as a persistent 'walk' kernel. The host builds a greedy longest-first assignment of (slice, tile) jobs across CTAs, and the kernel reads stage programs and slice metadata from global memory rather than a fixed-size parameter array. It also double-buffers TMEM when the columns fit, widens the fold routing threshold, and allows folding layer2 behind an env flag (default off). The aim is to cut the tail imbalance from slices with uneven stage counts and to remove the slice cap. In exchange, per-stage descriptor reads go to global memory instead of shared memory, and bias staging grows with the number of Cout slices.

```diff
diff --git a/multimodal-lip-sync-deepfake-detection-system_b200/csrc/bf16_path.cu b/multimodal-lip-sync-deepfake-detection-system_b200/csrc/bf16_path.cu
--- a/multimodal-lip-sync-deepfake-detection-system_b200/csrc/bf16_path.cu
+++ b/multimodal-lip-sync-deepfake-detection-system_b200/csrc/bf16_path.cu
@@ -249,12 +249,12 @@
 
 bool fold_route(int H, int W) {
   static const bool off = LSD_ENV("LSD_FOLD") && atoi(LSD_ENV("LSD_FOLD")) == 0;
-  return !off && H * W <= 36;
+  return !off && (int64_t)(H + 1) * (W + 1) * 20 >= (int64_t)23 * H * W;
 }
 
 struct BPlan {
   Shapes s;
-  bool fold3 = false, fold4 = false;
+  bool fold2 = false, fold3 = false, fold4 = false;
   Plan f32;
   std::map<std::string, PBuf> pb;
   size_t planar_begin = 0, planar_end = 0;
@@ -305,11 +305,13 @@
   P.addp("s_out", 64, 1, gs);
   P.addp("x1", 64, 1, g1);
   P.addp("l1a", 64, 1, g1);
-  P.addp("y1", 64, 4, g2);
-  P.addp("l2a", 128, 1, g2);
-  P.fold3 = fold_route(s.H3, s.W3);
+  static const bool fold_l2 = LSD_ENV("LSD_FOLD_LAYER2") && atoi(LSD_ENV("LSD_FOLD_LAYER2")) == 1;
   P.fold4 = fold_route(s.H4, s.W4);
+  P.fold3 = P.fold4 && fold_route(s.H3, s.W3);
+  P.fold2 = fold_l2 && P.fold3 && fold_route(s.H2, s.W2);
   const UcGeom gr = make_geom_ex(Bn, Tn, 1, 1, 1, 0, 0, 0, 0);
+  if (P.fold2) P.addp("y1", 64, s.H1 * s.W1, gr); else P.addp("y1", 64, 4, g2);
+  if (P.fold2) P.addp("l2a", 128, s.H2 * s.W2, gr); else P.addp("l2a", 128, 1, g2);
   if (P.fold3) P.addp("y2", 128, s.H2 * s.W2, gr); else P.addp("y2", 128, 4, g3);
   if (P.fold3) P.addp("l3a", 256, s.H3 * s.W3, gr); else P.addp("l3a", 256, 1, g3);
   if (P.fold4) P.addp("y3", 256, s.H3 * s.W3, gr); else P.addp("y3", 256, 4, g4);
@@ -387,7 +389,7 @@
   int res32_ld = 0;
 };
 
-int stage_program(const BCtx& c, const std::string& name, UmmaConvP& p, const std::function<void(std::vector<UcStageDesc>&)>& build,
+int stage_program(const BCtx& c, const std::string& name, UmmaConvP& p, const std::function<void(std::vector<char>&)>& build,
                   std::initializer_list<uint64_t> salt = {}) {
   uint64_t hkey = 1469598103934665603ull;
   for (uint64_t v : salt) { hkey ^= v; hkey *= 1099511628211ull; hkey ^= hkey >> 29; }
@@ -396,9 +398,9 @@
   for (size_t i = 0; i < sizeof(p) / 8; ++i) { hkey ^= pw[i]; hkey *= 1099511628211ull; hkey ^= hkey >> 29; }
   auto it = c.h->prog_cache.find(hkey);
   if (it == c.h->prog_cache.end()) {
-    std::vector<UcStageDesc> host;
+    std::vector<char> host;
     build(host);
-    const size_t bytes = host.size() * sizeof(UcStageDesc);
+    const size_t bytes = host.size();
     if (!c.h->prog_arena) {
       c.h->prog_cap = 64u << 20;
       if (cudaMalloc(&c.h->prog_arena, c.h->prog_cap) != cudaSuccess) return lsd_fail(c.h, LSD_ERR_CUDA, "stage-program arena allocation failed");
@@ -547,7 +549,10 @@
   if (L.groups[0].toeplitz) { const ConvP& cp = c.h->convs.at(name); kflop = (double)cp.kt * cp.kh * cp.kw * cp.Cin; }
   if (const char* e = getenv("LSD_UMMA_SKIP")) p.skip = atoi(e);
   if (const char* why = umma_conv_config_error(p)) return lsd_fail(c.h, LSD_ERR_UNSUPPORTED, "%s: %s", name.c_str(), why);
-  if (int rc = stage_program(c, name, p, [&](std::vector<UcStageDesc>& v) { v.resize((size_t)p.nst_tile); umma_conv_build_program(p, v.data()); }))
+  if (int rc = stage_program(c, name, p, [&](std::vector<char>& v) {
+        v.resize((size_t)p.nst_tile * sizeof(UcStageDesc));
+        umma_conv_build_program(p, reinterpret_cast<UcStageDesc*>(v.data()));
+      }))
     return rc;
   if (const char* e = getenv("LSD_UMMA_TRACE")) {
     static long long* dbuf = nullptr;
@@ -759,13 +764,14 @@
   p.y_plane_stride = yp.plane_stride; p.y_set_stride = yp.set_stride;
   p.g2 = yp.g;
   p.ymap_W = Wo;
+  static const bool walk = !(LSD_ENV("LSD_FOLD_WALK") && atoi(LSD_ENV("LSD_FOLD_WALK")) == 0);
   int mt = 2;
   if (const char* e = LSD_ENV("LSD_FOLD_MT")) mt = std::max(1, std::min(4, atoi(e)));
   p.MT = (int)std::max<int64_t>(1, std::min<int64_t>(mt, (og.P_total + 127) / 128));
-  p.nbuf = 1;
+  p.nbuf = walk && 2 * p.MT * L.ntile <= 512 ? 2 : 1;
   p.issuers = std::min(p.MT, 4);
   uint32_t cols = 32;
-  while ((int)cols < p.MT * L.ntile) cols *= 2;
+  while ((int)cols < p.nbuf * p.MT * L.ntile) cols *= 2;
   p.tmem_cols = cols;
   const int S = p.MT * 128;
   const PBuf* srcs[2] = {&x, x_ds};
@@ -807,17 +813,27 @@
     }
   std::stable_sort(pos.begin(), pos.end(), [](const std::array<int, 3>& a, const std::array<int, 3>& b) { return a[0] < b[0]; });
   const int nslices = (int)pos.size() * cslices;
-  if (nslices > UC_MAX_FSLICES || Ho > 255 || Wo > 255) return lsd_fail(c.h, LSD_ERR_UNSUPPORTED, "%s: map too large for the folded route", name.c_str());
+  if (Ho > 255 || Wo > 255) return lsd_fail(c.h, LSD_ERR_UNSUPPORTED, "%s: map too large for the folded route", name.c_str());
   auto chunks = [&](int k16) { return (k16 + p.kpack - 1) / p.kpack; };
-  int off = 0;
+  std::vector<UcFoldSlice> fslices((size_t)nslices);
+  uint32_t off = 0;
+  int max_nst = 0;
   for (int i = 0; i < nslices; ++i) {
     const auto& q = pos[(size_t)(i / cslices)];
     const int nst = -q[0] * chunks(p.groups[0].k16) + (x_ds ? chunks(p.groups[1].k16) : 0);
-    p.fslice[i] = UcFoldSlice{(uint16_t)off, (uint16_t)nst, (uint8_t)q[1], (uint8_t)q[2], (uint8_t)(i % cslices), 0};
-    p.nst_tile = std::max(p.nst_tile, nst);
-    off += nst;
-  }
-  if (off > 65535) return lsd_fail(c.h, LSD_ERR_UNSUPPORTED, "%s: folded stage programs too long", name.c_str());
+    fslices[(size_t)i] = UcFoldSlice{off, (uint16_t)nst, (uint8_t)q[1], (uint8_t)q[2], (uint32_t)(i % cslices)};
+    max_nst = std::max(max_nst, nst);
+    off += (uint32_t)nst;
+  }
+  const int tiles = (int)((og.P_total + S - 1) / S);
+  const int64_t njobs = (int64_t)nslices * tiles;
+  const int cta_budget = (c.max_ctas > 0 && c.max_ctas < c.h->num_sms) ? c.max_ctas : c.h->num_sms;
+  if (walk) {
+    p.fcols = cslices;
+    p.fctas = (int)std::min<int64_t>(cta_budget, njobs);
+  } else {
+    p.nst_tile = max_nst;
+  }
   const uint32_t stage = p.a_stage_bytes + p.w_stage_bytes;
   const uint32_t prog_bytes = (uint32_t)p.nst_tile * (uint32_t)umma_conv_stage_desc_bytes();
   const uint32_t budget = 211u * 1024u - (uint32_t)umma_conv_extra_smem_bytes(p);
@@ -825,9 +841,10 @@
   p.stages = std::max(2, std::min((int)((budget - prog_bytes) / stage), 8));
   if (const char* e = getenv("LSD_UMMA_SKIP")) p.skip = atoi(e);
   if (const char* why = umma_conv_config_error(p)) return lsd_fail(c.h, LSD_ERR_UNSUPPORTED, "%s: %s", name.c_str(), why);
-  auto build = [&](std::vector<UcStageDesc>& v) {
+  auto build = [&](std::vector<char>& blob) {
+    std::vector<UcStageDesc> v;
     for (int i = 0; i < nslices; ++i) {
-      const UcFoldSlice& f = p.fslice[i];
+      const UcFoldSlice& f = fslices[(size_t)i];
       for (int kh = 0; kh < 3; ++kh)
         for (int kw = 0; kw < 3; ++kw) {
           if (!inb(f.h, kh, Hi) || !inb(f.w, kw, Wi)) continue;
@@ -842,9 +859,51 @@
         for (int c0 = 0; c0 < p.groups[1].k16; c0 += p.kpack) v.push_back(umma_conv_stage(p, p.groups[1], bd, 1, c0, f.col));
       }
     }
+    auto put = [&](const void* src, size_t bytes) {
+      const size_t at = (blob.size() + 15) & ~size_t(15);
+      blob.resize(at + bytes);
+      memcpy(blob.data() + at, src, bytes);
+      return at;
+    };
+    put(v.data(), v.size() * sizeof(UcStageDesc));
+    put(fslices.data(), fslices.size() * sizeof(UcFoldSlice));
+    if (!walk) return;
+    std::vector<int64_t> order((size_t)njobs);
+    for (int64_t j = 0; j < njobs; ++j) order[(size_t)j] = j;
+    std::stable_sort(order.begin(), order.end(), [&](int64_t a, int64_t b) {
+      return fslices[(size_t)(a / tiles)].nst > fslices[(size_t)(b / tiles)].nst;
+    });
+    std::vector<std::vector<UcFoldJob>> lists((size_t)p.fctas);
+    std::vector<std::pair<int64_t, int>> load;
+    for (int k = 0; k < p.fctas; ++k) load.push_back({0, k});
+    auto later = [](const std::pair<int64_t, int>& a, const std::pair<int64_t, int>& b) { return a > b; };
+    for (int64_t j : order) {
+      std::pop_heap(load.begin(), load.end(), later);
+      auto& l = load.back();
+      const int sl = (int)(j / tiles);
+      lists[(size_t)l.second].push_back(UcFoldJob{(uint32_t)sl, (int32_t)(j % tiles)});
+      l.first += fslices[(size_t)sl].nst;
+      std::push_heap(load.begin(), load.end(), later);
+    }
+    std::vector<uint32_t> offs;
+    std::vector<UcFoldJob> jobs;
+    for (const auto& l : lists) { offs.push_back((uint32_t)jobs.size()); jobs.insert(jobs.end(), l.begin(), l.end()); }
+    offs.push_back((uint32_t)jobs.size());
+    put(offs.data(), offs.size() * sizeof(uint32_t));
+    put(jobs.data(), jobs.size() * sizeof(UcFoldJob));
   };
   if (int rc = stage_program(c, name + "#fold", p, build, {(uint64_t)Hi, (uint64_t)Wi, (uint64_t)stride, (uint64_t)Hd, (uint64_t)Wd,
-                                                          (uint64_t)x.set_stride, (uint64_t)(x_ds ? x_ds->set_stride : 0)})) return rc;
+                                                          (uint64_t)x.set_stride, (uint64_t)(x_ds ? x_ds->set_stride : 0),
+                                                          (uint64_t)Ho, (uint64_t)Wo, (uint64_t)walk, (uint64_t)cta_budget})) return rc;
+  const size_t slice_at = ((size_t)off * sizeof(UcStageDesc) + 15) & ~size_t(15);
+  const size_t off_at = (slice_at + (size_t)nslices * sizeof(UcFoldSlice) + 15) & ~size_t(15);
+  const size_t job_at = (off_at + (size_t)(p.fctas + 1) * sizeof(uint32_t) + 15) & ~size_t(15);
+  const char* blob = reinterpret_cast<const char*>(p.prog);
+  p.fslice = reinterpret_cast<const UcFoldSlice*>(blob + slice_at);
+  if (walk) {
+    p.fjob_off = reinterpret_cast<const uint32_t*>(blob + off_at);
+    p.fjobs = reinterpret_cast<const UcFoldJob*>(blob + job_at);
+  }
   double kflop = 0;
   for (const BGroup& G : L.groups) kflop += (double)G.taps_total * G.Cin;
   c.h->prof.begin(c.st, 2.0 * (double)og.N * og.T * Ho * Wo * L.Cout * kflop, 2);
@@ -973,7 +1032,7 @@
     P.add(p + ".conv1", p + ".conv1", s, s, "", nt, false, l >= 2, pairs);
     P.ds_sh = 2; P.ds_sw = 2;
     P.add(p + ".conv2", p + ".conv2", 1, 1, l == 1 ? "" : p + ".downsample", nt, false, false, pairs);
-    if (l >= 3) {
+    if (l >= 2) {
       int fnt = 128;
       if (const char* e = LSD_ENV("LSD_FOLD_NT")) fnt = atoi(e) == 256 ? 256 : 128;
       P.add_fold(p + ".conv1#fold", p + ".conv1", "", fnt);
@@ -1363,9 +1422,11 @@
   g_tl.mark(st, "M:stem");
   launch_planar_maxpool(b.org(so), so.plane_stride, so.g, b.org(x1), x1.plane_stride, x1.g, 64, st);
   g_tl.mark(st, "M:maxpool");
-  if ((rc = res_stage_umma(b, "visual_encoder.layer1", x1, pb["l1a"], pb["y1"], false, UC_Y_PARITY))) return rc;
+  if ((rc = res_stage_umma(b, "visual_encoder.layer1", x1, pb["l1a"], pb["y1"], false, P.fold2 ? UC_Y_FOLD : UC_Y_PARITY))) return rc;
   g_tl.mark(st, "M:layer1");
-  if ((rc = res_stage_umma(b, "visual_encoder.layer2", pb["y1"], pb["l2a"], pb["y2"], true, P.fold3 ? UC_Y_FOLD : UC_Y_PARITY))) return rc;
+  if (P.fold2) rc = res_stage_fold(b, "visual_encoder.layer2", pb["y1"], s.H1, s.W1, pb["l2a"], s.H2, s.W2, pb["y2"], UC_Y_FOLD);
+  else rc = res_stage_umma(b, "visual_encoder.layer2", pb["y1"], pb["l2a"], pb["y2"], true, P.fold3 ? UC_Y_FOLD : UC_Y_PARITY);
+  if (rc) return rc;
   g_tl.mark(st, "M:layer2");
   if (P.fold3) rc = res_stage_fold(b, "visual_encoder.layer3", pb["y2"], s.H2, s.W2, pb["l3a"], s.H3, s.W3, pb["y3"], UC_Y_FOLD);
   else rc = res_stage_umma(b, "visual_encoder.layer3", pb["y2"], pb["l3a"], pb["y3"], true, P.fold4 ? UC_Y_FOLD : UC_Y_PARITY);
diff --git a/multimodal-lip-sync-deepfake-detection-system_b200/csrc/umma_conv.cu b/multimodal-lip-sync-deepfake-detection-system_b200/csrc/umma_conv.cu
--- a/multimodal-lip-sync-deepfake-detection-system_b200/csrc/umma_conv.cu
+++ b/multimodal-lip-sync-deepfake-detection-system_b200/csrc/umma_conv.cu
@@ -70,7 +70,7 @@
 #define UC_COMMIT(...) do { if constexpr (CTA2) mma2_commit_pred(__VA_ARGS__); else mma_commit_pred(__VA_ARGS__); } while (0)
 template <int MODE>
 __global__ void __launch_bounds__(UC_THREADS, 1) umma_conv_kernel(const __grid_constant__ UmmaConvP p) {
-  constexpr bool GENERIC = MODE == 1, CTA2 = MODE == 3;
+  constexpr bool GENERIC = MODE == 1, CTA2 = MODE == 3, WALK = MODE == 4;
   extern __shared__ __align__(1024) uint8_t smem[];
   __shared__ uint64_t full_bar[8], empty_bar[8], tfull_bar[2], tempty_bar[2];
   __shared__ uint64_t full2_bar[8], tempty2_bar[2];
@@ -85,14 +85,21 @@
   const uint32_t cta_rank = CTA2 ? cluster_ctarank() : 0u;
   const int slice = blockIdx.y;
   const bool fold = p.fold != 0;
-  const int nst = fold ? (int)p.fslice[slice].nst : p.nst_tile;
-  const int ch0 = (fold ? (int)p.fslice[slice].col : slice) * p.Cout;
+  constexpr bool walk = WALK;
+  const int nst = fold ? (walk ? 0 : (int)p.fslice[slice].nst) : p.nst_tile;
+  const int ch0 = (fold ? (walk ? 0 : (int)p.fslice[slice].col) : slice) * p.Cout;
   const int bcols = CTA2 ? p.Cout >> 1 : p.Cout;
   const uint32_t buf_cols = (uint32_t)(p.MT * p.Cout);
   int tile_first = blockIdx.x, tile_step = gridDim.x, tile_end = num_tiles;
   if constexpr (CTA2) {
     tile_first = blockIdx.x >> 1; tile_step = gridDim.x >> 1; tile_end = (num_tiles + 1) >> 1;
   }
+  if (walk) { tile_first = (int)p.fjob_off[blockIdx.x]; tile_end = (int)p.fjob_off[blockIdx.x + 1]; tile_step = 1; }
+  auto walk_job = [&](int j, UcFoldSlice& fs) -> int64_t {
+    const UcFoldJob jb = p.fjobs[j];
+    fs = p.fslice[jb.slice];
+    return (int64_t)jb.tile * S;
+  };
   auto tile_p0 = [&](int tile) -> int64_t {
     if constexpr (CTA2) return (int64_t)min(2 * tile + (int)cta_rank, num_tiles - 1) * S;
     return (int64_t)tile * S;
@@ -114,10 +121,11 @@
   uint8_t* const bias_b = bias_a + 2048;
   if constexpr (!GENERIC) {
     for (int i = tid; i < 128; i += UC_THREADS) reinterpret_cast<uint4*>(bias_a)[i] = make_uint4(0x3F803F80u, 0x00003F80u, 0u, 0u);
-    for (int i = tid; i < 2 * bcols; i += UC_THREADS) {
+    for (int i = tid; i < 2 * bcols * (walk ? p.fcols : 1); i += UC_THREADS) {
       uint4 o = make_uint4(0u, 0u, 0u, 0u);
-      if (i < bcols && p.bias) {
-        const float b = p.bias[ch0 + (int)cta_rank * bcols + i];
+      const int r = walk ? i / (2 * bcols) : 0, ic = i - r * 2 * bcols;
+      if (ic < bcols && p.bias) {
+        const float b = p.bias[ch0 + r * p.Cout + (int)cta_rank * bcols + ic];
         const __nv_bfloat16 hi = __float2bfloat16_rn(b);
         const float r1 = b - __bfloat162float(hi);
         const __nv_bfloat16 mid = __float2bfloat16_rn(r1);
@@ -131,7 +139,7 @@
   }
   UcStageDesc* prog = reinterpret_cast<UcStageDesc*>(smem + (size_t)p.stages * stage_bytes);
   {
-    const uint4* psrc = reinterpret_cast<const uint4*>(p.prog + (fold ? (int)p.fslice[slice].prog_off : 0));
+    const uint4* psrc = reinterpret_cast<const uint4*>(p.prog + (fold && !walk ? p.fslice[slice].prog_off : 0u));
     uint4* pdst = reinterpret_cast<uint4*>(prog);
     for (int i = tid; i < nst * 4; i += UC_THREADS) pdst[i] = psrc[i];
   }
@@ -148,13 +156,18 @@
     const uint32_t smem_base = smem_u32(smem);
     const uint64_t slice64 = CTA2 ? (uint64_t)cta_rank : (uint64_t)slice;
     int k = 0;
-    for (int tile = tile_first; tile < tile_end; tile += tile_step, k += nst) {
-      const uint64_t p0_bytes = (uint64_t)tile_p0(tile) * 16u;
-      for (int si = ((warp - k) % npw + npw) % npw; si < nst; si += npw) {
+    for (int tile = tile_first; tile < tile_end; tile += tile_step) {
+      int64_t p0 = 0;
+      int nst_j = nst;
+      const UcStageDesc* gprog = nullptr;
+      if (walk) { UcFoldSlice fs; p0 = walk_job(tile, fs); nst_j = fs.nst; gprog = p.prog + fs.prog_off; }
+      else p0 = tile_p0(tile);
+      const uint64_t p0_bytes = (uint64_t)p0 * 16u;
+      for (int si = ((warp - k) % npw + npw) % npw; si < nst_j; si += npw) {
         const int kk = k + si;
         const int stage = kk % p.stages;
         const uint32_t ph = (uint32_t)(kk / p.stages) & 1u;
-        const UcStageDesc& d = prog[si];
+        const UcStageDesc& d = walk ? gprog[si] : prog[si];
         const uint32_t counts = d.counts;
         const uint32_t n_a = counts & 0xffu, n_all = n_a + ((counts >> 8) & 0xffu);
         const bool is_a = (uint32_t)lane < n_a;
@@ -174,6 +187,7 @@
         __syncwarp();
         if (dbg && lane == 0 && tile == (int)blockIdx.x && si < 8) p.dbg[56 + si] = clock64();
       }
+      k += nst_j;
     }
   } else if (warp < UC_MMA_WARP0 + UC_MMA_WARPS) {
     if (warp - UC_MMA_WARP0 >= n_issuers) goto done;
@@ -207,13 +221,18 @@
       const int buf = p.nbuf == 2 ? (lt & 1) : 0;
       const uint32_t use = p.nbuf == 2 ? ((uint32_t)lt >> 1) : (uint32_t)lt;
       const uint32_t tb = tmem_base + (uint32_t)buf * buf_cols + (uint32_t)(mt_lo * p.Cout);
+      int nst_j = nst;
+      const UcStageDesc* gprog = nullptr;
+      uint32_t bias_off = 0;
+      if (walk) { UcFoldSlice fs; walk_job(tile, fs); nst_j = fs.nst; gprog = p.prog + fs.prog_off; bias_off = fs.col * (uint32_t)bcols * 32u; }
+      uint32_t counts_next = walk && nst_j > 0 ? __ldg(&gprog[0].counts) : 0u;
       mbar_wait(&tempty_bar[buf], (use & 1u) ^ 1u);
       if constexpr (CTA2) mbar_wait_cluster(&tempty2_bar[buf], (use & 1u) ^ 1u);
       tc_fence_after();
       uint32_t acc = 0;
       if constexpr (!GENERIC) {
         const uint64_t da = desc_hi64 | (uint64_t)(smem_u32(bias_a) >> 4);
-        const uint64_t db = desc_hi64 | (uint64_t)((smem_u32(bias_b) >> 4) | b_lbo);
+        const uint64_t db = desc_hi64 | (uint64_t)((smem_u32(bias_b + bias_off) >> 4) | b_lbo);
         UC_MMA(tb, da, db, idesc, 0u, leader);
         if (mt_n > 1) UC_MMA(tb + (uint32_t)p.Cout, da, db, idesc, 0u, leader);
         if (mt_n > 2) {
@@ -222,8 +241,14 @@
         }
         acc = 1u;
       }
-      for (int si = 0; si < nst; ++si) {
-        const uint32_t counts = __shfl_sync(0xffffffffu, prog[si].counts, 0);
+      for (int si = 0; si < nst_j; ++si) {
+        uint32_t counts;
+        if (walk) {
+          counts = __shfl_sync(0xffffffffu, counts_next, 0);
+          if (si + 1 < nst_j) counts_next = __ldg(&gprog[si + 1].counts);
+        } else {
+          counts = __shfl_sync(0xffffffffu, prog[si].counts, 0);
+        }
         const int b = (int)((counts >> 16) & 0xffu), nc = (int)(counts >> 24);
         const UcBand& bd = p.bands[b];
         const int ntaps = bd.ntaps;
@@ -281,7 +306,13 @@
       const int buf = p.nbuf == 2 ? (lt & 1) : 0;
       const uint32_t use = p.nbuf == 2 ? ((uint32_t)lt >> 1) : (uint32_t)lt;
       const uint32_t tb = tmem_base + (uint32_t)buf * buf_cols + ((uint32_t)(quarter * 32) << 16);
-      const int64_t P0 = tile_p0(tile);
+      int64_t P0 = 0;
+      int fh = 0, fw = 0, jch0 = ch0;
+      if (walk) { UcFoldSlice fs; P0 = walk_job(tile, fs); fh = fs.h; fw = fs.w; jch0 = (int)fs.col * p.Cout; }
+      else {
+        P0 = tile_p0(tile);
+        if (fold) { fh = p.fslice[slice].h; fw = p.fslice[slice].w; }
+      }
       mbar_wait(&tfull_bar[buf], use & 1u);
       tc_fence_after();
       if (dbg && warp == UC_EPI_WARP0 && lane == 0 && lt == 0) p.dbg[4] = clock64();
@@ -292,7 +323,7 @@
         const int64_t P = P0 + (int64_t)m * 128 + rowt;
         int n = 0, t = 0, h = 0, w = 0;
         const bool valid = (p.skip & 8) ? true : uc_decode(p.g, P, n, t, h, w);
-        if (fold) { h = p.fslice[slice].h; w = p.fslice[slice].w; }
+        if (fold) { h = fh; w = fw; }
         const bool inrange = P < p.g.P_total;
         const int64_t outer = valid ? ((int64_t)n * p.g.T + t) * p.g.H + h : 0;
         int64_t dst = P * 8;
@@ -307,7 +338,7 @@
         const bool store_planar = ((p.y_mode == UC_Y_PLAIN && inrange) || (p.y_mode >= UC_Y_PARITY && valid)) && !(p.skip & 4);
         const int cbeg = split_c ? half * (p.Cout >> 1) : 0, cend = split_c ? cbeg + (p.Cout >> 1) : p.Cout;
         if constexpr (!GENERIC) {
-          char* yp = reinterpret_cast<char*>(p.y + (int64_t)((ch0 + cbeg) >> 3) * p.y_plane_stride + dst);
+          char* yp = reinterpret_cast<char*>(p.y + (int64_t)((jch0 + cbeg) >> 3) * p.y_plane_stride + dst);
           const char* rp = reinterpret_cast<const char*>(p.res + (int64_t)((ch0 + cbeg) >> 3) * p.res_plane_stride + P * 8);
           const int64_t yps = p.y_plane_stride * 2, rps = p.res_plane_stride * 2;
           const bool has_res = p.res != nullptr;
@@ -483,7 +514,7 @@
 static bool uc_is_generic(const UmmaConvP& p);
 size_t umma_conv_extra_smem_bytes(const UmmaConvP& p) {
   if (uc_is_generic(p)) return 0;
-  return 128 + 2048 + (size_t)(p.cta2 ? p.Cout / 2 : p.Cout) * 32u;
+  return 128 + 2048 + (size_t)(p.cta2 ? p.Cout / 2 : p.Cout) * 32u * (p.fold && p.fctas > 0 ? p.fcols : 1);
 }
 
 static bool uc_is_generic(const UmmaConvP& p) {
@@ -496,6 +527,8 @@
   if (p.MT / p.issuers > 4 || p.MT % p.issuers) return "unsupported M-tiles per issuing warp";
   if (p.fold && (uc_is_generic(p) || p.cta2 || p.res || p.MT > 4))
     return "folded convolutions need the lean epilogue, no residual, single CTAs and at most 4 M-tiles";
+  if (p.fold && p.fctas > 0 && (p.fcols < 1 || p.nst_tile != 0))
+    return "the folded job walk reads its stage programs from global memory and stages every Cout slice's bias";
   if (p.cta2 && (uc_is_generic(p) || (p.Cout & 31))) return "CTA pairs need the lean epilogue and a multiple of 32 columns";
   return nullptr;
 }
@@ -504,6 +537,7 @@
   cudaError_t e = cudaFuncSetAttribute(umma_conv_kernel<0>, cudaFuncAttributeMaxDynamicSharedMemorySize, 223 * 1024);
   if (e == cudaSuccess) e = cudaFuncSetAttribute(umma_conv_kernel<1>, cudaFuncAttributeMaxDynamicSharedMemorySize, 223 * 1024);
   if (e == cudaSuccess) e = cudaFuncSetAttribute(umma_conv_kernel<3>, cudaFuncAttributeMaxDynamicSharedMemorySize, 223 * 1024);
+  if (e == cudaSuccess) e = cudaFuncSetAttribute(umma_conv_kernel<4>, cudaFuncAttributeMaxDynamicSharedMemorySize, 223 * 1024);
   if (e == cudaSuccess) e = video_rows_device_init();
   return e;
 }
@@ -534,6 +568,11 @@
     count_launch();
     return;
   }
+  if (p.fold && p.fctas > 0) {
+    umma_conv_kernel<4><<<dim3(p.fctas, 1), UC_THREADS, umma_conv_smem_bytes(p), s>>>(p);
+    count_launch();
+    return;
+  }
   if (p.fold) gx = tiles;
   if (generic) umma_conv_kernel<1><<<dim3(gx, n_slices), UC_THREADS, umma_conv_smem_bytes(p), s>>>(p);
   else umma_conv_kernel<0><<<dim3(gx, n_slices), UC_THREADS, umma_conv_smem_bytes(p), s>>>(p);
diff --git a/multimodal-lip-sync-deepfake-detection-system_b200/csrc/umma_conv.cuh b/multimodal-lip-sync-deepfake-detection-system_b200/csrc/umma_conv.cuh
--- a/multimodal-lip-sync-deepfake-detection-system_b200/csrc/umma_conv.cuh
+++ b/multimodal-lip-sync-deepfake-detection-system_b200/csrc/umma_conv.cuh
@@ -31,11 +31,15 @@
 
 enum UcOut { UC_Y_NONE = 0, UC_Y_PLAIN = 1, UC_Y_PARITY = 2, UC_Y_PARITY_H = 3, UC_Y_FOLD = 5, UC_Y_MAP = 6 };
 
-constexpr int UC_MAX_FSLICES = 96;
 struct UcFoldSlice {
-  uint16_t prog_off, nst;
+  uint32_t prog_off;
+  uint16_t nst;
   uint8_t h, w;
-  uint8_t col, pad_;
+  uint32_t col;
+};
+struct UcFoldJob {
+  uint32_t slice;
+  int32_t tile;
 };
 
 struct UcGeom {
@@ -100,7 +104,11 @@
   UcBand bands[UC_MAX_BANDS];
   int ymap_W;
   int fold;
-  UcFoldSlice fslice[UC_MAX_FSLICES];
+  int fcols;
+  int fctas;
+  const UcFoldSlice* fslice;
+  const UcFoldJob* fjobs;
+  const uint32_t* fjob_off;
 };
 
 size_t umma_conv_smem_bytes(const UmmaConvP& p);
```

Result: no change. 26040 (median of 6 runs) (+0.7%).
